# ZhengkunTian/OpenTransformer

Measured on AMD Instinct MI355X. Metric: utterances/sec (80-d fbank, ~1000 frames) train fwd+bwd, higher is better.
Workload: dtype fp16; 1 GPU; AISHELL-1 transformer_baseline.yaml (+input_size 80), 12 enc / 6 dec layers, B=32/GPU x 1000 frames x 80-d fbank, 15 decoder rows, V=4234, residual_dropout 0.1; step = fwd + bwd + grad all-reduce + clip/Adam/Noam; global_batch=32, frames=1000, parallelism=dp1, hipgraph=True

## Files before the change

### include/otrans_hip.h

```cpp
#ifndef OTRANS_HIP_H
#define OTRANS_HIP_H
#include <stddef.h>
#include <stdint.h>
#ifdef __cplusplus
extern "C" {
#endif

#define OTR_F32 0
#define OTR_BF16 1
#define OTR_F16 2
#define OTR_ACT_NONE 0
#define OTR_ACT_RELU 1

#define OTR_ABI_VERSION 606
int32_t otr_version(void);
int32_t otr_half_type(void);
int32_t otr_debug_set(int32_t key, int32_t value);
int32_t otr_set_fault_counter(void* device_word);
int32_t otr_debug_trread(const void* image, const int32_t* addr, void* out, void* stream);
int32_t otr_debug_trace(void* buf);
const char* otr_last_error_string(void);

typedef struct {
  int32_t M, N, K;
// ... 34 lines not shown
int32_t otr_proj_ln_fwd(const float* x, const void* c16, int64_t ldc, const void* w_pack, const float* bias, const float* gamma,
                        const float* beta, const uint64_t* seed, float* y, void* y16, float* z, float* mean, float* rstd,
                        int64_t M, int32_t d_model, float eps, float p_drop, uint64_t rng_offset, void* stream);
int64_t otr_ln_bwd_proj_partial_rows(int64_t M);
int32_t otr_rb_linear_ln_bwd(const void* g16, int64_t ldg, const void* wt_pack, const float* skip, int64_t lds, const float* z,
                             const float* mean, const float* rstd, const float* gamma, const uint64_t* seed, float p_drop,
                             uint64_t rng_offset, float* dx, void* da16, float* partial, int64_t M, int32_t N, int32_t K,
                             void* stream);
int32_t otr_touch(const void* p, int64_t bytes, void* stream);
int32_t otr_zero_tick(float* buf, int64_t n, int64_t* counter, int64_t inc, void* stream);
int32_t otr_touch_hint(const void* p0, int64_t bytes0, const void* p1, int64_t bytes1);
int32_t otr_rb_linear_ln_bwd_pf(const void* g16, int64_t ldg, const void* wt_pack, const float* skip, int64_t lds, const float* z,
                                const float* mean, const float* rstd, const float* gamma, const uint64_t* seed, float p_drop,
                                uint64_t rng_offset, float* dx, void* da16, float* partial, int64_t M, int32_t N, int32_t K,
                                const void* prefetch, int64_t prefetch_bytes, void* stream);
int32_t otr_ln_bwd_proj(const float* dy, const float* z, const float* mean, const float* rstd, const float* gamma,
                        const uint64_t* seed, const void* wt_pack, float* dx, void* da16, void* dc16, int64_t ldc,
                        float* partial, int64_t M, int32_t d_model, float p_drop, uint64_t rng_offset, void* stream);

int64_t otr_ffn_split_scratch_bytes(int64_t M);
int64_t otr_ffn_split_sync_ints(int64_t M);
int64_t otr_ffn_split_hsave_bytes(int64_t M, int32_t F);
int64_t otr_ffn_split_padded_rows(int64_t M);
int32_t otr_ffn_ln_fwd_split(const float* x, const void* x16, const void* w1_pack, const float* b1, const void* w2_pack,
                             const float* b2, const float* gamma, const float* beta, const uint64_t* seed, float p_drop,
                             uint64_t rng_offset, float eps, float* y, void* y16, float* z, float* mean, float* rstd,
                             void* hsave, void* usave, void* scratch, int64_t scratch_bytes, int32_t* sync, int64_t sync_ints,
                             int64_t M, int32_t F, int32_t d_model, void* stream);
int32_t otr_ffn_bwd_split(const void* dy16, const void* hsave, const void* w2t_pack, const void* w1t_pack, void* dh,
                          const float* skip, float* dx, void* scratch, int64_t scratch_bytes, int32_t* sync, int64_t sync_ints,
                          int64_t M, int32_t F, int32_t d_model, void* stream);
int32_t otr_ffn_fwd_split_slab(const void* x16, const void* w1_pack, const float* b1, const void* w2_pack, void* hsave, void* usave,
                               void* slabs, int64_t M, int32_t F, int32_t d_model, void* stream);
int32_t otr_ffn_bwd_split_slab(const void* dy16, const void* hsave, const void* w2t_pack, const void* w1t_pack, void* dh, void* slabs,
                               int64_t M, int32_t F, int32_t d_model, void* stream);
int32_t otr_ln_bwd_proj_slabs(const float* dskip, const void* slabs, int32_t nslab, const float* z, const float* mean, const float* rstd,
                              const float* gamma, const uint64_t* seed, const void* wt_pack, float* dx, void* da16, void* dc16, int64_t ldc,
                              float* partial, int64_t M, int32_t d_model, float p_drop, uint64_t rng_offset, void* stream);
typedef struct {
  const void* dy;
  const void* x;
  float* dw;
  int32_t M, N, K;
  int64_t ldy, ldx, ldw;
  int32_t dy_dtype, x_dtype;
  float* dbias;
  int32_t overwrite;
} otr_wgrad_item_t;
int32_t otr_wgrad256_takes(const otr_wgrad_item_t* item, int32_t compute);
int32_t otr_debug_ffn_split_map(int64_t M, int32_t map, int32_t* out, int32_t cap);
int32_t otr_debug_attention_grid(int32_t nx, int32_t H, int32_t B, int32_t* out, int32_t cap);
int32_t otr_debug_wgrad256_plan(const otr_wgrad_item_t* items, int32_t n, int32_t grid_cap, int32_t* out);
int32_t otr_debug_wgrad256_errors(const void* workspace);
int32_t otr_linear_wgrad_grouped(const otr_wgrad_item_t* items, int32_t n, int32_t compute, void* workspace,
                                 int64_t workspace_bytes, void* stream);
typedef struct {
  const void* a;
  float* out;
  int64_t M, N, lda;
  int32_t dtype;
} otr_colsum_item_t;
int32_t otr_colsum_grouped(const otr_colsum_item_t* items, int32_t n, void* stream);

typedef struct {
  int32_t B, H, Tq, Tk, dk;
  int32_t dtype;
  int64_t q_bs, q_ts, k_bs, k_ts, v_bs, v_ts, o_bs, o_ts;
  int32_t causal;
  float scale;
} otr_attn_desc_t;
int32_t otr_attention_fwd(const otr_attn_desc_t* d, const void* q, const void* k, const void* v,
                          const uint8_t* key_mask, void* o, float* lse, void* stream);
int32_t otr_attention_bwd(const otr_attn_desc_t* d, const void* q, const void* k, const void* v,
                          const uint8_t* key_mask, const void* o, const void* do_, const float* lse,
                          float* delta, void* dq, void* dk, void* dv, void* stream);

int32_t otr_attention_bias_fwd(const otr_attn_desc_t* d, const void* q, const void* k, const void* v,
                               const uint8_t* key_mask, const float* bias, int64_t bias_bs, int64_t bias_hs,
                               int64_t bias_rs, int32_t rel_shift, void* o, float* lse, void* stream);
int32_t otr_attention_bias_bwd(const otr_attn_desc_t* d, const void* q, const void* k, const void* v,
                               const uint8_t* key_mask, const float* bias, void* dbias, int32_t dbias_dtype, int64_t bias_bs,
                               int64_t bias_hs, int64_t bias_rs, int32_t rel_shift, const void* o, const void* do_,
                               const float* lse, float* delta, void* dq, void* dk, void* dv, void* stream);

typedef struct {
  int64_t M;
  int32_t d;
  int32_t a_dtype;
  float eps, p_drop;
  uint64_t rng_offset;
  float a_scale;
  const uint8_t* a_row_mask;
  int32_t dy_dtype;
} otr_ln_desc_t;
int32_t otr_add_layernorm_fwd(const otr_ln_desc_t* d, const float* x, const void* a, const float* gamma,
                              const float* beta, const uint64_t* seed, float* y, void* y_bf16, float* z, float* mean,
                              float* rstd, void* stream);
int32_t otr_add_layernorm_bwd(const otr_ln_desc_t* d, const float* dy, const float* z, const float* mean,
                              const float* rstd, const float* gamma, const uint64_t* seed, float* dx, void* da,
                              float* dgamma, float* dbeta, float* da_colsum, float* partial, void* stream);
int64_t otr_add_layernorm_bwd_partial_rows(int64_t M);
int32_t otr_add_layernorm_bwd_skip(const otr_ln_desc_t* d, const float* dy, const float* z, const float* mean,
                                   const float* rstd, const float* gamma, const uint64_t* seed, const float* skip, float* dx,
                                   void* da, float* dgamma, float* dbeta, float* da_colsum, float* partial, void* stream);

int32_t otr_add_layernorm2_fwd(const otr_ln_desc_t* d, const float* x, const void* a, const float* gamma, const float* beta,
// ... 297 lines not shown
```

### opentransformer_amd/_lib.py

```python
import ctypes as C
import os

_HERE = os.path.dirname(os.path.abspath(__file__))
_LIB_DIR = os.environ.get('OTR_LIB_DIR') or os.path.join(_HERE, 'lib')
LIB_PATHS = {'bf16': os.path.join(_LIB_DIR, 'libotrans_hip.so'), 'fp16': os.path.join(_LIB_DIR, 'libotrans_hip_f16.so')}
LIB_PATH = LIB_PATHS['bf16']

OTR_F32, OTR_BF16, OTR_F16 = 0, 1, 2
OTR_ABI_VERSION = 606
OTR_OPT_STATE_FLOATS = 528
ACT_NONE, ACT_RELU = 0, 1


class LinearDesc(C.Structure):
    _fields_ = [('M', C.c_int32), ('N', C.c_int32), ('K', C.c_int32),
                ('x_dtype', C.c_int32), ('w_dtype', C.c_int32), ('y_dtype', C.c_int32), ('compute', C.c_int32),
                ('ldx', C.c_int64), ('ldw', C.c_int64), ('ldy', C.c_int64),
                ('act', C.c_int32), ('accumulate', C.c_int32)]


class WgradItem(C.Structure):
    _fields_ = [('dy', C.c_void_p), ('x', C.c_void_p), ('dw', C.c_void_p), ('M', C.c_int32), ('N', C.c_int32),
                ('K', C.c_int32), ('ldy', C.c_int64), ('ldx', C.c_int64), ('ldw', C.c_int64),
                ('dy_dtype', C.c_int32), ('x_dtype', C.c_int32), ('dbias', C.c_void_p), ('overwrite', C.c_int32)]
# ... 53 lines not shown
_I32, _I64, _F32 = C.c_int32, C.c_int64, C.c_float

SIGNATURES = {
    'otr_version': [],
    'otr_half_type': [],
    'otr_debug_set': [_I32, _I32],
    'otr_set_fault_counter': [_P],
    'otr_last_error_string': [],
    'otr_linear_fwd': [C.POINTER(LinearDesc), _P, _P, _P, _P, _P, _I64, _P],
    'otr_linear_fwd_batched': [C.POINTER(LinearDesc), _P, _P, _P, _I32, _I64, _I64, _I64, _P],
    'otr_linear_dgrad': [C.POINTER(LinearDesc), _P, _P, _P, _P, _I64, _P],
    'otr_linear_wgrad': [C.POINTER(LinearDesc), _P, _P, _P, _P, _I64, _P],
    'otr_ffn_glu_fwd': [_P, _I64, _P, _I64, _P, _P, _P, _I32, _I32, _I32, _P],
    'otr_ffn_glu_bwd': [_P, _I32, _I64, _P, _I64, _P, _I32, _P, _P, _I32, _P, _I32, _I32, _I32, _P],
    'otr_pack_frags': [_P, _P, _P, _I32, _I64, _P],
    'otr_ffn_ln_fwd': [_P, _P, _P, _P, _P, _P, _P, _P, _P, _F32, C.c_uint64, _F32, _P, _P, _P, _P, _P, _I64, _I32, _I32, _P],
    'otr_ffn_bwd': [_P, _P, _P, _P, _P, _P, _P, _P, _P, _P, _P, _I64, _I32, _I32, _P],
    'otr_ffn_split_scratch_bytes': [_I64],
    'otr_ffn_split_sync_ints': [_I64],
    'otr_ffn_split_hsave_bytes': [_I64, _I32],
    'otr_ffn_split_padded_rows': [_I64],
    'otr_ffn_ln_fwd_split': [_P, _P, _P, _P, _P, _P, _P, _P, _P, _F32, C.c_uint64, _F32, _P, _P, _P, _P, _P, _P, _P, _P, _I64, _P, _I64, _I64, _I32, _I32, _P],
    'otr_ffn_bwd_split': [_P, _P, _P, _P, _P, _P, _P, _P, _I64, _P, _I64, _I64, _I32, _I32, _P],
    'otr_linear_wgrad_grouped': [_P, _I32, _I32, _P, _I64, _P],
    'otr_colsum_grouped': [_P, _I32, _P],
    'otr_colsum': [_P, _I32, _I64, _I64, _I64, _P, _I32, _P],
    'otr_attention_fwd': [C.POINTER(AttnDesc), _P, _P, _P, _P, _P, _P, _P],
    'otr_attention_bwd': [C.POINTER(AttnDesc), _P, _P, _P, _P, _P, _P, _P, _P, _P, _P, _P, _P],
    'otr_attention_bias_fwd': [C.POINTER(AttnDesc), _P, _P, _P, _P, _P, _I64, _I64, _I64, _I32, _P, _P, _P],
    'otr_attention_bias_bwd': [C.POINTER(AttnDesc), _P, _P, _P, _P, _P, _P, _I32, _I64, _I64, _I64, _I32, _P, _P, _P, _P, _P, _P, _P, _P],
    'otr_add_layernorm_fwd': [C.POINTER(LnDesc), _P, _P, _P, _P, _P, _P, _P, _P, _P, _P, _P],
    'otr_add_layernorm_bwd': [C.POINTER(LnDesc), _P, _P, _P, _P, _P, _P, _P, _P, _P, _P, _P, _P, _P],
    'otr_add_layernorm_bwd_skip': [C.POINTER(LnDesc), _P, _P, _P, _P, _P, _P, _P, _P, _P, _P, _P, _P, _P, _P],
    'otr_add_layernorm2_fwd': [C.POINTER(LnDesc)] + [_P] * 15,
    'otr_add_layernorm2_bwd': [C.POINTER(LnDesc)] + [_P] * 15,
    'otr_add_layernorm3_fwd': [C.POINTER(LnDesc)] + [_P] * 20,
    'otr_add_layernorm3_bwd': [C.POINTER(LnDesc), _P, _P, _I32] + [_P] * 18,
    'otr_add_layernorm_bwd_partial_rows': [_I64],
    'otr_rb_linear': [_P, _I64, _P, _P, _P, _I64, _P, _I32, _I64, _I64, _I32, _I32, _P],
    'otr_proj_ln_fwd': [_P, _P, _I64, _P, _P, _P, _P, _P, _P, _P, _P, _P, _P, _I64, _I32, _F32, _F32, C.c_uint64, _P],
    'otr_ln_bwd_proj_partial_rows': [_I64],
    'otr_rb_linear_ln_bwd': [_P, _I64, _P, _P, _I64, _P, _P, _P, _P, _P, _F32, C.c_uint64, _P, _P, _P, _I64, _I32, _I32, _P],
    'otr_touch': [_P, _I64, _P],
    'otr_zero_tick': [_P, _I64, _P, _I64, _P],
    'otr_touch_hint': [_P, _I64, _P, _I64],
    'otr_rb_linear_ln_bwd_pf': [_P, _I64, _P, _P, _I64, _P, _P, _P, _P, _P, _F32, C.c_uint64, _P, _P, _P, _I64, _I32, _I32, _P, _I64, _P],
    'otr_ln_bwd_proj': [_P, _P, _P, _P, _P, _P, _P, _P, _P, _P, _I64, _P, _I64, _I32, _F32, C.c_uint64, _P],
    'otr_debug_trace': [_P],
    'otr_wgrad256_takes': [C.POINTER(WgradItem), _I32],
    'otr_debug_ffn_split_map': [_I64, _I32, _P, _I32],
    'otr_debug_attention_grid': [_I32, _I32, _I32, _P, _I32],
    'otr_debug_wgrad256_plan': [C.POINTER(WgradItem), _I32, _I32, _P],
    'otr_debug_wgrad256_errors': [_P],
    'otr_debug_trread': [_P, _P, _P, _P],
    'otr_spec_mask': [_P, _P, _I32, _I32, _I32, _I32, _P],
    'otr_transpose_batched': [_P, _P, _P, _I32, _I64, _I32, _P],
    'otr_glu_fwd': [_P, _P, _I32, _I64, _I64, _P, _P],
    'otr_glu_bwd': [_P, _P, _P, _P, _I32, _I64, _I64, _P, _I32, _P],
    'otr_posenc_fwd': [_P, _P, _P, _I64, _I32, _I32, _F32, _P],
    'otr_posenc_mask_fwd': [_P, _P, _P, _I64, _I32, _I32, _F32, _P, _I64, _I64, _P, _P],
    'otr_embed_posenc_fwd': [_P, _P, _P, _P, _I64, _I32, _I32, _I32, _F32, _P],
    'otr_embed_posenc_fwd_ld': [_P, _I64, _P, _P, _P, _I64, _I32, _I32, _I32, _F32, _P],
    'otr_embed_bwd_ld': [_P, _I64, _I32, _P, _P, _I32, _P, _I64, _I32, _I32, _F32, _P],
    'otr_embed_bwd': [_P, _P, _P, _I64, _I32, _I32, _F32, _P],
    'otr_scale': [_P, _P, _I64, _P, _F32, _P],
    'otr_scale_cast': [_P, _P, _I64, _F32, _P],
    'otr_cast_f32_to_bf16': [_P, _P, _I64, _P],
    'otr_conv1_fwd': [C.POINTER(ConvDesc), _P, _P, _P, _P, _P],
    'otr_conv1_wgrad': [C.POINTER(ConvDesc), _P, _P, _P, _P, _P, _P],
    'otr_conv1_wgrad_partial_rows': [],
    'otr_conv2_fwd': [C.POINTER(ConvDesc), _P, _P, _P, _P, _P],
    'otr_conv12_fwd': [C.POINTER(ConvDesc), _P, _P, _P, _P, _P, _P, _P, _P],
    'otr_conv2_dgrad_cols': [C.POINTER(ConvDesc), _P, _P, _P, _P],
    'otr_conv2_col2im': [C.POINTER(ConvDesc), _P, _P, _P, _P],
    'otr_conv2_dgrad': [C.POINTER(ConvDesc), _P, _P, _P, _P, _P],
    'otr_conv2_wide_scratch_bytes': [],
    'otr_conv2_dgrad_wide': [C.POINTER(ConvDesc), _P, _P, _P, _P, _P, _I64, _P],
    'otr_debug_conv2_dgrad_plan': [C.POINTER(ConvDesc), _P],
    'otr_conv2_wgrad': [C.POINTER(ConvDesc), _P, _P, _P, _P, _I64, _P],
    'otr_relu_bwd': [_P, _P, _P, _I32, _I64, _P],
    'otr_relu_bwd_colsum_partial_rows': [_I64, _I32, _I32],
    'otr_relu_bwd_colsum': [_P, _P, _P, _P, _I32, _I64, _I32, _P],
    'otr_act_fwd': [_P, _P, _I32, _I64, _I32, _P],
    'otr_act_bwd': [_P, _P, _P, _I32, _I64, _I32, _P],
    'otr_label_smoothing_loss': [_P, _P, _I64, _I32, _F32, _I32, _P, _P, _P, _P],
    'otr_label_smoothing_loss_ld': [_P, _I64, _P, _I64, _I32, _F32, _I32, _P, _P, _I64, _P, _P],
    'otr_label_smoothing_loss_fused': [_P, _I64, _P, _I64, _I32, _I64, _I32, _F32, _I32, _P, _P, _P, _I32, _I64, _P, _P, _P],
    'otr_log_softmax': [_P, _P, _I64, _I32, _P],
    'otr_ctc_loss': [_P, _P, _I64, _P, _P, _I32, _I32, _I32, _I32, _I32, _P, _P, _P, _P, _P],
    'otr_ffn_fwd_split_slab': [_P, _P, _P, _P, _P, _P, _P, _I64, _I32, _I32, _P],
    'otr_ffn_bwd_split_slab': [_P, _P, _P, _P, _P, _P, _I64, _I32, _I32, _P],
    'otr_ln_bwd_proj_slabs': [_P, _P, _I32, _P, _P, _P, _P, _P, _P, _P, _P, _P, _I64, _P, _I64, _I32, _F32, C.c_uint64, _P],
    'otr_rb_linear_ln': [C.POINTER(DecLn), _P, _P, _P, _I32, _I64, _I64, _I32, _I32, _P],
    'otr_dec_self_fwd': [C.POINTER(DecLn), _I32, _I32, _P, _P, _P, _P, _P, _P, _P, _P],
    'otr_dec_self_step': [C.POINTER(DecLn), _I64, _P, _P, _P, _P, _P, _P, _P, _I32, _P, _P],
    'otr_dec_cross_fwd': [C.POINTER(DecLn), _I32, _I32, _P, _P, _P, _P, _I64, _I64, _I32, _I32, _P, _I32, _P, _P, _P, _P, _P],
    'otr_dec_cross_fwd_shared': [C.POINTER(DecLn), _I32, _I32, _P, _P, _P, _P, _I64, _I64, _I32, _I32, _P, _I32, _I32, _P, _P, _P, _P, _P],
    'otr_dec_ffn_hsave_bytes': [_I64, _I32],
    'otr_dec_ffn_fwd': [C.POINTER(DecLn), _I64, _P, _P, _P, _I32, _I32, _P, _P, _P],
    'otr_dec_ln': [C.POINTER(DecLn), _I64, _P],
    'otr_dec_self_step_pair': [C.POINTER(DecSelfStep), C.POINTER(DecSelfStep), _P],
    'otr_dec_ffn_fwd_pair': [C.POINTER(DecFfnFwd), C.POINTER(DecFfnFwd), _P],
    'otr_dec_ln_pair': [C.POINTER(DecLn), _I64, C.POINTER(DecLn), _I64, _P],
    'otr_dec_ffn_bwd': [C.POINTER(DecLnB), _I64, _P, _P, _P, _I32, _I32, _P, _P, _P, _P, _P],
    'otr_dec_cross_bwd': [C.POINTER(DecLnB), _I32, _I32, _P, _P, _P, _P, _P, _P, _P, _I64, _I64, _I32, _I32, _P, _I32, _P, _P, _P],
    'otr_dec_self_bwd': [C.POINTER(DecLnB), _I32, _I32, _P, _P, _P, _P, _P, _P, _P, _P],
# ... 11 lines not shown
    'otr_ctc_topk': [_P, _I64, _P, _I32, _I32, _I32, _I32, _P, _P, _P],
    'otr_ctc_beam_search': [_P, _P, _P, _I32, _I32, _I32, _I32, _I32, _I32, _P, _I64, _P, _P, _P, _P],
    'otr_ngram_lookup': [_P, _I64, _I32, _I32, _I32, _P, _P, _P, _I64, _F32, _P, _P],
    'otr_ctc_beam_search_lm': [_P, _P, _P, _I32, _I32, _I32, _I32, _I32, _I32, _P, _I64, _P, _P, _P, _P, _I64, _I32, _I32, _F32, _F32,
                               _F32, _P, _P],
    'otr_ctc_align_workspace_bytes': [_I32, _I32, _I32],
    'otr_ctc_align': [_P, _I64, _P, _I64, _P, _P, _I32, _I32, _I32, _I32, _I32, _P, _I64, _P, _P, _P, _P, _P],
    'otr_edit_distance': [_P, _I64, _P, _P, _I64, _I64, _P, _I32, _I32, _I32, _I32, _I32, _P, _P, _P, _P],
    'otr_joint_prebeam': [_P, _I64, _P, _I64, _F32, _F32, _I64, _I32, _I32, _P, _P, _P],
    'otr_ctc_prefix_score': [_P, _I64, _P, _I32, _I32, _I32, _I32, _I32, _I64, _I32, _I32, _P, _P, _P, _P, _I64, _I32, _P, _P, _P, _P, _P,
                             _F32, _P, _P, _P, _I32, _P, _P, _P, _P],
    'otr_beam_prune_joint': [_P, _P, _P, _P, _P, _I64, _I32, _I32, _I32, _I32, _P, _P, _P, _P, _P, _P, _P],
    'otr_beam_prune_cached_joint': [_P, _P, _P, _P, _P, _I64, _I32, _I32, _I32, _P, _P, _P, _P, _I32, _P, _P, _P, _P, _P, _P, _P],
    'otr_rescore_pack': [_P, _P, _P, _I64, _I32, _I32, _I32, _I32, _I32, _P, _P, _P, _P],
    'otr_rescore_score': [_P, _I64, _P, _I64, _P, _I64, _P, _I64, _I32, _I32, _P, _P, _P],
    'otr_rescore_select': [_P, _P, _P, _P, _P, _P, _I32, _I32, _I32, _I32, _F32, _F32, _F32, _F32, _P, _P, _P, _P, _P, _P],
    'otr_rescore_select_add': [_P, _P, _P, _P, _P, _P, _P, _I32, _I32, _I32, _I32, _F32, _F32, _F32, _F32, _P, _P, _P, _P, _P, _P],
    'otr_ngram_score_cands': [_P, _I64, _I32, _I32, _I32, _P, _I64, _I32, _P, _P, _P, _P, _I64, _I32, _F32, _F32, _F32, _I32, _P, _P, _I32,
                              _P, _P, _P],
    'otr_ngram_score_seqs': [_P, _I64, _I32, _I32, _I32, _P, _P, _I64, _I32, _F32, _F32, _F32, _I32, _P, _P, _P],
    'otr_decode_embed': [_P, _I64, _P, _P, _P, _P, _I64, _I32, _I32, _F32, _P],
    'otr_decode_lookup': [_P, _I64, _P, _P, _P, _P, _I64, _I32, _I32, _P],
    'otr_lstm_cell': [_P, _P, _P, _P, _P, _P, _P, _I64, _I32, _P],
    'otr_lstm_step_supported': [_I64, _I32],
    'otr_lstm_pack_whh': [_P, _P, _P, _I32, _I32, _P],
    'otr_lstm_fwd_step': [_P, _P, _P, _P, _P, _P, _P, _P, _P, _I32, _I64, _I32, _P],
    'otr_lstm_bwd_step': [_P, _P, _P, _P, _P, _P, _P, _P, _P, _I32, _I64, _I32, _P],
    'otr_lstm_cell_fwd': [_P, _P, _P, _P, _P, _P, _P, _P, _I64, _I32, _P],
    'otr_lstm_cell_bwd': [_P, _P, _P, _P, _P, _P, _P, _P, _I32, _I64, _I32, _P],
    'otr_decode_self_attention': [_P, _P, _P, _P, _P, _P, _I32, _I64, _I32, _I32, _I32, _F32, _P],
    'otr_residual_add_fwd': [_P, _P, _I32, _P, _I64, _F32, _F32, _P, C.c_uint64, _P],
    'otr_residual_add_bwd': [_P, _P, _I32, _I64, _F32, _F32, _P, C.c_uint64, _P],
    'otr_dropout': [_P, _P, _I32, _I64, _F32, _P, C.c_uint64, _P],
    'otr_head_bias_add': [_P, _I64, _P, _P, _P, _I32, _I64, _I32, _P],
    'otr_add2_strided': [_P, _I64, _P, _I64, _P, _I64, _I32, _I64, _I32, _P],
    'otr_add2_colsum_partial_rows': [_I64],
    'otr_add2_strided_colsum': [_P, _I64, _P, _I64, _P, _I64, _I32, _I64, _I32, _P, _P],
    'otr_regroup_add': [_P, _P, _I64, _I32, _I32, _I32, _P],
    'otr_row_mask': [_P, _P, _P, _I64, _I32, _P],
    'otr_row_mask_cast': [_P, _I32, _P, _P, _I32, _I64, _I32, _P],
    'otr_dwconv_fwd': [_P, _I32, _P, _P, _P, _P, _I32, _I32, _I32, _I32, _I32, _P],
    'otr_dwconv_bwd': [_P, _P, _I32, _P, _P, _P, _P, _I32, _I32, _I32, _I32, _I32, _P],
    'otr_dwconv_bwd_part': [_P, _P, _I32, _P, _P, _P, _I32, _I32, _I32, _I32, _I32, _P],
    'otr_dwconv_bwd_partial_rows': [_I64],
    'otr_bn_swish_fwd': [_P, _P, _P, _P, _P, _P, _P, _P, _I32, _I64, _I32, _F32, _F32, _I32, _P],
    'otr_bn_swish_fwd_part': [_P, _P, _I32, _P, _P, _P, _P, _P, _P, _I32, _I64, _I32, _F32, _F32, _P],
    'otr_dwconv_fwd_part': [_P, _I32, _P, _P, _P, _P, _I32, _I32, _I32, _I32, _I32, _P],
    'otr_dwconv_fwd_partial_rows': [_I64],
    'otr_bn_swish_bwd_partial_rows': [_I64],
    'otr_bn_swish_bwd': [_P, _P, _I32, _P, _P, _P, _P, _P, _P, _P, _P, _I64, _I32, _I32, _P],
    'otr_bn_swish_bwd_sums': [_P, _P, _I32, _P, _P, _P, _P, _P, _P, _P, _I64, _I32, _P],
    'otr_conformer_conv_bwd_mid': [_P] * 13 + [_I32] * 7 + [_P],
}
_RESTYPE = {'otr_last_error_string': C.c_char_p, 'otr_dec_ffn_hsave_bytes': C.c_int64, 'otr_ffn_split_scratch_bytes': C.c_int64, 'otr_ffn_split_sync_ints': C.c_int64, 'otr_ffn_split_hsave_bytes': C.c_int64,
            'otr_ffn_split_padded_rows': C.c_int64, 'otr_add_layernorm_bwd_partial_rows': C.c_int64,
            'otr_ln_bwd_proj_partial_rows': C.c_int64, 'otr_dwconv_bwd_partial_rows': C.c_int64, 'otr_dwconv_fwd_partial_rows': C.c_int64,
            'otr_conv2_wide_scratch_bytes': C.c_int64, 'otr_add2_colsum_partial_rows': C.c_int64,
            'otr_ctc_beam_workspace_bytes': C.c_int64, 'otr_ctc_align_workspace_bytes': C.c_int64}

_libs = {}
_kind = 'bf16'


class OtransHipError(RuntimeError):
    pass


def select(kind):
    global _kind
    assert kind in LIB_PATHS
    _kind = kind


def load(kind=None):
    kind = kind or _kind
    lib = _libs.get(kind)
    if lib is not None:
        return lib
    path = LIB_PATHS[kind]
    if not os.path.exists(path):
        raise OtransHipError(
            '%s not found. Build it with `python -c "import __graft_entry__ as g; g.build()"` '
            '(or `make -C opentransformer_amd/csrc`). There is no CPU/PyTorch fallback.' % path)
    lib = C.CDLL(path)
    lib.otr_version.restype = C.c_int32
    if lib.otr_version() != OTR_ABI_VERSION:
        raise OtransHipError('%s answers ABI version %d, this binding was written against %d (include/otrans_hip.h): rebuild it with '
                             '`make -C opentransformer_amd/csrc`' % (path, lib.otr_version(), OTR_ABI_VERSION))
    for name, argtypes in SIGNATURES.items():
        fn = getattr(lib, name)
        fn.argtypes = argtypes
        fn.restype = _RESTYPE.get(name, C.c_int32)
    assert lib.otr_half_type() == (OTR_F16 if kind == 'fp16' else OTR_BF16), 'library / 16-bit type mismatch'
    for kv in filter(None, os.environ.get('OTR_DEBUG_SET', '').split(',')):
        k, v = kv.split('=')
        if lib.otr_debug_set(int(k), int(v)) != 0:
            raise OtransHipError('OTR_DEBUG_SET: bad entry %r' % kv)
    _libs[kind] = lib
    return lib


def check(ret, what):
    if ret != 0:
        msg = load().otr_last_error_string()
        raise OtransHipError('%s failed (%d): %s' % (what, ret, msg.decode() if msg else '?'))
```

### opentransformer_amd/csrc/api.hip

```cpp
#include <stdarg.h>
#include <stdio.h>
#include <stdlib.h>

#include <algorithm>
#include <vector>

#include "gemm_kernel.h"
#include "wgrad256.h"

static thread_local char g_err[512] = "";

void otr_set_error(const char* fmt, ...) {
  va_list ap;
  va_start(ap, fmt);
  vsnprintf(g_err, sizeof(g_err), fmt, ap);
  va_end(ap);
}

int32_t otr_check_launch(const char* what) {
  hipError_t e = hipGetLastError();
  if (e != hipSuccess) {
    otr_set_error("%s: launch failed: %s", what, hipGetErrorString(e));
    return (int32_t)e;
  }
  return 0;
}

static __global__ void zero_f32_kernel(float* p, int64_t n) {
  for (int64_t i = (int64_t)blockIdx.x * blockDim.x + threadIdx.x; i < n; i += (int64_t)gridDim.x * blockDim.x) p[i] = 0.f;
}
void otr_zero_f32(float* p, int64_t n, hipStream_t s) {
  if (n <= 0) return;
  unsigned g = (unsigned)((n + 255) / 256 > 1024 ? 1024 : (n + 255) / 256);
  hipLaunchKernelGGL(zero_f32_kernel, dim3(g), dim3(256), 0, s, p, n);
}

int g_otr_force_tile = 0;
int g_otr_force_ksplit = 0;
int g_otr_conv2_wgrad256 = 1;
int g_otr_attn_enc96 = 1;
int g_otr_wgrad256 = -1;
int g_otr_wgrad256_grid = 0;
int g_otr_conv2_fwd_direct = 1;
int g_otr_attn_enc = 1;
int g_otr_attn_xmap = 1;
int g_otr_attn_bwd_split = 0;
int g_otr_beam_reg = 1;
int g_otr_decode_attn64 = 1;
int g_otr_dec_group = 0;
int g_otr_ffn_map = 1;
int g_otr_ffn_coh_only = 0;
int g_otr_spin_limit = 1 << 22;
int32_t* g_otr_fault = nullptr;
unsigned long long* g_otr_trace = nullptr;
extern "C" int32_t otr_debug_trace(void* buf) { g_otr_trace = (unsigned long long*)buf; return 0; }
extern "C" int32_t otr_debug_set(int32_t key, int32_t value) {
  if (key == 0) g_otr_force_tile = value;
  else if (key == 1) g_otr_force_ksplit = value;
  else if (key == 6) g_otr_wgrad256 = value;
  else if (key == 7) g_otr_wgrad256_grid = value;
  else if (key == 11) g_otr_spin_limit = value > 0 ? value : 1 << 22;
  else if (key == 12) g_otr_ffn_coh_only = value;
  else if (key == 13) g_otr_attn_bwd_split = value;
  else if (key == 15) g_otr_ffn_map = value;
  else if (key == 16) g_otr_attn_xmap = value;
  else if (key == 21) g_otr_attn_enc = value;
  else if (key == 22) g_otr_conv2_fwd_direct = value;
  else if (key == 23) g_otr_dec_group = value;
  else if (key == 24) g_otr_decode_attn64 = value;
  else if (key == 25) g_otr_beam_reg = value;
  else if (key == 29) g_otr_conv2_wgrad256 = value;
  else if (key == 30) g_otr_conv2_dgrad_wide = value;
// ... 149 lines not shown
  a.act = OTR_ACT_GLU_BWD; a.accumulate = 0; a.aux_flag = h_has_sigmoid ? 1 : 0;
  a.a_vec = 1; a.b_vec = 1;
  a.allow_split = 0; a.ws = nullptr; a.ws_bytes = 0; a.trace = g_otr_trace;
  a.aux_in = h; a.aux_out = dh; a.aux_part = dbias_partial;
  const int keep = g_otr_force_tile;
  g_otr_force_tile = big ? 128 : 64;
  const int32_t e = run_gemm(a, OTR_H16, OTR_H16, OTR_H16, OTR_H16, MODE_KC, MODE_KC, stream);
  g_otr_force_tile = keep;
  if (e) return e;
  *partial_rows = rows;
  return 0;
}

static bool wgrad256_ok(const otr_wgrad_item_t& it, int compute) {
  return compute == OTR_H16 && it.dy && it.x && it.dw && it.dy_dtype == OTR_H16 && it.x_dtype == OTR_H16 && it.M >= 256 && it.N >= 128 &&
         it.K >= 96 && it.N % 8 == 0 && it.K % 8 == 0 && it.ldy >= it.N && it.ldx >= it.K && it.ldw >= it.K && it.ldy % 8 == 0 &&
         it.ldx % 8 == 0 && it.ldw % 4 == 0 && (uintptr_t)it.dy % 16 == 0 && (uintptr_t)it.x % 16 == 0 && (uintptr_t)it.dw % 16 == 0 &&
         it.ldy < (1ll << 24) && it.ldx < (1ll << 24) && (int64_t)(it.N + 256) * it.ldw * 4 < (1ll << 31) &&
         (!it.dbias || (uintptr_t)it.dbias % 4 == 0);
}
static void wgrad256_env() {
  if (g_otr_wgrad256 < 0) {
    const char* e = getenv("OTR_WGRAD256");
    g_otr_wgrad256 = (e && e[0] == '0') ? 0 : 1;
  }
}
extern "C" int32_t otr_wgrad256_takes(const otr_wgrad_item_t* item, int32_t compute) {
  wgrad256_env();
  return (item && g_otr_wgrad256 && wgrad256_ok(*item, compute)) ? 1 : 0;
}

extern "C" int32_t otr_linear_wgrad_grouped(const otr_wgrad_item_t* items, int32_t n, int32_t compute, void* workspace,
                                            int64_t workspace_bytes, void* stream) {
  OTR_REQUIRE(n >= 0 && (items || n == 0), "linear_wgrad_grouped: null items");
  OTR_REQUIRE(compute == OTR_H16 || compute == OTR_F32, "linear_wgrad_grouped: bad compute type");
  const int pm = compute == OTR_H16 ? 4 : 2;
  wgrad256_env();
  hipStream_t s = (hipStream_t)stream;
  std::vector<char> taken((size_t)n, 0);
  if (g_otr_wgrad256 && compute == OTR_H16) {
    std::vector<W256Item> big;
    std::vector<int> idx;
    for (int i = 0; i < n; ++i) {
      const otr_wgrad_item_t& it = items[i];
      if (!(it.dy && it.x && it.dw)) continue;
      const bool ok = wgrad256_ok(it, compute);
      if (ok) idx.push_back(i);
    }
    auto narrow = [&](int a) { return items[a].K < 128 ? 1 : 0; };
    std::stable_sort(idx.begin(), idx.end(), [&](int a, int b) {
      if (items[a].M != items[b].M) return items[a].M > items[b].M;
      return narrow(a) < narrow(b);
    });
    size_t c0 = 0;
    while (c0 < idx.size()) {
      size_t c1 = c0;
      while (c1 < idx.size() && c1 - c0 < (size_t)W256_MAX_PROBS && items[idx[c1]].M == items[idx[c0]].M && narrow(idx[c1]) == narrow(idx[c0])) ++c1;
      big.clear();
      for (size_t c = c0; c < c1; ++c) {
        const otr_wgrad_item_t& it = items[idx[c]];
        big.push_back(W256Item{it.dy, it.x, it.dw, it.dbias, it.M, it.N, it.K, it.ldy, it.ldx, it.ldw, it.overwrite != 0});
      }
      if (!workspace || wgrad256_workspace_bytes(big.data(), (int)big.size()) > workspace_bytes) break;
      if (int32_t e = wgrad256_launch(big.data(), (int)big.size(), workspace, workspace_bytes, g_otr_wgrad256_grid, s)) return e;
      for (size_t c = c0; c < c1; ++c) taken[(size_t)idx[c]] = 1;
      c0 = c1;
    }
  }
  std::vector<int> order[16];
  for (int i = 0; i < n; ++i) {
    if (taken[(size_t)i]) continue;
    const otr_wgrad_item_t& it = items[i];
    OTR_REQUIRE(!it.dbias, "linear_wgrad_grouped: item %d carries a bias gradient but does not run on the 256-wide kernel "
                "(check otr_wgrad256_takes first)", i);
    OTR_REQUIRE(it.dy && it.x && it.dw, "linear_wgrad_grouped: item %d has a null pointer", i);
    OTR_REQUIRE(it.M >= 0 && it.N > 0 && it.K > 0 && it.ldy >= it.N && it.ldx >= it.K && it.ldw >= it.K,
                "linear_wgrad_grouped: item %d has a bad shape", i);
    OTR_REQUIRE(dtype_ok(it.dy_dtype) && dtype_ok(it.x_dtype), "linear_wgrad_grouped: item %d has a bad dtype", i);
    if (it.M == 0) continue;
    const bool fast = mc_vec(it.dy, it.ldy, it.dy_dtype, compute) && mc_vec(it.x, it.ldx, it.x_dtype, compute) &&
                      it.N % pm == 0 && it.K % pm == 0 && it.M % (compute == OTR_H16 ? 8 : 4) == 0 &&
                      (uintptr_t)it.dw % 16 == 0 && it.ldw % 4 == 0 &&
                      it.ldy < (1ll << 31) && it.ldx < (1ll << 31) && it.ldw < (1ll << 31);
    if (!fast) {
      otr_linear_desc_t d{};
      d.M = it.M; d.N = it.N; d.K = it.K;
      d.x_dtype = it.x_dtype; d.w_dtype = OTR_F32; d.y_dtype = it.dy_dtype; d.compute = compute;
      d.ldx = it.ldx; d.ldw = it.ldw; d.ldy = it.ldy; d.act = OTR_ACT_NONE; d.accumulate = 1;
      if (int32_t e = otr_linear_wgrad(&d, it.dy, it.x, it.dw, workspace, workspace_bytes, stream)) return e;
      continue;
    }
    const int big = (it.N >= 128 && it.K >= 96) ? 1 : 0;
    order[(big << 2) | ((it.dy_dtype != OTR_F32) << 1) | (it.x_dtype != OTR_F32)].push_back(i);
  }
  for (int key = 4; key < 8; ++key) {
    int64_t t128 = 0;
    for (int i : order[key]) t128 += (int64_t)((items[i].N + 127) / 128) * ((items[i].K + 127) / 128);
    if (!order[key].empty() && t128 < 128) {
      order[key & 3].insert(order[key & 3].end(), order[key].begin(), order[key].end());
      order[key].clear();
    }
  }
  for (int key = 0; key < 8; ++key) {
    std::vector<int>& v = order[key];
    if (v.empty()) continue;
    std::stable_sort(v.begin(), v.end(), [&](int a, int b) { return items[a].M > items[b].M; });
    std::vector<GroupDesc> d(v.size());
    for (size_t c = 0; c < v.size(); ++c) {
      const otr_wgrad_item_t& it = items[v[c]];
      d[c].A = it.dy; d[c].B = it.x; d[c].C = it.dw;
      d[c].M = it.N; d[c].N = it.K; d[c].K = it.M;
      d[c].lda = (int)it.ldy; d[c].ldb = (int)it.ldx; d[c].ldc = (int)it.ldw;
      d[c].a_vec = 1; d[c].b_vec = 1;
    }
    const int ad = ((key >> 1) & 1) ? OTR_H16 : OTR_F32, bd = (key & 1) ? OTR_H16 : OTR_F32, big = key >> 2;
    OTR_REQUIRE(workspace && workspace_bytes >= 4096, "linear_wgrad_grouped: needs a workspace (descriptor table)");
    int32_t e = compute == OTR_H16 ? gemm_grouped_wgrad_bf16(d.data(), (int)d.size(), ad, bd, big, workspace, workspace_bytes, s)
                                    : gemm_grouped_wgrad_f32(d.data(), (int)d.size(), ad, bd, big, workspace, workspace_bytes, s);
    if (e) return e;
// ... 90 lines not shown
```

### opentransformer_amd/csrc/common.h

```cpp
#pragma once
#include <hip/hip_runtime.h>
#include <stdint.h>

#include "../../include/otrans_hip.h"

#ifdef OTR_HALF_FP16
typedef _Float16 otr_hreal;
#define OTR_H16 OTR_F16
#else
typedef __bf16 otr_hreal;
#define OTR_H16 OTR_BF16
#endif
typedef __attribute__((ext_vector_type(8))) otr_hreal bf16x8;
typedef __attribute__((ext_vector_type(2))) otr_hreal bf16x2;
typedef __attribute__((ext_vector_type(4))) float f32x4;
typedef __attribute__((ext_vector_type(2))) float f32x2;
typedef uint16_t bf16_t;

void otr_set_error(const char* fmt, ...);
int32_t otr_check_launch(const char* what);
void otr_zero_f32(float* p, int64_t n, hipStream_t s);
#define OTR_REQUIRE(cond, ...)          \
  do {                                  \
    if (!(cond)) {                      \
      otr_set_error(__VA_ARGS__);       \
      return -1;                        \
    }                                   \
  } while (0)

extern int g_otr_force_tile;
extern int g_otr_force_ksplit;
extern int g_otr_conv2_wgrad256;
extern int g_otr_attn_enc96;
extern int g_otr_wgrad256;
extern int g_otr_wgrad256_grid;
extern int g_otr_conv2_dgrad_wide;
extern int g_otr_conv2_wide;
extern int g_otr_conv2_fwd_direct;
extern int g_otr_attn_enc;
extern int g_otr_attn_xmap;
extern int g_otr_attn_bwd_split;
extern int g_otr_beam_reg;
extern int g_otr_decode_attn64;
extern int g_otr_dec_group;
extern int g_otr_ffn_map;
extern int g_otr_ffn_coh_only;
extern int g_otr_spin_limit;
extern int32_t* g_otr_fault;
extern unsigned long long* g_otr_trace;

typedef uint32_t otr_u32x4 __attribute__((ext_vector_type(4)));
typedef uint32_t otr_u32x2 __attribute__((ext_vector_type(2)));
#define OTR_GLOBAL __attribute__((address_space(1)))
__device__ __forceinline__ uint4 ld_global_b128(const void* p) {
  otr_u32x4 v = *(const OTR_GLOBAL otr_u32x4*)(p);
  return make_uint4(v.x, v.y, v.z, v.w);
}
__device__ __forceinline__ uint2 ld_global_b64(const void* p) {
  otr_u32x2 v = *(const OTR_GLOBAL otr_u32x2*)(p);
  return make_uint2(v.x, v.y);
}
__device__ __forceinline__ void st_global_b128(void* p, uint4 v) {
  otr_u32x4 t = {v.x, v.y, v.z, v.w};
  *(OTR_GLOBAL otr_u32x4*)(p) = t;
}

__device__ __forceinline__ void st_global_b128_nt(void* p, uint4 v) {
  otr_u32x4 t = {v.x, v.y, v.z, v.w};
#if defined(OTR_ST_WT) && OTR_ST_WT
  asm volatile("global_store_dwordx4 %0, %1, off sc0 sc1 nt\n\ts_nop 1" ::"v"(p), "v"(t) : "memory");
#else
  __builtin_nontemporal_store(t, (OTR_GLOBAL otr_u32x4*)(p));
#endif
}

#ifdef OTR_HALF_FP16
__device__ __forceinline__ float bf2f(bf16_t v) { return (float)__builtin_bit_cast(_Float16, v); }
__device__ __forceinline__ float h2f_lo(uint32_t w) { return bf2f((bf16_t)(w & 0xffffu)); }
__device__ __forceinline__ float h2f_hi(uint32_t w) { return bf2f((bf16_t)(w >> 16)); }
#else
__device__ __forceinline__ float bf2f(bf16_t v) { return __uint_as_float(((uint32_t)v) << 16); }
__device__ __forceinline__ float h2f_lo(uint32_t w) { return __uint_as_float(w << 16); }
__device__ __forceinline__ float h2f_hi(uint32_t w) { return __uint_as_float(w & 0xffff0000u); }
#endif
__device__ __forceinline__ bf16_t f2bf(float f) {
  otr_hreal h = (otr_hreal)f;
  return __builtin_bit_cast(bf16_t, h);
}
__device__ __forceinline__ uint32_t pack2bf(float lo, float hi) {
  f32x2 v = {lo, hi};
  bf16x2 h = __builtin_convertvector(v, bf16x2);
  return __builtin_bit_cast(uint32_t, h);
}

__device__ __forceinline__ float h2f(bf16_t v) { return bf2f(v); }
__device__ __forceinline__ bf16_t f2h(float f) { return f2bf(f); }
__device__ __forceinline__ uint32_t pack2h(float lo, float hi) { return pack2bf(lo, hi); }

typedef __attribute__((ext_vector_type(16))) float f32x16;
__device__ __forceinline__ void mma32(f32x16& acc, const uint4& a, const uint4& b) {
#ifdef OTR_HALF_FP16
  acc = __builtin_amdgcn_mfma_f32_32x32x16_f16(__builtin_bit_cast(bf16x8, a), __builtin_bit_cast(bf16x8, b), acc, 0, 0, 0);
#else
// ... 197 lines not shown
```

### opentransformer_amd/csrc/declayer.hip

```cpp
#include "tile32.h"
#include "ln_pro.h"

namespace {

constexpr int DL_H = 4, DL_DK = 64;
constexpr int DL_YS = DL_D * 2 + 16;
constexpr int DL_HS = DL_DK * 2 + 16;
constexpr int DL_VT = DL_RB * 2 + 8;
constexpr int DL_RS = DL_D + 4;

template <int TPW, int NK, int PD> struct DlStream {
  static constexpr int STEPS = TPW * NK;
  static_assert(STEPS % PD == 0 && PD <= STEPS, "ring slots are compile-time constants");
  const uint4* P;
  int nks, tstep;
  uint4 ring[PD];
  __device__ __forceinline__ const uint4* fptr(int s) const { return P + (int64_t)((s % TPW) * tstep * nks + (s / TPW)) * 64; }
  __device__ __forceinline__ void fill(const uint4* pack, int nks_total, int t0, int tstep_, int ks0, int lane) {
    nks = nks_total; tstep = tstep_;
    P = pack + ((int64_t)t0 * nks_total + ks0) * 64 + lane;
#pragma unroll
    for (int s = 0; s < PD; ++s) ring[s] = ld_global_b128(fptr(s));
    __builtin_amdgcn_sched_barrier(0);
  }
// ... 723 lines not shown
  const uint64_t seed = drop ? *q.seed : 0;
  const uint32_t thr = drop ? (uint32_t)fminf(q.p_drop * 4294967296.f, 4294967295.f) : 0;
  const float inv_keep = drop ? 1.f / (1.f - q.p_drop) : 1.f;
  float4 bb = make_float4(0.f, 0.f, 0.f, 0.f);
  if (q.bias) bb = *reinterpret_cast<const float4*>(q.bias + col);
  const float4 gm = *reinterpret_cast<const float4*>(q.gamma + col);
  const float4 bt = *reinterpret_cast<const float4*>(q.beta + col);
  const float g4[4] = {gm.x, gm.y, gm.z, gm.w}, b4[4] = {bt.x, bt.y, bt.z, bt.w};
#pragma unroll
  for (int i = 0; i < 2; ++i) {
    const int r = wid * 2 + i;
    if (r >= nrows) break;
    const int64_t row = row0 + r;
    const float4 xr = *reinterpret_cast<const float4*>(q.xres + row * DL_D + col);
    float a[4] = {bb.x, bb.y, bb.z, bb.w};
    for (int s0 = 0; s0 < q.nslab; s0 += 4) {
      uint2 t[4];
#pragma unroll
      for (int s = 0; s < 4; ++s)
        t[s] = *reinterpret_cast<const uint2*>(reinterpret_cast<const uint16_t*>(q.slabs) + ((int64_t)min(s0 + s, q.nslab - 1) * q.R + row) * DL_D + col);
#pragma unroll
      for (int s = 0; s < 4; ++s) {
        const float live = s0 + s < q.nslab ? 1.f : 0.f;
        a[0] += live * h2f_lo(t[s].x); a[1] += live * h2f_hi(t[s].x); a[2] += live * h2f_lo(t[s].y); a[3] += live * h2f_hi(t[s].y);
      }
    }
    const float xv[4] = {xr.x, xr.y, xr.z, xr.w};
    float v[4], sm = 0.f;
#pragma unroll
    for (int e = 0; e < 4; ++e) {
      float sc = 1.f;
      if (drop) sc = otr_rand32(seed, q.rng_offset + (uint64_t)(row * DL_D + col + e)) >= thr ? inv_keep : 0.f;
      v[e] = xv[e] + a[e] * sc;
      sm += v[e];
    }
    sm = wave_sum(sm) * (1.f / DL_D);
    float qq = 0.f;
#pragma unroll
    for (int e = 0; e < 4; ++e) { const float d = v[e] - sm; qq += d * d; }
    qq = wave_sum(qq);
    const float rstd = rsqrtf(qq * (1.f / DL_D) + q.eps);
    float o[4];
#pragma unroll
    for (int e = 0; e < 4; ++e) o[e] = (v[e] - sm) * rstd * g4[e] + b4[e];
    if (q.z) *reinterpret_cast<float4*>(q.z + row * DL_D + col) = make_float4(v[0], v[1], v[2], v[3]);
    if (q.y) *reinterpret_cast<float4*>(q.y + row * DL_D + col) = make_float4(o[0], o[1], o[2], o[3]);
    if (q.y16) *reinterpret_cast<uint2*>(q.y16 + row * DL_D + col) = make_uint2(pack2h(o[0], o[1]), pack2h(o[2], o[3]));
    if (lane == 0) {
      if (q.mean) q.mean[row] = sm;
      if (q.rstd) q.rstd[row] = rstd;
    }
  }
}
__global__ __launch_bounds__(256) void dec_ln_kernel(DlLnArgs p) { dec_ln_body(p, (int)blockIdx.x); }
struct DlLnPair { DlLnArgs a, b; int n0; };
__global__ __launch_bounds__(256) void dec_ln_pair_kernel(DlLnPair pp) {
  if ((int)blockIdx.x < pp.n0) dec_ln_body(pp.a, (int)blockIdx.x);
  else dec_ln_body(pp.b, (int)blockIdx.x - pp.n0);
}

struct DlLnB {
  const float* dskip;
  const void* slabs;
  int nslab;
  const float* z; const float* mean; const float* rstd; const float* gamma; const uint64_t* seed;
  float p_drop;
  uint64_t rng_offset;
  float* dz;
  uint16_t* da16;
  float* partial;
  int64_t R;
};

template <int NW, int NS> struct DlProB {
  static constexpr int RPW = DL_RB / NW, NP = RPW / 2, D = DL_D;
  int64_t rows[NP];
  float4 z0[NP], z1[NP], k0[NP], k1[NP];
  float mean[NP], rstd[NP];
  otr_u32x4 t[NS][NP];
  float4 gm0, gm1;
  uint64_t seed;
  __device__ __forceinline__ void issue(const DlLnB& p, int64_t row0, int nrows, int tid) {
    const int lane = tid & 63, wid = tid >> 6, hw = lane >> 5, col = (lane & 31) * 8;
    gm0 = *reinterpret_cast<const float4*>(p.gamma + col); gm1 = *reinterpret_cast<const float4*>(p.gamma + col + 4);
    seed = p.p_drop > 0.f ? *p.seed : 0;
#pragma unroll
    for (int k = 0; k < NP; ++k) {
      rows[k] = row0 + min(wid * RPW + 2 * k + hw, nrows - 1);
      z0[k] = *reinterpret_cast<const float4*>(p.z + rows[k] * D + col);
      z1[k] = *reinterpret_cast<const float4*>(p.z + rows[k] * D + col + 4);
      mean[k] = p.mean[rows[k]]; rstd[k] = p.rstd[rows[k]];
      k0[k] = k1[k] = make_float4(0.f, 0.f, 0.f, 0.f);
      if (p.dskip) { k0[k] = *reinterpret_cast<const float4*>(p.dskip + rows[k] * D + col); k1[k] = *reinterpret_cast<const float4*>(p.dskip + rows[k] * D + col + 4); }
    }
#pragma unroll
    for (int s = 0; s < NS; ++s)
      if (s < p.nslab) {
#pragma unroll
        for (int k = 0; k < NP; ++k) {
          const uint4 q = ld_global_b128(reinterpret_cast<const uint16_t*>(p.slabs) + ((int64_t)s * p.R + rows[k]) * D + col);
          t[s][k] = otr_u32x4{q.x, q.y, q.z, q.w};
        }
      }
  }
  __device__ __forceinline__ void finish(const DlLnB& p, int nrows, int block, bool write, unsigned char* img, float* stage, int tid) {
    const int lane = tid & 63, wid = tid >> 6, hw = lane >> 5, col = (lane & 31) * 8;
    const bool drop = p.p_drop > 0.f;
// ... 762 lines not shown
    return e;
  hipLaunchKernelGGL(dec_cross_fwd_kernel<false>, dim3(dl_grid(DL_H, (B + a.g.G - 1) / a.g.G)), dim3(512), 0, (hipStream_t)stream, a);
  return otr_check_launch("dec_cross_fwd");
}

extern "C" int32_t otr_dec_cross_fwd_shared(const otr_dec_ln_t* ln, int32_t B, int32_t L, const void* wq_pack, const float* bq, const void* wo_pack,
                                            const void* kv, int64_t kv_bs, int64_t kv_ts, int32_t koff, int32_t voff, const uint8_t* key_mask,
                                            int32_t Tk, int32_t share, void* q16, void* ctx16, float* lse, void* slabs, void* stream) {
  DlCrossArgs a{};
  OTR_REQUIRE(share >= 1 && B > 0 && B % share == 0, "dec_cross_fwd_shared: %d sequences are not a multiple of share=%d", B, share);
  if (int32_t e = dl_fill_cross("dec_cross_fwd_shared", a, ln, B, L, wq_pack, bq, wo_pack, kv, kv_bs, kv_ts, koff, voff, key_mask, Tk, q16, ctx16,
                                lse, slabs))
    return e;
  a.share = share;
  hipLaunchKernelGGL(dec_cross_fwd_kernel<true>, dim3(dl_grid(DL_H, (B + a.g.G - 1) / a.g.G)), dim3(512), 0, (hipStream_t)stream, a);
  return otr_check_launch("dec_cross_fwd_shared");
}

extern "C" int64_t otr_dec_ffn_hsave_bytes(int64_t R, int32_t F) { return R > 0 && F > 0 ? ((R + DL_RB - 1) / DL_RB) * (int64_t)(F / 32) * 4096 : 0; }

static int32_t dl_fill_ffn_fwd(DlFfnArgs& a, const otr_dec_ln_t* ln, int64_t R, const void* w1_pack, const float* b1, const void* w2_pack, int32_t F,
                               int32_t S, void* slabs, void* hsave) {
  OTR_REQUIRE(R > 0 && R < (1ll << 31), "dec_ffn_fwd: bad row count");
  if (int32_t e = dl_check_ln("dec_ffn_fwd", ln, R, a.ln)) return e;
  OTR_REQUIRE(w1_pack && b1 && w2_pack && slabs, "dec_ffn_fwd: null pointer");
  OTR_REQUIRE(F > 0 && S > 0 && F % (128 * S) == 0, "dec_ffn_fwd: d_ff = %d does not split into %d slices of whole 128-unit wave rounds", F, S);
  OTR_REQUIRE(((uintptr_t)w1_pack | (uintptr_t)b1 | (uintptr_t)w2_pack | (uintptr_t)slabs | (uintptr_t)hsave) % 16 == 0, "dec_ffn_fwd: buffers must be 16-byte aligned");
  a.p1 = (const uint4*)w1_pack; a.b1 = b1; a.p2 = (const uint4*)w2_pack; a.slabs = (uint16_t*)slabs; a.hsave = (uint4*)hsave; a.F = F; a.S = S; a.trace = g_otr_trace;
  return 0;
}
extern "C" int32_t otr_dec_ffn_fwd(const otr_dec_ln_t* ln, int64_t R, const void* w1_pack, const float* b1, const void* w2_pack, int32_t F,
                                   int32_t S, void* slabs, void* hsave, void* stream) {
  DlFfnArgs a{};
  if (int32_t e = dl_fill_ffn_fwd(a, ln, R, w1_pack, b1, w2_pack, F, S, slabs, hsave)) return e;
  hipLaunchKernelGGL(dec_ffn_fwd_kernel, dim3(dl_grid(S, (int)((R + DL_RB - 1) / DL_RB))), dim3(256), 0, (hipStream_t)stream, a);
  return otr_check_launch("dec_ffn_fwd");
}
extern "C" int32_t otr_dec_ffn_fwd_pair(const otr_dec_ffn_fwd_t* x, const otr_dec_ffn_fwd_t* y, void* stream) {
  OTR_REQUIRE(x && y, "dec_ffn_fwd_pair: null descriptor");
  DlFfnPair pp{};
  if (int32_t e = dl_fill_ffn_fwd(pp.a, &x->ln, x->R, x->w1_pack, x->b1, x->w2_pack, x->F, x->S, x->slabs, x->hsave)) return e;
  if (int32_t e = dl_fill_ffn_fwd(pp.b, &y->ln, y->R, y->w1_pack, y->b1, y->w2_pack, y->F, y->S, y->slabs, y->hsave)) return e;
  pp.n0 = (int)dl_grid(x->S, (int)((x->R + DL_RB - 1) / DL_RB));
  const unsigned n1 = dl_grid(y->S, (int)((y->R + DL_RB - 1) / DL_RB));
  hipLaunchKernelGGL(dec_ffn_fwd_pair_kernel, dim3((unsigned)pp.n0 + n1), dim3(256), 0, (hipStream_t)stream, pp);
  return otr_check_launch("dec_ffn_fwd_pair");
}

extern "C" int32_t otr_dec_ln(const otr_dec_ln_t* ln, int64_t R, void* stream) {
  DlLnArgs a{};
  OTR_REQUIRE(R > 0 && R < (1ll << 31), "dec_ln: bad row count");
  if (int32_t e = dl_check_ln("dec_ln", ln, R, a.ln)) return e;
  OTR_REQUIRE(ln->nslab > 0, "dec_ln: nothing to normalise");
  hipLaunchKernelGGL(dec_ln_kernel, dim3((unsigned)((R + 7) / 8)), dim3(256), 0, (hipStream_t)stream, a);
  return otr_check_launch("dec_ln");
}

extern "C" int32_t otr_dec_ln_pair(const otr_dec_ln_t* lx, int64_t Rx, const otr_dec_ln_t* ly, int64_t Ry, void* stream) {
  DlLnPair pp{};
  OTR_REQUIRE(Rx > 0 && Rx < (1ll << 31) && Ry > 0 && Ry < (1ll << 31), "dec_ln_pair: bad row count");
  if (int32_t e = dl_check_ln("dec_ln_pair", lx, Rx, pp.a.ln)) return e;
  if (int32_t e = dl_check_ln("dec_ln_pair", ly, Ry, pp.b.ln)) return e;
  OTR_REQUIRE(lx->nslab > 0 && ly->nslab > 0, "dec_ln_pair: nothing to normalise");
  pp.n0 = (int)((Rx + 7) / 8);
  hipLaunchKernelGGL(dec_ln_pair_kernel, dim3((unsigned)(pp.n0 + (int)((Ry + 7) / 8))), dim3(256), 0, (hipStream_t)stream, pp);
  return otr_check_launch("dec_ln_pair");
}

extern "C" int32_t otr_dec_ffn_bwd(const otr_dec_lnb_t* ln, int64_t R, const void* hsave, const void* w2t_pack, const void* w1t_pack,
                                   int32_t F, int32_t S, void* dh, void* u, float* db1_part, void* slabs, void* stream) {
  DlFfnBwdArgs a{};
  OTR_REQUIRE(R > 0 && R < (1ll << 31), "dec_ffn_bwd: bad row count");
  if (int32_t e = dl_check_lnb("dec_ffn_bwd", ln, R, a.ln)) return e;
  OTR_REQUIRE(hsave && w2t_pack && w1t_pack && dh && u && db1_part && slabs, "dec_ffn_bwd: null pointer");
  OTR_REQUIRE(F > 0 && S > 0 && F % (128 * S) == 0, "dec_ffn_bwd: d_ff = %d does not split into %d slices of whole 128-unit wave rounds", F, S);
  OTR_REQUIRE(((uintptr_t)hsave | (uintptr_t)w2t_pack | (uintptr_t)w1t_pack | (uintptr_t)dh | (uintptr_t)u |
               (uintptr_t)db1_part | (uintptr_t)slabs) % 16 == 0, "dec_ffn_bwd: buffers must be 16-byte aligned");
  a.hsave = (const uint4*)hsave; a.p3 = (const uint4*)w2t_pack; a.p4 = (const uint4*)w1t_pack;
  a.dh = (uint16_t*)dh; a.u = (uint16_t*)u; a.bpart = db1_part; a.slabs = (uint16_t*)slabs; a.F = F; a.S = S; a.trace = g_otr_trace;
  hipLaunchKernelGGL(dec_ffn_bwd_kernel, dim3(dl_grid(S, (int)((R + DL_RB - 1) / DL_RB))), dim3(256), 0, (hipStream_t)stream, a);
  return otr_check_launch("dec_ffn_bwd");
}

extern "C" int32_t otr_dec_cross_bwd(const otr_dec_lnb_t* ln, int32_t B, int32_t L, const void* wo_dgrad_pack, const void* wq_dgrad_pack,
                                     const void* q16, const void* ctx16, const float* lse, const void* kv, void* dkv, int64_t kv_bs,
                                     int64_t kv_ts, int32_t koff, int32_t voff, const uint8_t* key_mask, int32_t Tk, void* dq16, void* slabs,
                                     void* stream) {
  DlCrossBwdArgs a{};
  if (int32_t e = dl_check_geom("dec_cross_bwd", B, L, a.g)) return e;
  if (int32_t e = dl_check_lnb("dec_cross_bwd", ln, (int64_t)B * L, a.ln)) return e;
  OTR_REQUIRE(wo_dgrad_pack && wq_dgrad_pack && q16 && ctx16 && lse && kv && dkv && dq16 && slabs, "dec_cross_bwd: null pointer");
  OTR_REQUIRE(Tk > 0 && kv_ts % 8 == 0 && kv_bs % 8 == 0 && koff % 8 == 0 && voff % 8 == 0, "dec_cross_bwd: key / value rows must be 16-byte aligned");
  OTR_REQUIRE(((uintptr_t)wo_dgrad_pack | (uintptr_t)wq_dgrad_pack | (uintptr_t)q16 | (uintptr_t)ctx16 | (uintptr_t)kv | (uintptr_t)dkv |
               (uintptr_t)dq16 | (uintptr_t)slabs) % 16 == 0, "dec_cross_bwd: buffers must be 16-byte aligned");
  a.wo_t = (const uint4*)wo_dgrad_pack; a.wq_t = (const uint4*)wq_dgrad_pack; a.q16 = (const uint16_t*)q16; a.ctx16 = (const uint16_t*)ctx16;
  a.lse = lse; a.kv = (const uint16_t*)kv; a.dkv = (uint16_t*)dkv; a.kv_bs = kv_bs; a.kv_ts = kv_ts; a.koff = koff; a.voff = voff;
  a.kmask = key_mask; a.Tk = Tk; a.dq16 = (uint16_t*)dq16; a.slabs = (uint16_t*)slabs; a.scale = 0.125f; a.trace = g_otr_trace;
  hipLaunchKernelGGL(dec_cross_bwd_kernel, dim3(dl_grid(DL_H, (B + a.g.G - 1) / a.g.G)), dim3(512), 0, (hipStream_t)stream, a);
  return otr_check_launch("dec_cross_bwd");
}

extern "C" int32_t otr_dec_self_bwd(const otr_dec_lnb_t* ln, int32_t B, int32_t L, const void* wo_dgrad_pack, const void* wqkv_dgrad_pack,
                                    const void* qkv16, const void* ctx16, const float* lse, void* dqkv16, void* slabs, void* stream) {
  DlSelfBwdArgs a{};
  if (int32_t e = dl_check_geom("dec_self_bwd", B, L, a.g)) return e;
  if (int32_t e = dl_check_lnb("dec_self_bwd", ln, (int64_t)B * L, a.ln)) return e;
  OTR_REQUIRE(wo_dgrad_pack && wqkv_dgrad_pack && qkv16 && ctx16 && lse && dqkv16 && slabs, "dec_self_bwd: null pointer");
// ... 17 lines not shown
```

### opentransformer_amd/csrc/elementwise.hip

```cpp
#include "common.h"

static inline unsigned grid_for(int64_t work_items, int block = 256, int64_t cap = 2048 * 4) {
  int64_t g = (work_items + block - 1) / block;
  if (g < 1) g = 1;
  if (g > cap) g = cap;
  return (unsigned)g;
}

__device__ __forceinline__ float sigmoidf_(float x) { return 1.f / (1.f + __expf(-x)); }

template <class T> __global__ void glu_fwd_kernel(const T* h, T* u, int64_t M, int64_t F, const uint8_t* row_mask) {
  constexpr int V = 16 / sizeof(T);
  const int64_t per_row = F / V, total = M * per_row;
  for (int64_t i = (int64_t)blockIdx.x * blockDim.x + threadIdx.x; i < total; i += (int64_t)gridDim.x * blockDim.x) {
    int64_t row = i / per_row, c = (i - row * per_row) * V;
    float a[V], g[V], o[V];
    load_row<T, V>(h + row * 2 * F + c, V, true, a);
    load_row<T, V>(h + row * 2 * F + F + c, V, true, g);
    const bool live = !row_mask || row_mask[row];
#pragma unroll
    for (int e = 0; e < V; ++e) o[e] = live ? a[e] * sigmoidf_(g[e]) : 0.f;
    if constexpr (sizeof(T) == 4) *reinterpret_cast<float4*>(u + row * F + c) = make_float4(o[0], o[1], o[2], o[3]);
    else *reinterpret_cast<uint4*>(u + row * F + c) = MMA<bf16_t>::pack(o);
  }
// ... 454 lines not shown
    const int c = c0 + ty + 8 * i, f = f0 + tx;
    if (f < F && c < C) d[(int64_t)c * F + f] += tile[tx][ty + 8 * i];
  }
}
extern "C" int32_t otr_regroup_add(float* dst, float* src, int64_t rows, int32_t C, int32_t F, int32_t clear_src, void* stream) {
  OTR_REQUIRE(dst && src, "regroup_add: null pointer");
  OTR_REQUIRE(rows >= 0 && rows < 65536 && C > 0 && F > 0, "regroup_add: bad shape");
  if (rows == 0) return 0;
  hipLaunchKernelGGL(regroup_add_kernel, dim3((unsigned)((C + 31) / 32), (unsigned)((F + 31) / 32), (unsigned)rows), dim3(256), 0, (hipStream_t)stream,
                     dst, src, C, F, clear_src);
  return otr_check_launch("regroup_add");
}

constexpr int CS_RPB = 128;
template <class T> __global__ void colsum_kernel(const T* a, int64_t M, int64_t N, int64_t lda, float* out) {
  __shared__ float red[4][64][4];
  const int tx = threadIdx.x, ty = threadIdx.y;
  const int64_t c = ((int64_t)blockIdx.x * 64 + tx) * 4;
  float s[4] = {0.f, 0.f, 0.f, 0.f};
  if (c < N) {
    const int64_t r0 = (int64_t)blockIdx.y * CS_RPB, r1 = min(M, r0 + CS_RPB);
    const bool full = c + 4 <= N && (lda % 4 == 0);
    for (int64_t r = r0 + ty; r < r1; r += 4) {
      float v[4];
      load_row<T, 4>(a + r * lda + c, (int)min((int64_t)4, N - c), full, v);
#pragma unroll
      for (int e = 0; e < 4; ++e) s[e] += v[e];
    }
  }
#pragma unroll
  for (int e = 0; e < 4; ++e) red[ty][tx][e] = s[e];
  __syncthreads();
  if (ty == 0 && c < N) {
#pragma unroll
    for (int e = 0; e < 4; ++e)
      if (c + e < N) atomicAdd(out + c + e, red[0][tx][e] + red[1][tx][e] + red[2][tx][e] + red[3][tx][e]);
  }
}
extern "C" int32_t otr_colsum(const void* a, int32_t dtype, int64_t M, int64_t N, int64_t lda, float* out,
                              int32_t accumulate, void* stream) {
  OTR_REQUIRE(a && out, "colsum: null pointer");
  OTR_REQUIRE(dtype == OTR_F32 || dtype == OTR_H16, "colsum: bad dtype");
  OTR_REQUIRE(N > 0 && M >= 0 && lda >= N, "colsum: bad shape");
  OTR_REQUIRE((uintptr_t)a % 16 == 0, "colsum: input must be 16-byte aligned");
  hipStream_t s = (hipStream_t)stream;
  if (!accumulate) otr_zero_f32(out, N, s);
  if (M == 0) return 0;
  dim3 grid((unsigned)((N + 255) / 256), (unsigned)((M + CS_RPB - 1) / CS_RPB)), block(64, 4);
  if (dtype == OTR_F32) hipLaunchKernelGGL(colsum_kernel<float>, grid, block, 0, s, (const float*)a, M, N, lda, out);
  else hipLaunchKernelGGL(colsum_kernel<bf16_t>, grid, block, 0, s, (const bf16_t*)a, M, N, lda, out);
  return otr_check_launch("colsum");
}

constexpr int CSG_MAX = 64;
struct ColsumGroup {
  int n;
  int first[CSG_MAX + 1];
  const void* a[CSG_MAX];
  float* out[CSG_MAX];
  int M[CSG_MAX], N[CSG_MAX], lda[CSG_MAX], rblocks[CSG_MAX];
  int tpr[CSG_MAX];
  int rpb[CSG_MAX];
};
template <class T> __global__ void colsum_grouped_kernel(ColsumGroup g) {
  constexpr int EPT = 4, UN = 8;
  __shared__ float red[256][EPT];
  const int b = (int)blockIdx.x;
  int i = 0;
  for (int j = 1; j < g.n; ++j) i = (g.first[j] <= b) ? j : i;
  const T* a = reinterpret_cast<const T*>(g.a[i]);
  float* out = g.out[i];
  const int64_t M = g.M[i], N = g.N[i], lda = g.lda[i];
  const int tpr = g.tpr[i], nrl = 256 / tpr;
  const int rpb = g.rpb[i];
  const int lb = b - g.first[i], by = lb % g.rblocks[i], bx = lb / g.rblocks[i];
  const int t = (int)(threadIdx.y * 64 + threadIdx.x);
  const int tx = t % tpr, ty = t / tpr;
  const int64_t c = ((int64_t)bx * tpr + tx) * EPT;
  float s[EPT];
#pragma unroll
  for (int e = 0; e < EPT; ++e) s[e] = 0.f;
  if (c < N && ty < nrl) {
    const int64_t r0 = (int64_t)by * rpb, r1 = min(M, r0 + rpb);
    const bool full = c + EPT <= N && (lda % EPT == 0);
    int64_t r = r0 + ty;
    if (full) {
      for (; r < r1; r += (int64_t)UN * nrl) {
        float v[UN][EPT];
#pragma unroll
        for (int u = 0; u < UN; ++u) load_row<T, EPT>(a + min(r + (int64_t)nrl * u, M - 1) * lda + c, EPT, true, v[u]);
#pragma unroll
        for (int u = 0; u < UN; ++u) {
          const float w = (r + (int64_t)nrl * u < r1) ? 1.f : 0.f;
#pragma unroll
          for (int e = 0; e < EPT; ++e) s[e] += w * v[u][e];
        }
      }
    } else {
      for (; r < r1; r += nrl) {
        float v[EPT];
        load_row<T, EPT>(a + r * lda + c, (int)min((int64_t)EPT, N - c), false, v);
#pragma unroll
        for (int e = 0; e < EPT; ++e) s[e] += v[e];
      }
    }
  }
#pragma unroll
  for (int e = 0; e < EPT; ++e) red[t][e] = s[e];
  __syncthreads();
  if (ty == 0 && c < N) {
#pragma unroll
    for (int e = 0; e < EPT; ++e) {
      float v = 0.f;
      for (int q = 0; q < nrl; ++q) v += red[q * tpr + tx][e];
      if (c + e < N) atomicAdd(out + c + e, v);
    }
  }
}
extern "C" int32_t otr_colsum_grouped(const otr_colsum_item_t* items, int32_t n, void* stream) {
  OTR_REQUIRE(n >= 0 && (items || n == 0), "colsum_grouped: null items");
  hipStream_t s = (hipStream_t)stream;
  for (int pass = 0; pass < 2; ++pass) {
    const int dt = pass == 0 ? OTR_F32 : OTR_H16;
    ColsumGroup g{};
    int blocks = 0;
    auto flush = [&]() -> int32_t {
      if (g.n == 0) return 0;
      g.first[g.n] = blocks;
      if (dt == OTR_F32) hipLaunchKernelGGL(colsum_grouped_kernel<float>, dim3((unsigned)blocks), dim3(64, 4), 0, s, g);
      else hipLaunchKernelGGL(colsum_grouped_kernel<bf16_t>, dim3((unsigned)blocks), dim3(64, 4), 0, s, g);
      g.n = 0;
      blocks = 0;
      return otr_check_launch("colsum_grouped");
    };
    for (int i = 0; i < n; ++i) {
      const otr_colsum_item_t& it = items[i];
      OTR_REQUIRE(it.a && it.out, "colsum_grouped: item %d has a null pointer", i);
      OTR_REQUIRE(it.dtype == OTR_F32 || it.dtype == OTR_H16, "colsum_grouped: item %d has a bad dtype", i);
      OTR_REQUIRE(it.N > 0 && it.M >= 0 && it.lda >= it.N && it.lda < (1ll << 31) && it.M < (1ll << 31),
                  "colsum_grouped: item %d has a bad shape", i);
      OTR_REQUIRE((uintptr_t)it.a % 16 == 0, "colsum_grouped: item %d input must be 16-byte aligned", i);
      if (it.dtype != dt || it.M == 0) continue;
      int tpr = 64;
      while (tpr > 8 && (int64_t)(tpr / 2) * 4 >= it.N) tpr /= 2;
      const int nrl = 256 / tpr, pass_rows = nrl * 8 > 128 ? nrl * 8 : 128;
      int rpb = pass_rows;
      if ((it.M + rpb - 1) / rpb > 192) rpb = (int)(((it.M + 191) / 192 + pass_rows - 1) / pass_rows) * pass_rows;
      const int cpb = tpr * 4;
      const int rb = (int)((it.M + rpb - 1) / rpb), cb = (int)((it.N + cpb - 1) / cpb);
      const int k = g.n++;
      g.first[k] = blocks;
      g.a[k] = it.a; g.out[k] = it.out; g.M[k] = (int)it.M; g.N[k] = (int)it.N; g.lda[k] = (int)it.lda; g.rblocks[k] = rb; g.tpr[k] = tpr; g.rpb[k] = rpb;
      blocks += rb * cb;
      if (g.n == CSG_MAX)
        if (int32_t e = flush()) return e;
    }
    if (int32_t e = flush()) return e;
  }
  return 0;
}

template <class T>
__global__ __launch_bounds__(256) void transpose_batched_kernel(const T* __restrict__ src, T* __restrict__ dst,
                                                               const int64_t* __restrict__ table, int n_mats) {
  __shared__ T tile[64][65];
  const int64_t b = blockIdx.x;
  int lo = 0, hi = n_mats - 1;
  while (lo < hi) {
    int mid = (lo + hi + 1) >> 1;
    if (table[mid * 4 + 3] <= b) lo = mid; else hi = mid - 1;
  }
  const int64_t off = table[lo * 4], rows = table[lo * 4 + 1], cols = table[lo * 4 + 2];
  const int64_t t = b - table[lo * 4 + 3];
  const int64_t tc = (cols + 63) >> 6;
  const int64_t r0 = (t / tc) << 6, c0 = (t % tc) << 6;
  const T* s = src + off;
  T* d = dst + off;
  if constexpr (sizeof(T) == 2) {
    const bool fast = r0 + 64 <= rows && c0 + 64 <= cols && cols % 8 == 0 && rows % 8 == 0 && off % 8 == 0;
    if (fast) {
      const int tid = threadIdx.x;
#pragma unroll
      for (int u = 0; u < 2; ++u) {
        const int id = tid + 256 * u, r = id >> 3, ch = id & 7;
        const uint4 v = *reinterpret_cast<const uint4*>(s + (r0 + r) * cols + c0 + ch * 8);
        const uint32_t w[4] = {v.x, v.y, v.z, v.w};
#pragma unroll
        for (int e = 0; e < 8; ++e) tile[r][ch * 8 + e] = (T)((w[e >> 1] >> ((e & 1) * 16)) & 0xffffu);
      }
      __syncthreads();
#pragma unroll
      for (int u = 0; u < 2; ++u) {
        const int id = tid + 256 * u, c = id >> 3, ch = id & 7;
        uint32_t w[4];
#pragma unroll
        for (int e = 0; e < 4; ++e) w[e] = (uint32_t)tile[ch * 8 + 2 * e][c] | ((uint32_t)tile[ch * 8 + 2 * e + 1][c] << 16);
        *reinterpret_cast<uint4*>(d + (c0 + c) * rows + r0 + ch * 8) = make_uint4(w[0], w[1], w[2], w[3]);
      }
      return;
    }
  }
  const int tx = threadIdx.x & 63, ty = threadIdx.x >> 6;
  for (int r = ty; r < 64; r += 4)
    if (r0 + r < rows && c0 + tx < cols) tile[r][tx] = s[(r0 + r) * cols + c0 + tx];
  __syncthreads();
  for (int c = ty; c < 64; c += 4)
    if (c0 + c < cols && r0 + tx < rows) d[(c0 + c) * rows + r0 + tx] = tile[tx][c];
}

extern "C" int32_t otr_transpose_batched(const void* src, void* dst, const int64_t* table, int32_t n_mats,
                                         int64_t total_tiles, int32_t elem_bytes, void* stream) {
  OTR_REQUIRE(src && dst && table, "transpose_batched: null pointer");
// ... 36 lines not shown
```

### opentransformer_amd/csrc/norm.hip

```cpp
#include "common.h"

struct LnArgs {
  const float* x; const void* a; const float* gamma; const float* beta; const uint64_t* seed;
  float* y; float* z; float* mean; float* rstd; bf16_t* y_lp;
  const float* dy; float* dx; void* da; float* dgamma; float* dbeta; const float* zin; float* da_colsum; float* partial;
  int64_t M; int d;
  float eps, p_drop;
  uint64_t rng_offset;
  const float* skip;
  float a_scale;
  const float* gamma2; const float* beta2; float* mean2; float* rstd2;
  const float* gamma3; const float* beta3; float* mean3; float* rstd3; float* y3; bf16_t* y3_lp; const void* dy3; int dy3_h16;
  int dy_h16;
  const uint8_t* amask;
};

constexpr int LN_MAXV = 4;

template <class AT> __device__ __forceinline__ void ld4(const AT* p, float* o) {
  if constexpr (sizeof(AT) == 4) {
    float4 v = *reinterpret_cast<const float4*>(p);
    o[0] = v.x; o[1] = v.y; o[2] = v.z; o[3] = v.w;
  } else {
    uint2 v = *reinterpret_cast<const uint2*>(p);
    o[0] = h2f_lo(v.x); o[1] = h2f_hi(v.x);
    o[2] = h2f_lo(v.y); o[3] = h2f_hi(v.y);
  }
}
template <class AT> __device__ __forceinline__ void st4(AT* p, const float* o) {
  if constexpr (sizeof(AT) == 4) *reinterpret_cast<float4*>(p) = make_float4(o[0], o[1], o[2], o[3]);
  else *reinterpret_cast<uint2*>(p) = make_uint2(pack2bf(o[0], o[1]), pack2bf(o[2], o[3]));
}

__device__ __forceinline__ float drop_scale(uint64_t seed, uint64_t idx, uint32_t thr, float inv_keep) {
  return otr_rand32(seed, idx) >= thr ? inv_keep : 0.f;
}

template <class AT, bool HAS_A, bool LN2 = false> __global__ __launch_bounds__(256) void add_ln_fwd_kernel(LnArgs p) {
  const int lane = threadIdx.x & 63, wid = threadIdx.x >> 6;
  const int64_t row = (int64_t)blockIdx.x * 4 + wid;
  if (row >= p.M) return;
  const int d = p.d;
  const bool drop = HAS_A && p.p_drop > 0.f;
  const uint64_t seed = drop ? *p.seed : 0;
  const uint32_t thr = drop ? (uint32_t)fminf(p.p_drop * 4294967296.f, 4294967295.f) : 0;
  const float inv_keep = (drop ? 1.f / (1.f - p.p_drop) : 1.f) * p.a_scale;
  float v[LN_MAXV][4];
  float s = 0.f;
  const float am = (HAS_A && p.amask) ? (p.amask[row] ? 1.f : 0.f) : 1.f;
#pragma unroll
  for (int i = 0; i < LN_MAXV; ++i) {
    int col = (i * 64 + lane) * 4;
    if (col < d) {
      ld4<float>(p.x + row * d + col, v[i]);
      if constexpr (HAS_A) {
        float a[4];
        ld4<AT>(reinterpret_cast<const AT*>(p.a) + row * d + col, a);
#pragma unroll
        for (int e = 0; e < 4; ++e) {
          float sc = drop ? drop_scale(seed, p.rng_offset + (uint64_t)(row * d + col + e), thr, inv_keep) : inv_keep;
          v[i][e] += a[e] * sc * am;
        }
      }
      if (p.z) st4<float>(p.z + row * d + col, v[i]);
      s += v[i][0] + v[i][1] + v[i][2] + v[i][3];
    }
  }
// ... 49 lines not shown
    }
    if (lane == 0) { p.mean[row] = mean; p.rstd[row] = rstd; p.mean2[row] = mean2; p.rstd2[row] = rstd2; }
    if (p.gamma3) {
      float s3 = 0.f;
#pragma unroll
      for (int i = 0; i < LN_MAXV; ++i)
        if ((i * 64 + lane) * 4 < d) s3 += v[i][0] + v[i][1] + v[i][2] + v[i][3];
      const float mean3 = wave_sum(s3) / d;
      float q3 = 0.f;
#pragma unroll
      for (int i = 0; i < LN_MAXV; ++i)
        if ((i * 64 + lane) * 4 < d) {
#pragma unroll
          for (int e = 0; e < 4; ++e) { float t = v[i][e] - mean3; q3 += t * t; }
        }
      const float rstd3 = rsqrtf(wave_sum(q3) / d + p.eps);
#pragma unroll
      for (int i = 0; i < LN_MAXV; ++i) {
        int col = (i * 64 + lane) * 4;
        if (col < d) {
          float g[4], bta[4], o[4];
          ld4<float>(p.gamma3 + col, g);
          ld4<float>(p.beta3 + col, bta);
#pragma unroll
          for (int e = 0; e < 4; ++e) o[e] = (v[i][e] - mean3) * rstd3 * g[e] + bta[e];
          if (p.y3) st4<float>(p.y3 + row * d + col, o);
          if (p.y3_lp) st4<bf16_t>(p.y3_lp + row * d + col, o);
        }
      }
      if (lane == 0) { p.mean3[row] = mean3; p.rstd3[row] = rstd3; }
    }
    return;
  }
#pragma unroll
  for (int i = 0; i < LN_MAXV; ++i) {
    int col = (i * 64 + lane) * 4;
    if (col < d) {
      float g[4], bta[4], o[4];
      ld4<float>(p.gamma + col, g);
      ld4<float>(p.beta + col, bta);
#pragma unroll
      for (int e = 0; e < 4; ++e) o[e] = (v[i][e] - mean) * rstd * g[e] + bta[e];
      if (p.y) st4<float>(p.y + row * d + col, o);
      if (p.y_lp) st4<bf16_t>(p.y_lp + row * d + col, o);
    }
  }
  if (lane == 0) { p.mean[row] = mean; p.rstd[row] = rstd; }
}

constexpr int LN_BWD_ROWS = 4;

template <class AT, bool HAS_A, int NV, bool LN2 = false> __global__ __launch_bounds__(512) void add_ln_bwd_kernel(LnArgs p) {
  constexpr int ROWS = 1, NWV = 8, NTH = 64 * NWV;
  __shared__ float red[2][NWV][NV * 256];
  const int lane = threadIdx.x & 63, wid = threadIdx.x >> 6;
  const int d = p.d;
  const bool drop = HAS_A && p.p_drop > 0.f;
  const uint64_t seed = drop ? *p.seed : 0;
  const uint32_t thr = drop ? (uint32_t)fminf(p.p_drop * 4294967296.f, 4294967295.f) : 0;
  const float inv_keep = (drop ? 1.f / (1.f - p.p_drop) : 1.f) * p.a_scale;
  const bool want_ab = HAS_A && p.da_colsum != nullptr;
  float gam[NV][4], dg[NV][4], db[NV][4], dab[NV][4];
  int colv[NV];
  float cmask[NV];
#pragma unroll
  for (int i = 0; i < NV; ++i) {
    const int col = (i * 64 + lane) * 4;
    cmask[i] = col < d ? 1.f : 0.f;
    colv[i] = min(col, d - 4);
#pragma unroll
    for (int e = 0; e < 4; ++e) { dg[i][e] = 0.f; db[i][e] = 0.f; dab[i][e] = 0.f; }
    ld4<float>(p.gamma + colv[i], gam[i]);
  }
  float gam2[NV][4], bet1[NV][4], dg2[NV][4], db2[NV][4];
  float gam3[NV][4], bet2[NV][4], dg3[NV][4], db3[NV][4];
  const bool three = LN2 && p.dy3 != nullptr;
  if constexpr (LN2) {
#pragma unroll
    for (int i = 0; i < NV; ++i) {
      ld4<float>(p.gamma2 + colv[i], gam2[i]);
      ld4<float>(p.beta + colv[i], bet1[i]);
#pragma unroll
      for (int e = 0; e < 4; ++e) { dg2[i][e] = 0.f; db2[i][e] = 0.f; dg3[i][e] = 0.f; db3[i][e] = 0.f; gam3[i][e] = 0.f; bet2[i][e] = 0.f; }
      if (three) { ld4<float>(p.gamma3 + colv[i], gam3[i]); ld4<float>(p.beta2 + colv[i], bet2[i]); }
    }
  }
  const int64_t row0 = ((int64_t)blockIdx.x * NWV + wid) * ROWS;
  float dyv[ROWS][NV][4], zh[ROWS][NV][4], mean[ROWS], rstd[ROWS];
  float mean2[ROWS], rstd2[ROWS], mean3[ROWS], rstd3[ROWS];
  float dy3v[LN2 ? ROWS : 1][NV][4];
#pragma unroll
  for (int rr = 0; rr < ROWS; ++rr) {
    const int64_t row = min(row0 + rr, p.M - 1);
    mean[rr] = p.mean[row];
    rstd[rr] = p.rstd[row];
    if constexpr (LN2) {
      mean2[rr] = p.mean2[row]; rstd2[rr] = p.rstd2[row];
      mean3[rr] = three ? p.mean3[row] : 0.f; rstd3[rr] = three ? p.rstd3[row] : 0.f;
    }
#pragma unroll
    for (int i = 0; i < NV; ++i) {
      if (p.dy_h16) ld4<bf16_t>(reinterpret_cast<const bf16_t*>(p.dy) + row * d + colv[i], dyv[rr][i]);
      else ld4<float>(p.dy + row * d + colv[i], dyv[rr][i]);
      ld4<float>(p.zin + row * d + colv[i], zh[rr][i]);
      if constexpr (LN2) {
        if (three) {
// ... 175 lines not shown
    }
  }
}

static int32_t ln_check(const otr_ln_desc_t* d) {
  OTR_REQUIRE(d != nullptr, "layernorm: null descriptor");
  OTR_REQUIRE(d->M >= 0 && d->d > 0 && d->d % 4 == 0 && d->d <= LN_MAXV * 256,
              "layernorm: d=%d must be a multiple of 4 and <= %d", d->d, LN_MAXV * 256);
  OTR_REQUIRE(d->p_drop >= 0.f && d->p_drop < 1.f, "layernorm: p_drop=%f out of [0,1)", (double)d->p_drop);
  OTR_REQUIRE(d->a_dtype == OTR_F32 || d->a_dtype == OTR_H16, "layernorm: bad a_dtype");
  return 0;
}

extern "C" int32_t otr_add_layernorm_fwd(const otr_ln_desc_t* d, const float* x, const void* a, const float* gamma,
                                         const float* beta, const uint64_t* seed, float* y, void* y_bf16, float* z,
                                         float* mean, float* rstd, void* stream) {
  if (int32_t e = ln_check(d)) return e;
  OTR_REQUIRE(x && gamma && beta && (y || y_bf16) && mean && rstd, "add_layernorm_fwd: null pointer");
  OTR_REQUIRE(d->p_drop == 0.f || (a && seed), "add_layernorm_fwd: dropout needs a and seed");
  if (d->M == 0) return 0;
  LnArgs p{};
  p.x = x; p.a = a; p.gamma = gamma; p.beta = beta; p.seed = seed; p.y = y; p.z = z; p.mean = mean; p.rstd = rstd; p.y_lp = (bf16_t*)y_bf16;
  p.M = d->M; p.d = d->d; p.eps = d->eps; p.p_drop = d->p_drop; p.rng_offset = d->rng_offset;
  p.a_scale = d->a_scale == 0.f ? 1.f : d->a_scale; p.amask = d->a_row_mask;
  dim3 grid((unsigned)((d->M + 3) / 4));
  hipStream_t s = (hipStream_t)stream;
  if (!a) hipLaunchKernelGGL((add_ln_fwd_kernel<float, false>), grid, dim3(256), 0, s, p);
  else if (d->a_dtype == OTR_F32) hipLaunchKernelGGL((add_ln_fwd_kernel<float, true>), grid, dim3(256), 0, s, p);
  else hipLaunchKernelGGL((add_ln_fwd_kernel<bf16_t, true>), grid, dim3(256), 0, s, p);
  return otr_check_launch("add_layernorm_fwd");
}

extern "C" int32_t otr_add_layernorm_bwd(const otr_ln_desc_t* d, const float* dy, const float* z, const float* mean,
                                         const float* rstd, const float* gamma, const uint64_t* seed, float* dx,
                                         void* da, float* dgamma, float* dbeta, float* da_colsum, float* partial,
                                         void* stream) {
  return otr_add_layernorm_bwd_skip(d, dy, z, mean, rstd, gamma, seed, nullptr, dx, da, dgamma, dbeta, da_colsum, partial, stream);
}
extern "C" int32_t otr_add_layernorm_bwd_skip(const otr_ln_desc_t* d, const float* dy, const float* z, const float* mean,
                                              const float* rstd, const float* gamma, const uint64_t* seed, const float* skip,
                                              float* dx, void* da, float* dgamma, float* dbeta, float* da_colsum, float* partial,
                                              void* stream) {
  if (int32_t e = ln_check(d)) return e;
  OTR_REQUIRE(dy && z && mean && rstd && gamma && dx && (partial || (dgamma && dbeta)), "add_layernorm_bwd: null pointer");
  OTR_REQUIRE(d->p_drop == 0.f || seed, "add_layernorm_bwd: dropout needs seed");
  if (d->M == 0) return 0;
  LnArgs p{};
  p.dy = dy; p.zin = z; p.mean = const_cast<float*>(mean); p.rstd = const_cast<float*>(rstd); p.gamma = gamma;
  OTR_REQUIRE(d->dy_dtype == OTR_F32 || d->dy_dtype == OTR_H16, "add_layernorm_bwd: bad dy_dtype %d", d->dy_dtype);
  p.dy_h16 = d->dy_dtype == OTR_H16;
  p.seed = seed; p.skip = skip; p.dx = dx; p.da = da; p.dgamma = dgamma; p.dbeta = dbeta; p.da_colsum = da ? da_colsum : nullptr; p.partial = partial;
  p.M = d->M; p.d = d->d; p.eps = d->eps; p.p_drop = d->p_drop; p.rng_offset = d->rng_offset;
  p.a_scale = d->a_scale == 0.f ? 1.f : d->a_scale; p.amask = d->a_row_mask;
  dim3 grid((unsigned)((d->M + 2 * LN_BWD_ROWS - 1) / (2 * LN_BWD_ROWS)));
  hipStream_t s = (hipStream_t)stream;
#define LN_BWD_LAUNCH(NV)                                                                                   \
  {                                                                                                         \
    if (!da) hipLaunchKernelGGL((add_ln_bwd_kernel<float, false, NV>), grid, dim3(512), 0, s, p);           \
    else if (d->a_dtype == OTR_F32) hipLaunchKernelGGL((add_ln_bwd_kernel<float, true, NV>), grid, dim3(512), 0, s, p); \
    else hipLaunchKernelGGL((add_ln_bwd_kernel<bf16_t, true, NV>), grid, dim3(512), 0, s, p);               \
  }
  const int nv = (d->d + 255) / 256;
  if (nv == 1) LN_BWD_LAUNCH(1) else if (nv == 2) LN_BWD_LAUNCH(2) else if (nv == 3) LN_BWD_LAUNCH(3) else LN_BWD_LAUNCH(4)
#undef LN_BWD_LAUNCH
  return otr_check_launch("add_layernorm_bwd");
}

extern "C" int32_t otr_add_layernorm2_fwd(const otr_ln_desc_t* d, const float* x, const void* a, const float* gamma, const float* beta,
                                          const float* gamma2, const float* beta2, const uint64_t* seed, float* y2, void* y2_bf16,
                                          float* z, float* mean, float* rstd, float* mean2, float* rstd2, void* stream) {
  if (int32_t e = ln_check(d)) return e;
  OTR_REQUIRE(x && gamma && beta && gamma2 && beta2 && y2 && mean && rstd && mean2 && rstd2, "add_layernorm2_fwd: null pointer");
  OTR_REQUIRE(d->p_drop == 0.f || (a && seed), "add_layernorm2_fwd: dropout needs a and seed");
  if (d->M == 0) return 0;
  LnArgs p{};
  p.x = x; p.a = a; p.gamma = gamma; p.beta = beta; p.gamma2 = gamma2; p.beta2 = beta2; p.seed = seed; p.y = y2; p.z = z;
  p.mean = mean; p.rstd = rstd; p.mean2 = mean2; p.rstd2 = rstd2; p.y_lp = (bf16_t*)y2_bf16;
  p.M = d->M; p.d = d->d; p.eps = d->eps; p.p_drop = d->p_drop; p.rng_offset = d->rng_offset;
  p.a_scale = d->a_scale == 0.f ? 1.f : d->a_scale; p.amask = d->a_row_mask;
  dim3 grid((unsigned)((d->M + 3) / 4));
  hipStream_t s = (hipStream_t)stream;
  if (!a) hipLaunchKernelGGL((add_ln_fwd_kernel<float, false, true>), grid, dim3(256), 0, s, p);
  else if (d->a_dtype == OTR_F32) hipLaunchKernelGGL((add_ln_fwd_kernel<float, true, true>), grid, dim3(256), 0, s, p);
  else hipLaunchKernelGGL((add_ln_fwd_kernel<bf16_t, true, true>), grid, dim3(256), 0, s, p);
  return otr_check_launch("add_layernorm2_fwd");
}

extern "C" int32_t otr_add_layernorm2_bwd(const otr_ln_desc_t* d, const float* dy2, const float* z, const float* mean, const float* rstd,
                                          const float* gamma, const float* beta, const float* mean2, const float* rstd2,
                                          const float* gamma2, const uint64_t* seed, const float* skip, float* dx, void* da,
                                          float* partial, void* stream) {
  if (int32_t e = ln_check(d)) return e;
  OTR_REQUIRE(dy2 && z && mean && rstd && gamma && beta && mean2 && rstd2 && gamma2 && dx && partial, "add_layernorm2_bwd: null pointer");
  OTR_REQUIRE(d->p_drop == 0.f || seed, "add_layernorm2_bwd: dropout needs seed");
  if (d->M == 0) return 0;
  LnArgs p{};
  p.dy = dy2; p.zin = z; p.mean = const_cast<float*>(mean); p.rstd = const_cast<float*>(rstd); p.gamma = gamma; p.beta = beta;
  p.mean2 = const_cast<float*>(mean2); p.rstd2 = const_cast<float*>(rstd2); p.gamma2 = gamma2;
  p.seed = seed; p.skip = skip; p.dx = dx; p.da = da; p.partial = partial;
  p.M = d->M; p.d = d->d; p.eps = d->eps; p.p_drop = d->p_drop; p.rng_offset = d->rng_offset;
  p.a_scale = d->a_scale == 0.f ? 1.f : d->a_scale; p.amask = d->a_row_mask;
  dim3 grid((unsigned)((d->M + 2 * LN_BWD_ROWS - 1) / (2 * LN_BWD_ROWS)));
  hipStream_t s = (hipStream_t)stream;
#define LN2_BWD_LAUNCH(NV)                                                                                        \
  {                                                                                                               \
    if (!da) hipLaunchKernelGGL((add_ln_bwd_kernel<float, false, NV, true>), grid, dim3(512), 0, s, p);           \
    else if (d->a_dtype == OTR_F32) hipLaunchKernelGGL((add_ln_bwd_kernel<float, true, NV, true>), grid, dim3(512), 0, s, p); \
// ... 64 lines not shown
```

### opentransformer_amd/csrc/optim.hip

```cpp
#include "common.h"

struct OptState {
  float step;
  float lr;
  float bc1, bc2;
  float sqnorm;
  float skipped;
  float loss_scale;
  float good_steps;
  float unscale;
  float growth_interval;
  float faults;
  float reserved[5];
  float norm_part[512];
};
constexpr int OPT_NORM_WG = 512;

__global__ void sqnorm_kernel(const float* g, int64_t n, OptState* st) {
  __shared__ float sh[4];
  float s = 0.f;
  const int64_t n4 = n / 4;
  const float4* g4 = reinterpret_cast<const float4*>(g);
  const int64_t stride = (int64_t)gridDim.x * blockDim.x;
  int64_t i = (int64_t)blockIdx.x * blockDim.x + threadIdx.x;
  for (; i + 3 * stride < n4; i += 4 * stride) {
    float4 v0 = g4[i], v1 = g4[i + stride], v2 = g4[i + 2 * stride], v3 = g4[i + 3 * stride];
    s += v0.x * v0.x + v0.y * v0.y + v0.z * v0.z + v0.w * v0.w;
    s += v1.x * v1.x + v1.y * v1.y + v1.z * v1.z + v1.w * v1.w;
    s += v2.x * v2.x + v2.y * v2.y + v2.z * v2.z + v2.w * v2.w;
    s += v3.x * v3.x + v3.y * v3.y + v3.z * v3.z + v3.w * v3.w;
  }
  for (; i < n4; i += stride) {
    float4 v = g4[i];
    s += v.x * v.x + v.y * v.y + v.z * v.z + v.w * v.w;
  }
  if (blockIdx.x == 0 && threadIdx.x < (n & 3)) { float v = g[n4 * 4 + threadIdx.x]; s += v * v; }
  s = wave_sum(s);
  if ((threadIdx.x & 63) == 0) sh[threadIdx.x >> 6] = s;
  __syncthreads();
  if (threadIdx.x == 0) st->norm_part[blockIdx.x] = sh[0] + sh[1] + sh[2] + sh[3];
}

__global__ void opt_tick_kernel(OptState* st, float base_lr, float model_size, float warmup, float factor,
                                float step_offset, float beta1, float beta2, float grad_scale, int32_t* fault, int nparts) {
  float part = 0.f;
  for (int i = threadIdx.x; i < nparts; i += 64) part += st->norm_part[i];
  part = wave_sum(part);
  if (threadIdx.x != 0) return;
  st->sqnorm = part;
  const float ls = st->loss_scale > 0.f ? st->loss_scale : 1.f;
  const float us = grad_scale / ls;
  st->unscale = us;
  if (fault) {
    const int32_t nf = __hip_atomic_exchange(fault, 0, __ATOMIC_RELAXED, __HIP_MEMORY_SCOPE_AGENT);
    if (nf != 0) {
      st->faults += (float)nf;
      st->skipped += 1.f;
      st->unscale = __builtin_nanf("");
      return;
    }
  }
  float norm = sqrtf(st->sqnorm) * us;
  if (!isfinite(norm)) {
    st->skipped += 1.f;
    if (st->loss_scale > 0.f) { st->loss_scale = fmaxf(ls * 0.5f, 1.f); st->good_steps = 0.f; }
    return;
  }
  if (st->loss_scale > 0.f) {
    st->good_steps += 1.f;
    if (st->growth_interval > 0.f && st->good_steps >= st->growth_interval) {
      st->loss_scale = fminf(ls * 2.f, 65536.f);
      st->good_steps = 0.f;
    }
  }
  float t = st->step + 1.f;
  st->step = t;
  st->bc1 = 1.f - powf(beta1, t);
  st->bc2 = 1.f - powf(beta2, t);
  if (warmup > 0.f) {
    float s = t + step_offset;
    st->lr = factor * rsqrtf(model_size) * fminf(rsqrtf(s), s * powf(warmup, -1.5f));
  } else {
    st->lr = base_lr;
  }
}

__device__ __forceinline__ float otr_gauss(uint64_t seed, uint64_t idx) {
  const float u1 = ((float)otr_rand32_sm64(seed, 2 * idx) + 1.f) * (1.f / 4294967296.f);
  const float u2 = (float)otr_rand32_sm64(seed, 2 * idx + 1) * (1.f / 4294967296.f);
  return sqrtf(-2.f * __logf(u1)) * __cosf(6.2831853f * u2);
}

__device__ __forceinline__ void adam_one(float& pi, float gi, float& mi, float& vi, int64_t i, float coef, float wd, float beta1, float beta2,
                                         float step_size, float rbc2, float eps, float noise_std, uint64_t nseed) {
  const bool pad = gi == 0.f && pi == 0.f;
  gi *= coef;
  if (noise_std > 0.f && !pad) gi += noise_std * otr_gauss(nseed, (uint64_t)i);
  gi += wd * pi;
  mi = beta1 * mi + (1.f - beta1) * gi;
  vi = beta2 * vi + (1.f - beta2) * gi * gi;
  pi = pi - step_size * mi / (sqrtf(vi) * rbc2 + eps);
}
__global__ __launch_bounds__(256) void adam_kernel(float* p, const float* g, float* m, float* v, int64_t n, const OptState* st, bf16_t* p_lp,
                                                   float beta1, float beta2, float eps, float wd, float clip, float noise_std) {
  const float us = st->unscale;
  const float norm = sqrtf(st->sqnorm) * us;
  if (!isfinite(norm)) return;
  const float coef = us * (clip > 0.f ? fminf(1.f, clip / (norm + 1e-6f)) : 1.f);
  const float lr = st->lr, bc1 = st->bc1, rbc2 = rsqrtf(st->bc2);
  const float step_size = lr / bc1;
  const uint64_t nseed = 0x6E015Eull + (uint64_t)st->step * 0x9E3779B97F4A7C15ull;
  typedef float f4 __attribute__((ext_vector_type(4)));
  const int64_t n4 = n >> 2;
  for (int64_t i = (int64_t)blockIdx.x * blockDim.x + threadIdx.x; i < n4; i += (int64_t)gridDim.x * blockDim.x) {
    f4 pv = __builtin_nontemporal_load(reinterpret_cast<const f4*>(p) + i);
    const f4 gv = *(reinterpret_cast<const f4*>(g) + i);
    f4 mv = __builtin_nontemporal_load(reinterpret_cast<const f4*>(m) + i);
    f4 vv = __builtin_nontemporal_load(reinterpret_cast<const f4*>(v) + i);
#pragma unroll
    for (int e = 0; e < 4; ++e) {
      float pi = pv[e], mi = mv[e], vi = vv[e];
      adam_one(pi, gv[e], mi, vi, 4 * i + e, coef, wd, beta1, beta2, step_size, rbc2, eps, noise_std, nseed);
      pv[e] = pi; mv[e] = mi; vv[e] = vi;
    }
    __builtin_nontemporal_store(mv, reinterpret_cast<f4*>(m) + i);
    __builtin_nontemporal_store(vv, reinterpret_cast<f4*>(v) + i);
    __builtin_nontemporal_store(pv, reinterpret_cast<f4*>(p) + i);
    if (p_lp) *reinterpret_cast<uint2*>(p_lp + 4 * i) = make_uint2((uint32_t)f2bf(pv[0]) | ((uint32_t)f2bf(pv[1]) << 16), (uint32_t)f2bf(pv[2]) | ((uint32_t)f2bf(pv[3]) << 16));
  }
  if (blockIdx.x == 0 && threadIdx.x < (n & 3)) {
    const int64_t i = 4 * n4 + threadIdx.x;
    float pi = p[i], mi = m[i], vi = v[i];
    adam_one(pi, g[i], mi, vi, i, coef, wd, beta1, beta2, step_size, rbc2, eps, noise_std, nseed);
    p[i] = pi; m[i] = mi; v[i] = vi;
    if (p_lp) p_lp[i] = f2bf(pi);
  }
}

extern "C" int32_t otr_optimizer_step(float* param, const float* grad, float* exp_avg, float* exp_avg_sq, int64_t n,
                                      float* state, int32_t state_floats, void* param_bf16, float base_lr, float beta1, float beta2, float eps,
                                      float weight_decay, float grad_scale, float clip_norm, float noam_model_size,
                                      float noam_warmup, float noam_factor, float noam_step_offset, float grad_noise_std,
                                      void* stream) {
  OTR_REQUIRE(param && grad && exp_avg && exp_avg_sq && state, "optimizer_step: null pointer");
  OTR_REQUIRE(n > 0, "optimizer_step: empty parameter buffer");
  OTR_REQUIRE(grad_noise_std >= 0.f, "optimizer_step: grad_noise_std must be >= 0");
  OTR_REQUIRE((uintptr_t)grad % 16 == 0, "optimizer_step: grad buffer must be 16-byte aligned");
  OTR_REQUIRE(state_floats >= OTR_OPT_STATE_FLOATS, "optimizer_step: the state block must hold OTR_OPT_STATE_FLOATS floats "
              "(the gradient-norm partial sums live behind the 16 state slots)");
  OTR_REQUIRE(((uintptr_t)param | (uintptr_t)exp_avg | (uintptr_t)exp_avg_sq) % 16 == 0 && (!param_bf16 || (uintptr_t)param_bf16 % 8 == 0),
              "optimizer_step: parameter / moment buffers must be 16-byte aligned (the 16-bit shadow 8-byte)");
  hipStream_t s = (hipStream_t)stream;
  OptState* st = reinterpret_cast<OptState*>(state);
  unsigned grid = (unsigned)((n / 4 + 255) / 256 > OPT_NORM_WG ? OPT_NORM_WG : (n / 4 + 255) / 256);
  if (grid < 1) grid = 1;
  hipLaunchKernelGGL(sqnorm_kernel, dim3(grid), dim3(256), 0, s, grad, n, st);
  hipLaunchKernelGGL(opt_tick_kernel, dim3(1), dim3(64), 0, s, st, base_lr, noam_model_size, noam_warmup, noam_factor,
                     noam_step_offset, beta1, beta2, grad_scale, g_otr_fault, (int)grid);
  unsigned g2 = (unsigned)((n / 4 + 255) / 256 > 4096 ? 4096 : (n / 4 + 255) / 256);
  if (g2 < 1) g2 = 1;
  hipLaunchKernelGGL(adam_kernel, dim3(g2), dim3(256), 0, s, param, grad, exp_avg, exp_avg_sq, n, st, (bf16_t*)param_bf16, beta1, beta2, eps,
                     weight_decay, clip_norm, grad_noise_std);
  return otr_check_launch("optimizer_step");
}
```

### opentransformer_amd/csrc/rowblock.hip

```cpp
#include "tile32.h"
#include "ln_pro.h"

namespace {

constexpr int RB = 32;
constexpr int RB_PD = 16;

template <int K, int NTHR = 256> __device__ __forceinline__ void rb_stage_rows(uint4* dst, const uint16_t* src, int64_t ld, int row0, int M, int tid) {
  constexpr int CPR = K / 8, PER = RB * CPR / NTHR;
  uint4 v[PER];
#pragma unroll
  for (int j = 0; j < PER; ++j) {
    const int i = tid + j * NTHR, r = i / CPR, ch = i % CPR;
    v[j] = ld_global_b128(src + (int64_t)min(row0 + r, M - 1) * ld + ch * 8);
  }
#pragma unroll
  for (int j = 0; j < PER; ++j) {
    const int i = tid + j * NTHR, r = i / CPR, ch = i % CPR;
    dst[r * CPR + (ch ^ (r & 15))] = v[j];
  }
}

template <int K, int TPW> struct RbStream {
  static constexpr int NKS = K / 16, STEPS = NKS * TPW;
  static_assert(STEPS % RB_PD == 0, "ring slots are compile-time constants");
  const uint4* P;
  int rot;
  uint4 ring[RB_PD];
  __device__ __forceinline__ int ks_of(int s) const {
    const int k = s / TPW + rot;
    return k >= NKS ? k - NKS : k;
  }
  __device__ __forceinline__ const uint4* fptr(int s) const { return P + (int64_t)((s % TPW) * NKS + ks_of(s)) * 64; }
  __device__ __forceinline__ void fill(const uint4* pw, int t0, int lane) {
    rot = (int)((blockIdx.x >> 3) % (unsigned)NKS);
    P = pw + (int64_t)t0 * NKS * 64 + lane;
#pragma unroll
    for (int s = 0; s < RB_PD; ++s) ring[s] = ld_global_b128(fptr(s));
    __builtin_amdgcn_sched_barrier(0);
  }
  __device__ __forceinline__ void run(f32x16 (&acc)[TPW], const uint4* xs, int lane) {
    const int m = lane & 31, hi = lane >> 5;
    uint4 xb;
#pragma clang loop unroll(full)
    for (int s = 0; s < STEPS; ++s) {
      if (s % TPW == 0) xb = frag_xor<K>(xs, m, hi, ks_of(s));
      const uint4 w = ring[s % RB_PD];
      mma32(acc[s % TPW], w, xb);
      if (s + RB_PD < STEPS) ring[s % RB_PD] = ld_global_b128(fptr(s + RB_PD));
      __builtin_amdgcn_sched_barrier(0);
    }
  }
};

struct RbTouch { const unsigned char* p[2]; int64_t lines[2]; };
constexpr int RB_TOUCH_PER = 10;
__device__ __forceinline__ void rb_touch_issue(const RbTouch& t, uint32_t (&sink)[RB_TOUCH_PER], int tid, int nthr) {
  if (!t.p[0]) return;
  const int64_t total = t.lines[0] + t.lines[1];
  const int64_t per = min((total + gridDim.x - 1) / gridDim.x, (int64_t)RB_TOUCH_PER * nthr), l0 = (int64_t)blockIdx.x * per;
#pragma unroll
  for (int k = 0; k < RB_TOUCH_PER; ++k) {
    const int64_t l = l0 + tid + (int64_t)k * nthr;
    if (l < l0 + per && l < total) {
      const unsigned char* a = l < t.lines[0] ? t.p[0] + l * 64 : t.p[1] + (l - t.lines[0]) * 64;
      asm volatile("global_load_dword %0, %1, off" : "+v"(sink[k]) : "v"(a) : "memory");
    }
  }
}
__device__ __forceinline__ void rb_touch_wait(uint32_t (&sink)[RB_TOUCH_PER]) {
  asm volatile("s_waitcnt vmcnt(0)" : "+v"(sink[0]), "+v"(sink[1]), "+v"(sink[2]), "+v"(sink[3]), "+v"(sink[4]), "+v"(sink[5]), "+v"(sink[6]), "+v"(sink[7]),
               "+v"(sink[8]), "+v"(sink[9])::"memory");
}

struct RbLinArgs {
  const uint16_t* x16;
  const uint4* pw;
  const float* bias;
  const float* skip;
  void* out;
  int64_t ldx, lds, ldo;
  int M, N, out_h16;
};

template <int K, int TPW, int NSPLIT = 1>
__global__ __launch_bounds__(256, NSPLIT) void rb_linear_kernel(RbLinArgs p) {
  constexpr int N = 128 * TPW, RS = N + 4;
  const int cbase = (int)blockIdx.y * N;
  __shared__ __attribute__((aligned(16))) unsigned char smem[RB * K * 2 + RB * RS * 4];
  uint4* xs = reinterpret_cast<uint4*>(smem);
  float* red = reinterpret_cast<float*>(smem + RB * K * 2);
  const int tid = threadIdx.x, lane = tid & 63;
  const int wid = __builtin_amdgcn_readfirstlane(tid >> 6);
  const int row0 = blockIdx.x * RB;
  RbStream<K, TPW> ws;
  ws.fill(p.pw, (int)blockIdx.y * 4 * TPW + wid * TPW, lane);
  rb_stage_rows<K>(xs, p.x16, p.ldx, row0, p.M, tid);
  __syncthreads();
  f32x16 acc[TPW];
#pragma unroll
  for (int i = 0; i < TPW; ++i)
#pragma unroll
    for (int r = 0; r < 16; ++r) acc[i][r] = 0.f;
  ws.run(acc, xs, lane);
#pragma unroll
  for (int i = 0; i < TPW; ++i) put_tile<RS>(red, acc[i], (wid * TPW + i) * 32, lane);
  __syncthreads();
#pragma unroll
// ... 438 lines not shown

}

extern "C" int32_t otr_rb_linear(const void* x16, int64_t ldx, const void* w_pack, const float* bias, const float* skip, int64_t lds,
                                 void* out, int32_t out_dtype, int64_t ldo, int64_t M, int32_t N, int32_t K, void* stream) {
  OTR_REQUIRE(x16 && w_pack && out, "rb_linear: null pointer");
  OTR_REQUIRE(M >= 0 && M < (1ll << 31), "rb_linear: bad M");
  OTR_REQUIRE((K == 256 && (N == 256 || N == 768)) || (K == 768 && N == 256), "rb_linear: built for (N, K) in {(256,256), (768,256), (256,768)}, got (%d, %d)", N, K);
  OTR_REQUIRE(out_dtype == OTR_F32 || out_dtype == OTR_H16, "rb_linear: bad out dtype");
  OTR_REQUIRE(ldx >= K && ldx % 8 == 0 && (uintptr_t)x16 % 16 == 0, "rb_linear: x rows must be 16-byte aligned");
  OTR_REQUIRE(ldo >= N && ldo % 4 == 0 && (uintptr_t)out % 16 == 0 && (uintptr_t)w_pack % 16 == 0, "rb_linear: out / pack alignment");
  OTR_REQUIRE(!skip || (lds >= N && lds % 4 == 0 && (uintptr_t)skip % 16 == 0), "rb_linear: skip alignment");
  OTR_REQUIRE(!bias || (uintptr_t)bias % 16 == 0, "rb_linear: bias alignment");
  if (M == 0) return 0;
  RbLinArgs p{};
  p.x16 = reinterpret_cast<const uint16_t*>(x16); p.pw = reinterpret_cast<const uint4*>(w_pack); p.bias = bias; p.skip = skip; p.out = out;
  p.ldx = ldx; p.lds = lds; p.ldo = ldo; p.M = (int)M; p.N = N; p.out_h16 = out_dtype == OTR_H16;
  const dim3 grid((unsigned)((M + RB - 1) / RB));
  hipStream_t s = (hipStream_t)stream;
  if (K == 256 && N == 256) hipLaunchKernelGGL((rb_linear_kernel<256, 2>), grid, dim3(256), 0, s, p);
  else if (K == 256) hipLaunchKernelGGL((rb_linear_kernel<256, 3, 2>), dim3(grid.x, 2), dim3(256), 0, s, p);
  else hipLaunchKernelGGL((rb_linear_kernel<768, 2>), grid, dim3(256), 0, s, p);
  return otr_check_launch("rb_linear");
}

extern "C" int32_t otr_rb_linear_ln(const otr_dec_ln_t* ln, const void* w_pack, const float* bias, void* out, int32_t out_dtype, int64_t ldo,
                                    int64_t M, int32_t N, int32_t K, void* stream) {
  OTR_REQUIRE(ln && w_pack && out, "rb_linear_ln: null pointer");
  OTR_REQUIRE(M > 0 && M < (1ll << 31) && N == 768 && K == 256, "rb_linear_ln: built for the q|k|v projection (N, K) = (768, 256), got (%d, %d)", N, K);
  OTR_REQUIRE(ln->nslab > 0 && ln->nslab <= 4 && ln->xres && ln->slabs && ln->gamma && ln->beta, "rb_linear_ln: bad LayerNorm descriptor");
  OTR_REQUIRE(ln->p_drop >= 0.f && ln->p_drop < 1.f && (ln->p_drop == 0.f || ln->seed), "rb_linear_ln: bad dropout arguments");
  OTR_REQUIRE(out_dtype == OTR_F32 || out_dtype == OTR_H16, "rb_linear_ln: bad out dtype");
  OTR_REQUIRE(ldo >= N && ldo % 4 == 0 && ((uintptr_t)out | (uintptr_t)w_pack | (uintptr_t)bias | (uintptr_t)ln->xres | (uintptr_t)ln->slabs |
                                           (uintptr_t)ln->bias | (uintptr_t)ln->gamma | (uintptr_t)ln->beta | (uintptr_t)ln->y | (uintptr_t)ln->y16 |
                                           (uintptr_t)ln->z) % 16 == 0, "rb_linear_ln: alignment");
  RbLinLnArgs p{};
  p.ln.xres = ln->xres; p.ln.x16 = nullptr; p.ln.slabs = ln->slabs; p.ln.nslab = ln->nslab; p.ln.bias = ln->bias; p.ln.gamma = ln->gamma;
  p.ln.beta = ln->beta; p.ln.seed = ln->seed; p.ln.p_drop = ln->p_drop; p.ln.eps = ln->eps; p.ln.rng_offset = ln->rng_offset;
  p.ln.y = ln->y; p.ln.y16 = (uint16_t*)ln->y16; p.ln.z = ln->z; p.ln.mean = ln->mean; p.ln.rstd = ln->rstd; p.ln.R = M;
  p.pw = reinterpret_cast<const uint4*>(w_pack); p.bias = bias; p.out = out; p.ldo = ldo; p.M = (int)M; p.out_h16 = out_dtype == OTR_H16;
  hipLaunchKernelGGL((rb_linear_ln_kernel<3, 1, 8>), dim3((unsigned)((M + RB - 1) / RB), 1), dim3(512), 0, (hipStream_t)stream, p);
  return otr_check_launch("rb_linear_ln");
}

static thread_local RbTouch g_touch_hint{};
extern "C" int32_t otr_touch_hint(const void* p0, int64_t bytes0, const void* p1, int64_t bytes1) {
  OTR_REQUIRE(bytes0 >= 0 && bytes1 >= 0 && (p0 || bytes0 == 0) && (p1 || bytes1 == 0), "touch_hint: bad range");
  g_touch_hint = RbTouch{};
  int n = 0;
  if (bytes0 >= 64) { g_touch_hint.p[n] = reinterpret_cast<const unsigned char*>(p0); g_touch_hint.lines[n] = bytes0 / 64; ++n; }
  if (bytes1 >= 64) { g_touch_hint.p[n] = reinterpret_cast<const unsigned char*>(p1); g_touch_hint.lines[n] = bytes1 / 64; ++n; }
  return 0;
}
static RbTouch take_touch_hint() { RbTouch t = g_touch_hint; g_touch_hint = RbTouch{}; return t; }

extern "C" int32_t otr_proj_ln_fwd(const float* x, const void* c16, int64_t ldc, const void* w_pack, const float* bias, const float* gamma,
                                   const float* beta, const uint64_t* seed, float* y, void* y16, float* z, float* mean, float* rstd,
                                   int64_t M, int32_t d_model, float eps, float p_drop, uint64_t rng_offset, void* stream) {
  OTR_REQUIRE(x && c16 && w_pack && gamma && beta && y && mean && rstd, "proj_ln_fwd: null pointer");
  OTR_REQUIRE(d_model == 256, "proj_ln_fwd: built for d_model = 256 (got %d)", d_model);
  OTR_REQUIRE(M >= 0 && M < (1ll << 31) && ldc >= 256 && ldc % 8 == 0 && (uintptr_t)c16 % 16 == 0, "proj_ln_fwd: bad shape / alignment");
  OTR_REQUIRE(p_drop >= 0.f && p_drop < 1.f && (p_drop == 0.f || seed), "proj_ln_fwd: bad dropout");
  if (M == 0) return 0;
  ProjLnArgs p{};
  p.x = x; p.c16 = reinterpret_cast<const uint16_t*>(c16); p.pw = reinterpret_cast<const uint4*>(w_pack); p.bias = bias; p.gamma = gamma;
  p.beta = beta; p.seed = seed; p.y = y; p.y16 = reinterpret_cast<uint16_t*>(y16); p.z = z; p.mean = mean; p.rstd = rstd;
  p.ldc = ldc; p.M = (int)M; p.eps = eps; p.p_drop = p_drop; p.rng_offset = rng_offset;
  p.touch = take_touch_hint();
  hipLaunchKernelGGL(proj_ln_fwd_kernel<8>, dim3((unsigned)((M + RB - 1) / RB)), dim3(512), 0, (hipStream_t)stream, p);
  return otr_check_launch("proj_ln_fwd");
}

extern "C" int64_t otr_ln_bwd_proj_partial_rows(int64_t M) { return (M + RB - 1) / RB; }


extern "C" int32_t otr_ln_bwd_proj(const float* dy, const float* z, const float* mean, const float* rstd, const float* gamma,
                                   const uint64_t* seed, const void* wt_pack, float* dx, void* da16, void* dc16, int64_t ldc,
                                   float* partial, int64_t M, int32_t d_model, float p_drop, uint64_t rng_offset, void* stream) {
  OTR_REQUIRE(dy && z && mean && rstd && gamma && wt_pack && dc16, "ln_bwd_proj: null pointer");
  OTR_REQUIRE(d_model == 256, "ln_bwd_proj: built for d_model = 256 (got %d)", d_model);
  OTR_REQUIRE(M >= 0 && M < (1ll << 31) && ldc >= 256 && ldc % 4 == 0 && (uintptr_t)dc16 % 8 == 0, "ln_bwd_proj: bad shape / alignment");
  OTR_REQUIRE(p_drop >= 0.f && p_drop < 1.f && (p_drop == 0.f || seed), "ln_bwd_proj: bad dropout");
  if (M == 0) return 0;
  LnBwdProjArgs p{};
  p.dy = dy; p.z = z; p.mean = mean; p.rstd = rstd; p.gamma = gamma; p.seed = seed; p.pwt = reinterpret_cast<const uint4*>(wt_pack);
  p.dx = dx; p.da16 = reinterpret_cast<uint16_t*>(da16); p.dc16 = reinterpret_cast<uint16_t*>(dc16); p.partial = partial;
  p.ldc = ldc; p.M = (int)M; p.p_drop = p_drop; p.rng_offset = rng_offset;
  p.touch = take_touch_hint();
  hipLaunchKernelGGL(ln_bwd_proj_kernel<8>, dim3((unsigned)((M + RB - 1) / RB)), dim3(512), 0, (hipStream_t)stream, p);
  return otr_check_launch("ln_bwd_proj");
}

extern "C" int32_t otr_ln_bwd_proj_slabs(const float* dskip, const void* slabs, int32_t nslab, const float* z, const float* mean, const float* rstd,
                                         const float* gamma, const uint64_t* seed, const void* wt_pack, float* dx, void* da16, void* dc16,
                                         int64_t ldc, float* partial, int64_t M, int32_t d_model, float p_drop, uint64_t rng_offset,
                                         void* stream) {
  OTR_REQUIRE(dskip && slabs && z && mean && rstd && gamma && wt_pack && dc16, "ln_bwd_proj_slabs: null pointer");
  OTR_REQUIRE(nslab > 0 && nslab <= 4 && (uintptr_t)slabs % 8 == 0, "ln_bwd_proj_slabs: 1 .. 4 slabs");
  OTR_REQUIRE(d_model == 256, "ln_bwd_proj_slabs: built for d_model = 256 (got %d)", d_model);
  OTR_REQUIRE(M >= 0 && M < (1ll << 31) && ldc >= 256 && ldc % 4 == 0 && (uintptr_t)dc16 % 8 == 0, "ln_bwd_proj_slabs: bad shape / alignment");
  OTR_REQUIRE(p_drop >= 0.f && p_drop < 1.f && (p_drop == 0.f || seed), "ln_bwd_proj_slabs: bad dropout");
  if (M == 0) return 0;
  LnBwdProjArgs p{};
  p.slabs = reinterpret_cast<const uint16_t*>(slabs); p.nslab = nslab;
  p.dy = dskip; p.z = z; p.mean = mean; p.rstd = rstd; p.gamma = gamma; p.seed = seed; p.pwt = reinterpret_cast<const uint4*>(wt_pack);
  p.dx = dx; p.da16 = reinterpret_cast<uint16_t*>(da16); p.dc16 = reinterpret_cast<uint16_t*>(dc16); p.partial = partial;
  p.ldc = ldc; p.M = (int)M; p.p_drop = p_drop; p.rng_offset = rng_offset;
  p.touch = take_touch_hint();
  hipLaunchKernelGGL(ln_bwd_proj_kernel<8>, dim3((unsigned)((M + RB - 1) / RB)), dim3(512), 0, (hipStream_t)stream, p);
  return otr_check_launch("ln_bwd_proj_slabs");
}

extern "C" int32_t otr_rb_linear_ln_bwd_pf(const void* g16, int64_t ldg, const void* wt_pack, const float* skip, int64_t lds, const float* z,
                                           const float* mean, const float* rstd, const float* gamma, const uint64_t* seed, float p_drop,
                                           uint64_t rng_offset, float* dx, void* da16, float* partial, int64_t M, int32_t N, int32_t K,
                                           const void* prefetch, int64_t prefetch_bytes, void* stream);
extern "C" int32_t otr_rb_linear_ln_bwd(const void* g16, int64_t ldg, const void* wt_pack, const float* skip, int64_t lds, const float* z,
                                        const float* mean, const float* rstd, const float* gamma, const uint64_t* seed, float p_drop,
                                        uint64_t rng_offset, float* dx, void* da16, float* partial, int64_t M, int32_t N, int32_t K,
                                        void* stream) {
  return otr_rb_linear_ln_bwd_pf(g16, ldg, wt_pack, skip, lds, z, mean, rstd, gamma, seed, p_drop, rng_offset, dx, da16, partial, M, N, K, nullptr,
                                 0, stream);
}

extern "C" int32_t otr_rb_linear_ln_bwd_pf(const void* g16, int64_t ldg, const void* wt_pack, const float* skip, int64_t lds, const float* z,
                                           const float* mean, const float* rstd, const float* gamma, const uint64_t* seed, float p_drop,
                                           uint64_t rng_offset, float* dx, void* da16, float* partial, int64_t M, int32_t N, int32_t K,
                                           const void* prefetch, int64_t prefetch_bytes, void* stream) {
  OTR_REQUIRE(prefetch_bytes >= 0 && (prefetch || prefetch_bytes == 0), "rb_linear_ln_bwd: bad prefetch range");
  OTR_REQUIRE(g16 && wt_pack && z && mean && rstd && gamma && dx && da16 && partial, "rb_linear_ln_bwd: null pointer");
  OTR_REQUIRE(N == 256 && (K == 256 || K == 768), "rb_linear_ln_bwd: built for N = 256, K in {256, 768} (got %d, %d)", N, K);
  OTR_REQUIRE(M >= 0 && M < (1ll << 31) && ldg >= K && ldg % 8 == 0 && (uintptr_t)g16 % 16 == 0 && (uintptr_t)wt_pack % 16 == 0,
              "rb_linear_ln_bwd: bad shape / alignment");
  OTR_REQUIRE(!skip || (lds >= N && lds % 4 == 0 && (uintptr_t)skip % 16 == 0), "rb_linear_ln_bwd: skip alignment");
  OTR_REQUIRE(p_drop >= 0.f && p_drop < 1.f && (p_drop == 0.f || seed), "rb_linear_ln_bwd: bad dropout");
  if (M == 0) return 0;
  RbLinLnBwdArgs p{};
  p.g16 = reinterpret_cast<const uint16_t*>(g16); p.pw = reinterpret_cast<const uint4*>(wt_pack); p.skip = skip; p.z = z; p.mean = mean;
  p.rstd = rstd; p.gamma = gamma; p.seed = seed; p.dx = dx; p.da16 = reinterpret_cast<uint16_t*>(da16); p.partial = partial;
  p.ldg = ldg; p.lds = lds; p.M = (int)M; p.p_drop = p_drop; p.rng_offset = rng_offset;
  if (prefetch_bytes >= 64) { p.touch.p[0] = reinterpret_cast<const unsigned char*>(prefetch); p.touch.lines[0] = prefetch_bytes / 64; }
  {
    const RbTouch h = take_touch_hint();
    if (h.p[0]) {
      const int k = p.touch.p[0] ? 1 : 0;
      p.touch.p[k] = h.p[0]; p.touch.lines[k] = h.lines[0];
    }
  }
  const dim3 grid((unsigned)((M + RB - 1) / RB));
  hipStream_t s = (hipStream_t)stream;
  if (K == 768) hipLaunchKernelGGL((rb_linear_ln_bwd_kernel<768, 8>), grid, dim3(512), 0, s, p);
  else hipLaunchKernelGGL((rb_linear_ln_bwd_kernel<256, 8>), grid, dim3(512), 0, s, p);
  return otr_check_launch("rb_linear_ln_bwd");
}
```

### opentransformer_amd/csrc/wgrad256.h

```cpp
#pragma once
#include <hip/hip_runtime.h>
#include <stdint.h>

#include "common.h"

constexpr int W256_MAX_PROBS = 56;

struct W256Item {
  const void* dy;
  const void* x;
  float* dw;
  float* dbias;
  int M, N, K;
  int64_t ldy, ldx, ldw;
  int overwrite;
};

struct W256Prob {
  const uint16_t* dy;
  const uint16_t* x;
  float* dw;
  float* dbias;
  int start;
  int M, N, K, ldy, ldx, ldw;
  int flag0;
};

struct W256Args {
  W256Prob p[W256_MAX_PROBS];
  int total, chunk;
  int mode, nfull, rem_tiles, parts;
  int nprob, spin_limit;
  int cT1, cF1, cT2, cF2, cC1;
  FastDiv cdivF2, cdivT2;
  float* split_ws;
  int* flags;
  const void* zeros;
  int* fault;
};

int32_t wgrad256_launch(const W256Item* items, int n, void* workspace, int64_t workspace_bytes, int grid_cap, hipStream_t s);
int64_t wgrad256_workspace_bytes(const W256Item* items, int n);
int32_t wgrad256_conv_launch(const void* g2, const void* act1, float* dw2r, int B, int T1, int F1, int T2, int F2, int C1, int C2,
                             void* workspace, int64_t workspace_bytes, hipStream_t s);
```

### opentransformer_amd/csrc/wgrad256.hip

```cpp
#include "common.h"
#include "wgrad256.h"

#include <algorithm>

namespace {

typedef short v4s __attribute__((ext_vector_type(4)));
typedef __attribute__((address_space(3))) v4s lds_v4s;

constexpr int SLAB_ROWS = 16;
constexpr int SLAB_BYTES = 16384;
constexpr int RING = 8, AHEAD = 6;
constexpr int LDS_BYTES = RING * SLAB_BYTES;

__device__ __forceinline__ uint2 tr_read(uint32_t lds_addr) {
  v4s r = __builtin_amdgcn_ds_read_tr16_b64_v4i16((lds_v4s*)(uintptr_t)lds_addr);
  return __builtin_bit_cast(uint2, r);
}

struct Frags {
  uint4 a[4], b[2];
};

__device__ __forceinline__ void read_frags_lo(Frags& f, uint32_t slab_addr, uint32_t a_off, uint32_t b_off) {
// ... 358 lines not shown
}

static inline int w256_tiles(const W256Item& it) { return ((it.N + 255) / 256) * ((it.K + 255) / 256); }

static int32_t wgrad256_plan(const W256Item* it, int n, int grid_cap, W256Args& g, int& grid, int& flags) {
  if (n > W256_MAX_PROBS) {
    otr_set_error("wgrad256: %d problems exceed the table of %d", n, W256_MAX_PROBS);
    return -1;
  }
  int64_t total = 0;
  flags = 0;
  bool same_rows = true;
  for (int i = 0; i < n; ++i) {
    W256Prob& p = g.p[i];
    p.dy = reinterpret_cast<const uint16_t*>(it[i].dy); p.x = reinterpret_cast<const uint16_t*>(it[i].x); p.dw = it[i].dw;
    p.dbias = it[i].dbias;
    p.M = it[i].M; p.N = it[i].N; p.K = it[i].K; p.ldy = (int)it[i].ldy; p.ldx = (int)it[i].ldx; p.ldw = (int)it[i].ldw;
    p.start = (int)total;
    p.flag0 = flags | (it[i].overwrite ? (1 << 30) : 0);
    const int tiles = w256_tiles(it[i]), slabs = (it[i].M + SLAB_ROWS - 1) / SLAB_ROWS;
    same_rows = same_rows && it[i].M == it[0].M;
    total += (int64_t)tiles * slabs;
    flags += tiles;
  }
  if (total >= (1ll << 30)) {
    otr_set_error("wgrad256: %lld slabs do not fit the 32-bit work index", (long long)total);
    return -1;
  }
  int cap = grid_cap > 0 ? grid_cap : (grid_cap < 0 ? -grid_cap : 248);
  g.nprob = n; g.total = (int)total; g.spin_limit = g_otr_spin_limit; g.fault = g_otr_fault;
  if (same_rows && grid_cap >= 0 && flags >= 8) {
    const int R = (it[0].M + SLAB_ROWS - 1) / SLAB_ROWS, T = flags;
    double best = 1e30;
    int bestG = 8;
    for (int G = cap / 8 * 8; G >= 8 && G >= cap / 2; G -= 8) {
      const int nfull = T / G, rem = T - nfull * G, parts = rem ? std::min(G / rem, 8) : 1;
      const double cost = nfull + (rem ? 1.0 / parts + 0.02 : 0.0);
      if (cost < best - 1e-9) { best = cost; bestG = G; }
    }
    grid = bestG;
    g.mode = 1; g.chunk = R;
    g.nfull = T / grid; g.rem_tiles = T - g.nfull * grid; g.parts = g.rem_tiles ? std::min(grid / g.rem_tiles, 8) : 1;
    if (g.parts > R) g.parts = R;
  } else {
    while (cap > 1 && total / cap < 64) cap /= 2;
    const int64_t chunk = (total + cap - 1) / cap;
    grid = (int)((total + chunk - 1) / chunk);
    if (grid >= 8) grid = (grid + 7) / 8 * 8;
    g.mode = 0; g.chunk = (int)chunk;
  }
  return 0;
}

int32_t wgrad256_launch(const W256Item* it, int n, void* workspace, int64_t workspace_bytes, int grid_cap, hipStream_t s) {
  if (n <= 0) return 0;
  W256Args g{};
  int grid = 0, flags = 0;
  if (int32_t e = wgrad256_plan(it, n, grid_cap, g, grid, flags)) return e;
  const int64_t need = 64 + (int64_t)flags * 4;
  if (!workspace || workspace_bytes < need) {
    otr_set_error("wgrad256: workspace of %lld bytes, need %lld", (long long)workspace_bytes, (long long)need);
    return -1;
  }
  g.zeros = workspace;
  g.flags = reinterpret_cast<int*>(reinterpret_cast<unsigned char*>(workspace) + 64);
  hipLaunchKernelGGL(wgrad256_init_kernel, dim3(1), dim3(256), 0, s, g.flags, flags, reinterpret_cast<uint32_t*>(workspace));
  hipLaunchKernelGGL(wgrad256_kernel<>, dim3((unsigned)grid), dim3(512), 0, s, g);
  return otr_check_launch("wgrad256");
}

__global__ __launch_bounds__(256) void w256_reduce_kernel(const float* __restrict__ ws, int nslab, int64_t elems, float* __restrict__ dw) {
  const int64_t i = ((int64_t)blockIdx.x * 256 + threadIdx.x) * 4;
  if (i >= elems) return;
  float4 a = *reinterpret_cast<const float4*>(ws + i);
  for (int s = 1; s < nslab; ++s) {
    const float4 v = *reinterpret_cast<const float4*>(ws + (int64_t)s * elems + i);
    a.x += v.x; a.y += v.y; a.z += v.z; a.w += v.w;
  }
  *reinterpret_cast<float4*>(dw + i) = a;
}

int32_t wgrad256_conv_launch(const void* g2, const void* act1, float* dw2r, int B, int T1, int F1, int T2, int F2, int C1, int C2,
                             void* workspace, int64_t workspace_bytes, hipStream_t s) {
  const int64_t M = (int64_t)B * T2 * F2, K = 9ll * C1, elems = (int64_t)C2 * K;
  if (C1 % 256 != 0 || C2 % 8 != 0 || M < 16 * 2 * RING || M >= (1ll << 31) - 16) return 1;
  if (((uintptr_t)g2 | (uintptr_t)act1 | (uintptr_t)dw2r) % 16 != 0 || !workspace) return 1;
  const int tiles = ((C2 + 255) / 256) * (int)(K / 256);
  if (tiles > 256) return 1;
  const int64_t head = 256;
  int parts = 256 / tiles;
  const int64_t fit = (workspace_bytes - head) / (elems * 4);
  if (fit < parts) parts = (int)fit;
  const int R = (int)((M + SLAB_ROWS - 1) / SLAB_ROWS);
  if (parts > R / (2 * RING)) parts = R / (2 * RING);
  if (parts < 1) return 1;
  W256Args g{};
  W256Prob& p = g.p[0];
  p.dy = reinterpret_cast<const uint16_t*>(g2); p.x = reinterpret_cast<const uint16_t*>(act1); p.dw = dw2r; p.dbias = nullptr;
  p.M = (int)M; p.N = C2; p.K = (int)K; p.ldy = C2; p.ldx = C1; p.ldw = (int)K; p.start = 0; p.flag0 = 0;
  g.nprob = 1; g.total = tiles * R; g.chunk = R; g.mode = 2; g.nfull = 0; g.rem_tiles = tiles; g.parts = parts;
  g.spin_limit = g_otr_spin_limit; g.fault = g_otr_fault;
  g.cT1 = T1; g.cF1 = F1; g.cT2 = T2; g.cF2 = F2; g.cC1 = C1; g.cdivF2 = make_fastdiv((uint32_t)F2); g.cdivT2 = make_fastdiv((uint32_t)T2);
  g.zeros = workspace; g.flags = nullptr;
  g.split_ws = reinterpret_cast<float*>(reinterpret_cast<unsigned char*>(workspace) + head);
  hipLaunchKernelGGL(wgrad256_init_kernel, dim3(1), dim3(256), 0, s, nullptr, 0, reinterpret_cast<uint32_t*>(workspace));
  const int grid = (tiles * parts + 7) / 8 * 8;
  hipLaunchKernelGGL((wgrad256_kernel<true>), dim3((unsigned)grid), dim3(512), 0, s, g);
  if (int32_t e = otr_check_launch("wgrad256(conv)")) return e;
  hipLaunchKernelGGL(w256_reduce_kernel, dim3((unsigned)((elems / 4 + 255) / 256)), dim3(256), 0, s, g.split_ws, parts, elems, dw2r);
  return otr_check_launch("wgrad256(conv reduce)");
}

int64_t wgrad256_workspace_bytes(const W256Item* it, int n) {
  int64_t flags = 0;
  for (int i = 0; i < n; ++i) flags += w256_tiles(it[i]);
  return 64 + flags * 4;
}

extern "C" int32_t otr_debug_trread(const void* image, const int32_t* addr, void* out, void* stream) {
// ... 29 lines not shown
```

### opentransformer_amd/model.py

```python
import torch
import torch.nn as nn

from . import ops
from .nn import (BLK, EOS, ConformerEncoder, ConvFrontEnd, LabelSmoothingLoss, TransformerDecoder, TransformerEncoder,
                 _unsupported)

BuildFrontEnd = {'conv': ConvFrontEnd}
BuildEncoder = {'transformer': TransformerEncoder, 'conformer': ConformerEncoder}
BuildDecoder = {'transformer': TransformerDecoder}


class CTCAssistor(nn.Module):

    def __init__(self, hidden_size, vocab_size, blank=BLK, lookahead_steps=-1):
        super().__init__()
        self.lookahead_steps, self.apply_look_ahead, self.blank = lookahead_steps, lookahead_steps > 0, blank
        if self.apply_look_ahead:
            if lookahead_steps > 6 or hidden_size % 4:
                _unsupported('CTCAssistor lookahead_steps > 6 (the depthwise-conv kernels hold at most 7 taps)')
            self.lookahead_conv = nn.Conv1d(hidden_size, hidden_size, lookahead_steps + 1, padding=0, stride=1, bias=False,
                                            groups=hidden_size)
        self.output_layer = nn.Linear(hidden_size, vocab_size)

    def _look_ahead(self, memory):
        return ops.LookaheadConvFn.apply(memory, self.lookahead_conv.weight) if self.apply_look_ahead else memory

    def compute_logits(self, enc_states):
        return ops.linear(enc_states, self.output_layer.weight, self.output_layer.bias)

    def forward(self, memory, memory_length=None, targets=None, tgt_length=None, return_logits=False):
        logits = self.compute_logits(self._look_ahead(memory))
        if return_logits:
            return logits
        return self.compute_loss(logits, memory_length, targets, tgt_length)

    def compute_loss(self, logits, enc_length, targets, targets_length):
        return ops.CTCLossFn.apply(logits, targets, enc_length, targets_length, self.blank)

    def inference(self, memory, memory_mask):
        logits = self.compute_logits(self._look_ahead(memory))
        memory_length = torch.sum(memory_mask.squeeze(1) if memory_mask.dim() == 3 else memory_mask, dim=-1)
        return ops.log_softmax(logits), memory_length

    @torch.no_grad()
    def align(self, memory, memory_mask, labels, labels_length):
        log_probs, memory_length = self.inference(memory, memory_mask)
        return ops.ctc_forced_align(log_probs, memory_length, labels, labels_length, blank=self.blank)


class SpeechToText(nn.Module):

    def __init__(self, params):
        super().__init__()
        self.frontend = BuildFrontEnd[params['frontend_type']](**params['frontend'])
        self.encoder = BuildEncoder[params['encoder_type']](**params['encoder'])
        self.decoder = BuildDecoder[params['decoder_type']](**params['decoder'])
        self.crit = LabelSmoothingLoss(size=params['decoder']['vocab_size'], smoothing=params['smoothing'])
        self.ctc_weight = params['ctc_weight']
        if self.ctc_weight > 0.0:
            self.assistor = CTCAssistor(hidden_size=params['encoder_output_size'],
                                        vocab_size=params['decoder']['vocab_size'],
                                        lookahead_steps=params['lookahead_steps'] if 'lookahead_steps' in params else 0)

    def forward(self, inputs, targets):
        enc_inputs, enc_mask = inputs['inputs'], inputs['mask']
        truth, truth_length = targets['targets'], targets['targets_length']
        enc_inputs, enc_mask = self.frontend(enc_inputs, enc_mask)
        memory, memory_mask, _ = self.encoder(enc_inputs, enc_mask)
        memory = ops.early_mark(memory, self)
        if self.ctc_weight > 0 or not truth.is_cuda or truth.stride(-1) != 1:
            shifted = torch.stack((truth[:, :-1], truth[:, 1:]))
            dec_in, target_out = shifted[0], shifted[1]
        else:
            dec_in, target_out = truth[:, :-1], truth[:, 1:]
        logits, _ = self.decoder(dec_in, memory, memory_mask)
        if self.ctc_weight <= 0 and isinstance(self.crit, LabelSmoothingLoss):
            self.crit._otr_grad_scale = ops.loss_scale_of(self)
            try:
                return self.crit(logits, target_out), None
            finally:
                self.crit._otr_grad_scale = None
        loss = self.crit(logits, target_out)
        if self.ctc_weight > 0:
            loss_ctc = self.compute_ctc_loss(memory, memory_mask, target_out, truth_length)
            total = (1 - self.ctc_weight) * loss + self.ctc_weight * loss_ctc
            return ops.scale_loss_grad(total, self), {'CTCLoss': loss_ctc.detach()}
        return ops.scale_loss_grad(loss, self), None

    def compute_ctc_loss(self, memory, memory_mask, targets_out, targets_length):
        memory_length = torch.sum(memory_mask, dim=-1)
        return self.assistor(memory, memory_length, targets_out, targets_length)

    @torch.no_grad()
    def align(self, inputs, inputs_mask, labels, labels_length):
        if getattr(self, 'assistor', None) is None:
            raise ValueError('align needs the model\'s CTC head (model.assistor): build the model with ctc_weight > 0')
        n = labels_length.to(torch.int64)
        ext = torch.cat((labels.to(torch.int64), labels.new_zeros((labels.size(0), 1), dtype=torch.int64)), dim=1)
        ext.scatter_(1, n.clamp(0, labels.size(1)).unsqueeze(1), EOS)
        enc_inputs, enc_mask = self.frontend(inputs, inputs_mask)
        memory, memory_mask, _ = self.encoder(enc_inputs, enc_mask)
        frame_token, spans, label_logp, score = self.assistor.align(memory, memory_mask, ext, torch.where(n < 0, n, n + 1))
        keep = torch.arange(labels.size(1), device=labels.device).unsqueeze(0) < n.unsqueeze(1)
        spans = torch.where(keep.unsqueeze(-1), spans[:, :-1], torch.full_like(spans[:, :-1], -1))
        label_logp = torch.where(keep, label_logp[:, :-1], torch.zeros_like(label_logp[:, :-1]))
        return frame_token, spans, label_logp, score

    def save_checkpoint(self, params, name):
        checkpoint = {'params': params, 'frontend': self.frontend.state_dict(), 'encoder': self.encoder.state_dict(),
                      'decoder': self.decoder.state_dict()}
        if self.ctc_weight > 0.0:
            checkpoint['ctc'] = self.assistor.state_dict()
        torch.save(checkpoint, name)

    def load_model(self, chkpt):
        self.frontend.load_state_dict(chkpt['frontend'])
        self.encoder.load_state_dict(chkpt['encoder'])
        self.decoder.load_state_dict(chkpt['decoder'])
        if 'ctc' in chkpt and self.ctc_weight > 0.0:
            self.assistor.load_state_dict(chkpt['ctc'])

    def set_epoch(self, epoch):
        pass


class CTCModel(nn.Module):

    def __init__(self, params):
# ... 42 lines not shown
```

### opentransformer_amd/ops.py

```python
import contextlib
import ctypes as C
import gc
import math

import torch

from . import _lib as L

_state = {'compute': 'bf16', 'rng_offset': 0, 'seed': None}


@contextlib.contextmanager
def graph_capture(graph, **kw):
    gc.collect()
    was_enabled = gc.isenabled()
    gc.disable()
    _capture['serial'] += 1
    _capture['active'] = _capture['serial']
    try:
        with torch.cuda.graph(graph, **kw):
            yield graph
    finally:
        _capture['active'] = None
        if was_enabled:
# ... 306 lines not shown

    def __init__(self):
        self.armed = False
        self.buf = None


def new_link():
    return ResidualLink() if torch.is_grad_enabled() else None


class PreNormLink:
    __slots__ = ('armed', 'buf')

    def __init__(self):
        self.armed = False
        self.buf = None


def new_prenorm_link():
    return PreNormLink() if torch.is_grad_enabled() else None


class LnOutLink:
    __slots__ = ('armed', 'saved', 'params', 'result', 'prefetch')

    def __init__(self):
        self.armed, self.saved, self.params, self.result = False, None, None, None
        self.prefetch = None


_LNOUT = True


class LnInLink:
    __slots__ = ('armed', 'result', 'z')

    def __init__(self):
        self.armed, self.result, self.z = False, None, None


class PendingLn:
    __slots__ = ('kw', 'M', 'done')

    def __init__(self):
        self.kw, self.M, self.done = None, 0, True

    def desc(self):
        return _dec_ln(**self.kw)

    def finish(self):
        self.done, self.kw = True, None


def materialize(x):
    pend = getattr(x, '_otr_pending', None)
    if pend is not None and not pend.done:
        M = pend.M
        d = pend.desc()
        L.check(_timed('dec_ln', {'bytes': M * 256 * (4 + 8 + 4 + 2 + 4)}, lambda: L.load().otr_dec_ln(C.byref(d), M, _stream())), 'otr_dec_ln')
        pend.finish()
    return x


def _zero_placeholder(device, shape):
    z = _state.setdefault('zero_scalar', {}).get(device)
    if z is None:
        z = _state['zero_scalar'][device] = torch.zeros((), dtype=torch.float32, device=device)
    return z.expand(shape)


def _is_zero_placeholder(t):
    z = _state.get('zero_scalar', {}).get(t.device)
    return z is not None and t.data_ptr() == z.data_ptr() and all(st == 0 for st in t.stride())


def linear_fwd_raw(x2, w, b, out_dtype, act=L.ACT_NONE, out=None):
    M, K = x2.shape
    N = w.shape[0]
    y = out if out is not None else torch.empty((M, N), dtype=out_dtype, device=x2.device)
    d = _linear_desc(M, N, K, x2.dtype, w.dtype, y.dtype, x2.stride(0), w.stride(0), y.stride(0), act,
                     accumulate=int(out is not None))
    ws = _workspace(x2.device)
    L.check(_timed('linear_fwd %dx%dx%d' % (M, N, K), {'flops': 2.0 * M * N * K},
                   lambda: L.load().otr_linear_fwd(C.byref(d), _p(x2), _p(w), _p(b), _p(y), _p(ws), _WS_BYTES, _stream())),
            'otr_linear_fwd')
    return y


def linear_dgrad_raw(dy2, w, dx_dtype, out=None):
    M, N = dy2.shape
    K = w.shape[1]
    dx = out if out is not None else torch.empty((M, K), dtype=dx_dtype, device=dy2.device)
    d = _linear_desc(M, N, K, dx.dtype, w.dtype, dy2.dtype, dx.stride(0), w.stride(0), dy2.stride(0),
                     accumulate=int(out is not None))
    ws = _workspace(dy2.device)
    L.check(L.load().otr_linear_dgrad(C.byref(d), _p(dy2), _p(w), _p(dx), _p(ws), _WS_BYTES, _stream()), 'otr_linear_dgrad')
    return dx


_wq = {'on': False, 'w': [], 'b': [], 'post': [], 'armed': False, 'task': None}
_wq_excl = {'single_writer': set(), 'written': set(), 'cleared_in': {}}
_WG_OVERWRITE = True


def register_single_writer_grads(ptrs):
    _wq_excl['single_writer'].update(ptrs)


def unregister_single_writer_grads(ptrs):
    _wq_excl['single_writer'].difference_update(ptrs)
    _wq_excl['written'].difference_update(ptrs)
# ... 1344 lines not shown
                usave = torch.empty((lib.otr_ffn_split_padded_rows(M), F), dtype=x16.dtype, device=x.device)
            L.check(_timed('ffn_ln_fwd_split', {'flops': 6.0 * M * F * d,
                                                'bytes': M * d * (4 + 2 + 4 + 2 + 4) + 6 * F * d + (M * F * 6 if need_grad else 0)},
                           lambda: lib.otr_ffn_ln_fwd_split(_p(x2), _p(x16), _p(packs[0]), _p(b1), _p(packs[1]), _p(b2), _p(gamma),
                                                            _p(beta), _p(seed), p_drop, off, eps, _p(y), _p(y16), _p(z), _p(mean),
                                                            _p(rstd), _p(hsave), _p(usave), _p(scratch), nb, _p(sync), sync.numel(),
                                                            M, F, d, _stream())),
                    'otr_ffn_ln_fwd_split')
        else:
            L.check(_timed('ffn_ln_fwd', {'flops': 6.0 * M * F * d, 'bytes': M * d * (4 + 2 + 4 + 2 + 4) + 6 * F * d},
                           lambda: L.load().otr_ffn_ln_fwd(_p(x2), _p(x16), _p(packs[0]), _p(b1), _p(packs[1]), _p(b2), _p(gamma),
                                                           _p(beta), _p(seed), p_drop, off, eps, _p(y), _p(y16), _p(z), _p(mean),
                                                           _p(rstd), M, F, d, _stream())), 'otr_ffn_ln_fwd')
        ctx.save_for_backward(x16, z, mean, rstd, gamma, seed, b1, hsave, usave)
        ctx.packs = packs
        ctx.refs = (w1, b1, w2, b2, gamma, beta)
        ctx.cfg = (M, d, F, eps, p_drop, off, x.shape)
        ctx.olink = olink
        if olink is not None and need_grad:
            olink.saved, olink.params, olink.armed = (z, mean, rstd, gamma, seed, p_drop, off), (gamma, beta, b2), True
            if ctx.split and packs[3].data_ptr() == packs[2].data_ptr() + packs[2].numel() * packs[2].element_size():
                olink.prefetch = (packs[2], (packs[2].numel() + packs[3].numel()) * packs[2].element_size())
        y16 = y16.view(x.shape)
        ctx.mark_non_differentiable(y16)
        return y.view(x.shape), y16

    @staticmethod
    def backward(ctx, dy, _dy16=None):
        if dy is None:
            return (None,) * 13
        x16, z, mean, rstd, gamma, seed, b1, hsave, usave = ctx.saved_tensors
        M, d, F, eps, p_drop, off, xshape = ctx.cfg
        w1p, b1p, w2p, b2p, gp, bp = ctx.refs
        P1, _, P3, P4 = ctx.packs
        lib = L.load()
        gg, gb, gb2 = grad_target(gp), grad_target(bp), grad_target(b2p)
        stash = None
        if ctx.olink is not None:
            stash, ctx.olink.result = ctx.olink.result, None
        part, dgb = None, None
        if stash is not None and _is_zero_placeholder(dy):
            dx, da, part = stash
            stash = None
        else:
            dy2 = dy.reshape(-1, d).contiguous()
            dx = torch.empty_like(dy2)
            da = torch.empty((M, d), dtype=x16.dtype, device=dy.device)
            inplace = gg is not None and gb is not None and gb2 is not None
            desc = L.LnDesc(M, d, _code(da.dtype), eps, p_drop, off)
            if inplace and _wq['on'] and _in_backward():
                part = torch.empty((lib.otr_add_layernorm_bwd_partial_rows(M), 3 * d), dtype=torch.float32, device=dy.device)
            else:
                dgb = torch.zeros((3, d), dtype=torch.float32, device=dy.device)
            L.check(lib.otr_add_layernorm_bwd(C.byref(desc), _p(dy2), _p(z), _p(mean), _p(rstd), _p(gamma), _p(seed), _p(dx), _p(da),
                                              _p(dgb[0]) if dgb is not None else None, _p(dgb[1]) if dgb is not None else None,
                                              _p(dgb[2]) if dgb is not None else None, _p(part), _stream()), 'otr_add_layernorm_bwd')
            if stash is not None:
                dx.add_(stash[0])
                da = (da.float() + stash[1].float()).to(da.dtype)
                colsum_raw(stash[2][:, :d], out=gg)
                colsum_raw(stash[2][:, d:2 * d], out=gb)
                colsum_raw(stash[2][:, 2 * d:], out=gb2)
        ret_g = ret_b = ret_b2 = None
        if part is not None:
            colsum_raw(part[:, :d], out=gg)
            colsum_raw(part[:, d:2 * d], out=gb)
            colsum_raw(part[:, 2 * d:], out=gb2)
        else:
            if gg is not None:
                gg.add_(dgb[0])
            else:
                ret_g = dgb[0]
            if gb is not None:
                gb.add_(dgb[1])
            else:
                ret_b = dgb[1]
            if gb2 is not None:
                gb2.add_(dgb[2])
            else:
                ret_b2 = dgb[2]
        if ctx.split and hsave is not None:
            dh = torch.empty((usave.shape[0], 2 * F), dtype=x16.dtype, device=dy.device)[:M]
            if ctx.slab:
                bslabs = torch.empty((4, M, d), dtype=x16.dtype, device=dy.device)
                L.check(_timed('ffn_bwd_slab', {'flops': 6.0 * M * F * d, 'bytes': M * d * (2 + 8) + M * F * 8 + 6 * F * d},
                               lambda: lib.otr_ffn_bwd_split_slab(_p(da), _p(hsave), _p(P3), _p(P4), _p(dh), _p(bslabs), M, F, d,
                                                                  _stream())), 'otr_ffn_bwd_split_slab')
                il = ctx.ilink
                if il is not None and il.armed and il.result is None and _in_backward():
                    il.result = (dx, bslabs)
                    _park(il)
                    dx = _zero_placeholder(dy.device, xshape)
                else:
                    tot = torch.empty_like(dx)
                    L.check(lib.otr_dec_sum(_p(dx), _p(bslabs), 4, M, _p(tot), _stream()), 'otr_dec_sum')
                    dx = tot
            else:
                nb = lib.otr_ffn_split_scratch_bytes(M)
                scratch = torch.empty(nb // 4, dtype=torch.float32, device=dy.device)
                sync = _ffn_sync(dy.device)
                L.check(_timed('ffn_bwd_split', {'flops': 6.0 * M * F * d, 'bytes': M * d * (2 + 4 + 4) + M * F * 8 + 6 * F * d},
                               lambda: lib.otr_ffn_bwd_split(_p(da), _p(hsave), _p(P3), _p(P4), _p(dh), _p(dx), _p(dx), _p(scratch), nb,
                                                             _p(sync), sync.numel(), M, F, d, _stream())), 'otr_ffn_bwd_split')
            gw1, gb1, gw2 = grad_target(w1p), grad_target(b1p), grad_target(w2p)
            dw1 = linear_wgrad_raw(dh, x16, None, out=gw1)
            dw2 = linear_wgrad_raw(da, usave[:M], None, out=gw2)
# ... 47 lines not shown
        return u.view(*h.shape[:-1], F2 // 2)

    @staticmethod
    def backward(ctx, du):
        (h2,) = ctx.saved_tensors
        du2 = du.reshape(-1, du.shape[-1]).contiguous().to(h2.dtype)
        dh = torch.empty_like(h2)
        L.check(L.load().otr_glu_bwd(_p(h2), _p(du2), _p(dh), None, _code(h2.dtype), h2.shape[0], du2.shape[1], None, 0, _stream()),
                'otr_glu_bwd')
        return dh.view(ctx.hshape)


GLU_RPB = 32


_DEC_FUSED = True
_DEC_FFN_SLICES = 8
_EMBED_SINK = True
DEC_LAYER_PARAMS = 18


def dec_ffn_slices(F):
    for s in range(min(_DEC_FFN_SLICES, 64), 0, -1):
        if F % (128 * s) == 0:
            return s
    return 0


def _dec_ln(xres=None, x16=None, slabs=None, nslab=0, bias=None, gamma=None, beta=None, seed=None, p_drop=0.0, eps=1e-5, off=0,
            y=None, y16=None, z=None, mean=None, rstd=None):
    pv = lambda t: t.data_ptr() if t is not None else None
    return L.DecLn(pv(xres), pv(x16), pv(slabs), nslab, pv(bias), pv(gamma), pv(beta), pv(seed), p_drop, eps, off,
                   pv(y), pv(y16), pv(z), pv(mean), pv(rstd))


def _dec_lnb(dskip, slabs, nslab, saved, gamma, seed, p_drop, dz, da16, partial):
    z, mean, rstd, off = saved
    pv = lambda t: t.data_ptr() if t is not None else None
    return L.DecLnB(pv(dskip), pv(slabs), nslab, pv(z), pv(mean), pv(rstd), pv(gamma), pv(seed), p_drop, off, pv(dz), pv(da16), pv(partial))


def _grad_w(dy2, x2, w):
    gt = grad_target(w)
    r = linear_wgrad_raw(dy2, x2, None, out=gt)
    return None if gt is not None else r


def _grad_b(a2, b):
    gt = grad_target(b)
    r = colsum_raw(a2, out=gt)
    return None if gt is not None else r


class DecoderStackFn(torch.autograd.Function):

    @staticmethod
    def forward(ctx, x0, kv_all, kmask, n_layers, p_drop, eps, S, share, *params):
        _cuda(x0, kv_all)
        ctx.set_materialize_grads(False)
        lib = L.load()
        B, Lq, d = x0.shape
        R, H = B * Lq, 4
        T, W = kv_all.shape[1], kv_all.shape[2]
        dev, hdt = x0.device, half_dtype()
        assert share >= 1 and kv_all.shape[0] * share == B
        ctx.share = share
        assert d == 256 and kv_all.is_contiguous() and kv_all.dtype == hdt and W == n_layers * 512 and len(params) == DEC_LAYER_PARAMS * n_layers
        xres, x16 = x0.reshape(R, d).contiguous(), lp_of(x0).reshape(R, d).contiguous()
        seed = rng_seed_tensor(dev) if p_drop > 0 else None
        f32 = lambda *sh: torch.empty(sh, dtype=torch.float32, device=dev)
        h16 = lambda *sh: torch.empty(sh, dtype=hdt, device=dev)
        slA, slB, slC = h16(4, R, d), h16(4, R, d), h16(S, R, d)
        need = any(ctx.needs_input_grad)
        st = _stream()

        def ln_out(xres_, slabs, nslab, bias, gamma, beta):
            y, y16, z, mean, rstd = f32(R, d), h16(R, d), f32(R, d), f32(R), f32(R)
            off = _next_rng_offset(R * d) if p_drop > 0 else 0
            desc = _dec_ln(xres_, None, slabs, nslab, bias, gamma, beta, seed, p_drop, eps, off, y, y16, z, mean, rstd)
            return desc, y, y16, (z, mean, rstd, off)

        layers, packs_all = [], []
        y_in, y_in16, pending = xres, x16, None
        F = params[12].shape[0] // 2
        if need:
            rng = []
            for l in range(n_layers):
                pr = params[DEC_LAYER_PARAMS * l:DEC_LAYER_PARAMS * (l + 1)]
                for t in (*lin_packs(pr[0]), *lin_packs(pr[2]), *lin_packs(pr[6]), *lin_packs(pr[8]), *ffn_packs(pr[12], pr[14])):
                    rng.append((t.data_ptr(), t.numel() * t.element_size()))
            rng.sort()
            merged = [list(rng[0])]
            for a, n in rng[1:]:
                if a <= merged[-1][0] + merged[-1][1] + 4096:
                    merged[-1][1] = max(merged[-1][1], a + n - merged[-1][0])
                else:
                    merged.append([a, n])
            for a, n in merged:
                L.check(lib.otr_touch(C.c_void_p(a), n, st), 'otr_touch')
        for l in range(n_layers):
            (wqkv, bqkv, wo, bo, g1, be1, wq, bq, wo2, bo2, g2, be2, w1, b1, w2, b2, g3, be3) = params[DEC_LAYER_PARAMS * l:DEC_LAYER_PARAMS * (l + 1)]
            pk = (lin_packs(wqkv), lin_packs(wo), lin_packs(wq), lin_packs(wo2), ffn_packs(w1, w2))
            packs_all.append(pk)
            rec = {}
            if pending is None:
                lnA, y0, y016 = _dec_ln(None, x16, None, 0), xres, x16
            else:
                lnA, y0, y016, rec_prev = ln_out(y_in, *pending)
                layers[-1]['ln3'] = rec_prev
            qkv16, ctx1, lse1 = h16(R, 3 * d), h16(R, d), f32(B, H, Lq)
            fl_self = 2.0 * R * d * (3 * d + d) + 4.0 * R * Lq * d
            L.check(_timed('dec_self_fwd', {'flops': fl_self}, lambda lnA=lnA, pk=pk, bqkv=bqkv, qkv16=qkv16, ctx1=ctx1, lse1=lse1: lib.otr_dec_self_fwd(
                C.byref(lnA), B, Lq, _p(pk[0][0]), _p(bqkv), _p(pk[1][0]), _p(qkv16), _p(ctx1), _p(lse1), _p(slA), _stream())), 'otr_dec_self_fwd')
            lnB, y1, y116, rec['ln1'] = ln_out(y0, slA, 4, bo, g1, be1)
            q16, ctx2, lse2 = h16(R, d), h16(R, d), f32(B, H, Lq)
            fl_cross = 2.0 * R * d * (d + d) + 4.0 * R * T * d
            if share == 1:
                L.check(_timed('dec_cross_fwd', {'flops': fl_cross}, lambda lnB=lnB, pk=pk, bq=bq, q16=q16, ctx2=ctx2, lse2=lse2, l=l: lib.otr_dec_cross_fwd(
                    C.byref(lnB), B, Lq, _p(pk[2][0]), _p(bq), _p(pk[3][0]), _p(kv_all), T * W, W, l * 512, l * 512 + 256, _p(kmask), T, _p(q16), _p(ctx2),
                    _p(lse2), _p(slB), _stream())), 'otr_dec_cross_fwd')
            else:
                L.check(lib.otr_dec_cross_fwd_shared(C.byref(lnB), B, Lq, _p(pk[2][0]), _p(bq), _p(pk[3][0]), _p(kv_all), T * W, W, l * 512,
                                                     l * 512 + 256, _p(kmask), T, share, _p(q16), _p(ctx2), _p(lse2), _p(slB), _stream()),
                        'otr_dec_cross_fwd_shared')
            lnC, y2, y216, rec['ln2'] = ln_out(y1, slB, 4, bo2, g2, be2)
            hsave = torch.empty(lib.otr_dec_ffn_hsave_bytes(R, F) // 2, dtype=hdt, device=dev) if need else None
            L.check(_timed('dec_ffn_fwd', {'flops': 6.0 * R * F * d}, lambda lnC=lnC, pk=pk, b1=b1, hsave=hsave: lib.otr_dec_ffn_fwd(
                C.byref(lnC), R, _p(pk[4][0]), _p(b1), _p(pk[4][1]), F, S, _p(slC), _p(hsave), _stream())), 'otr_dec_ffn_fwd')
            rec.update(hsave=hsave, y016=y016, qkv16=qkv16, ctx1=ctx1, lse1=lse1, y116=y116, q16=q16, ctx2=ctx2, lse2=lse2, y216=y216)
            layers.append(rec)
            y_in, pending = y2, (slC, S, b2, g3, be3)
        lnF, y3, y316, rec_last = ln_out(y_in, *pending)
        layers[-1]['ln3'] = rec_last
        L.check(lib.otr_dec_ln(C.byref(lnF), R, st), 'otr_dec_ln')
        ctx.layers, ctx.packs, ctx.params = layers, packs_all, params
        ctx.cfg = (B, Lq, d, T, W, n_layers, p_drop, S, F, seed)
        ctx.kv, ctx.kmask = kv_all, kmask
        ctx.sink = getattr(x0, '_otr_embed_sink', None) if _EMBED_SINK else None
        y3, y316 = y3.view(B, Lq, d), y316.view(B, Lq, d)
        ctx.mark_non_differentiable(y316)
        return y3, y316

    @staticmethod
    def backward(ctx, dy, _dy16=None):
        n_in = 8
        assert ctx.share == 1, 'the shared-memory decoder stack is forward only'
        if dy is None:
            return (None,) * (n_in + len(ctx.params))
        lib = L.load()
        B, Lq, d, T, W, n_layers, p_drop, S, F, seed = ctx.cfg
        R, G = B * Lq, max(1, lib.otr_dec_group_size(B, Lq))
        ngrp, nblk = (B + G - 1) // G, (R + 31) // 32
# ... 30 lines not shown
            dz1, da1, part1, dqkv16, slAb = f32(R, d), h16(R, d), f32(ngrp, 3 * d), h16(R, 3 * d), h16(4, R, d)
            lnb = _dec_lnb(dz2, slBb, 4, rec['ln1'], g1, seed, p_drop, dz1, da1, part1)
            L.check(_timed('dec_self_bwd', {'flops': 2.0 * R * d * (3 * d + d) + 10.0 * R * Lq * d},
                           lambda lnb=lnb, pk=pk, rec=rec, dqkv16=dqkv16, slAb=slAb: lib.otr_dec_self_bwd(
                               C.byref(lnb), B, Lq, _p(pk[1][1]), _p(pk[0][1]), _p(rec['qkv16']), _p(rec['ctx1']), _p(rec['lse1']), _p(dqkv16),
                               _p(slAb), _stream())), 'otr_dec_self_bwd')
            grads[o + 4], grads[o + 5], grads[o + 3] = _grad_b(part1[:, :d], g1), _grad_b(part1[:, d:2 * d], be1), _grad_b(part1[:, 2 * d:], bo)
            grads[o + 2], grads[o + 0], grads[o + 1] = _grad_w(da1, rec['ctx1'], wo), _grad_w(dqkv16, rec['y016'], wqkv), _grad_b(dqkv16, bqkv)
            dskip, slabs, nslab = dz1, slAb, 4
        dx0 = None
        if ctx.needs_input_grad[0]:
            sink = ctx.sink
            if sink is not None and sink.buf is None and _in_backward() and slabs is not None:
                sink.buf = (dskip, slabs, nslab)
                _park(sink)
                dx0 = _zero_placeholder(dev, (B, Lq, d))
            else:
                dx0 = f32(R, d)
                L.check(lib.otr_dec_sum(_p(dskip), _p(slabs), nslab, R, _p(dx0), st), 'otr_dec_sum')
                dx0 = dx0.view(B, Lq, d)
        return (dx0, dkv if ctx.needs_input_grad[1] else None, None, None, None, None, None, None, *grads)


def decoder_stack_applies(x0, memory, blocks, normalize_before):
    if not _DEC_FUSED or not is_half() or not x0.is_cuda or normalize_before or lp_of(x0) is None or x0.dim() != 3:
        return 0
    B, Lq, d = x0.shape
    if d != 256 or Lq > 32 or Lq < 1 or len(blocks) < 1:
        return 0
    F = None
    for b in blocks:
        sa, ca, ff = b.slf_attn, b.src_attn, b.feed_forward
        if (b.concat_after or b.normalize_before or sa.nheads != 4 or ca.nheads != 4 or sa.share_qvk_proj or ca.share_vk_proj
                or ff.activation != 'glu' or (b.training and (sa.dropout_rate or ca.dropout_rate or ff.dropout))):
            return 0
        if ff.w_1.bias is None or ff.w_2.bias is None or tuple(ff.w_2.weight.shape) != (256, ff.w_1.weight.shape[0] // 2):
            return 0
        if F is None:
            F = ff.w_2.weight.shape[1]
        if ff.w_2.weight.shape[1] != F or tuple(ca.vk_proj.weight.shape) != (512, memory.shape[-1]):
            return 0
        for w in (sa.qvk_proj.weight, sa.output_proj.weight, ca.q_proj.weight, ca.output_proj.weight):
            if lin_packs(w) is None:
                return 0
        if ffn_packs(ff.w_1.weight, ff.w_2.weight) is None:
            return 0
    return dec_ffn_slices(F)


def decoder_stack(x0, kv_all, kmask_u8, blocks, S, share=1):
    p = blocks[0].residual_dropout if blocks[0].training else 0.0
    params = []
    for b in blocks:
        sa, ca, ff = b.slf_attn, b.src_attn, b.feed_forward
        params += [sa.qvk_proj.weight, sa.qvk_proj.bias, sa.output_proj.weight, sa.output_proj.bias, b.norm1.weight, b.norm1.bias,
                   ca.q_proj.weight, ca.q_proj.bias, ca.output_proj.weight, ca.output_proj.bias, b.norm2.weight, b.norm2.bias,
                   ff.w_1.weight, ff.w_1.bias, ff.w_2.weight, ff.w_2.bias, b.norm3.weight, b.norm3.bias]
    y, y16 = DecoderStackFn.apply(x0, kv_all, kmask_u8, len(blocks), float(p), float(blocks[0].norm1.eps), S, int(share), *params)
    return attach_lp(y, y16)


class _Grad16Link:
    buf = None
    armed = False


_G16 = True


class PosEncFn(torch.autograd.Function):

    @staticmethod
    def forward(ctx, x, mask=None):
        _cuda(x)
        ctx.set_materialize_grads(False)
        B, T, d = x.shape
        x = x.contiguous().float()
        y = torch.empty_like(x)
        ylp = torch.empty(x.shape, dtype=half_dtype(), device=x.device) if is_half() else None
        ctx.scale = math.sqrt(d)
        ctx.g16 = getattr(x, '_otr_g16', None)
        u8 = None
        if (mask is not None and d % 4 == 0 and mask.is_cuda and mask.dim() == 2 and tuple(mask.shape) == (B, T)
                and mask.dtype in (torch.bool, torch.uint8) and getattr(mask, '_otr_u8', (None,))[0] != mask._version):
            u8 = torch.empty((B, T), dtype=torch.uint8, device=x.device)
            L.check(L.load().otr_posenc_mask_fwd(_p(x), _p(y), _p(ylp), B * T, T, d, ctx.scale, _p(mask), mask.stride(0), mask.stride(1),
                                                 _p(u8), _stream()), 'otr_posenc_mask_fwd')
            mask._otr_u8 = (mask._version, u8)
        else:
            L.check(L.load().otr_posenc_fwd(_p(x), _p(y), _p(ylp), B * T, T, d, ctx.scale, _stream()), 'otr_posenc_fwd')
        if ylp is not None:
            ctx.mark_non_differentiable(ylp)
        return y, ylp

    @staticmethod
    def backward(ctx, dy, _dylp=None):
        if dy is None:
            return None, None
        dy = dy.contiguous()
        link = ctx.g16
        if (link is not None and link.armed and link.buf is None and dy.dtype == torch.float32 and is_half() and _in_backward()
                and dy.data_ptr() % 16 == 0):
            g16 = torch.empty(dy.shape, dtype=half_dtype(), device=dy.device)
            L.check(L.load().otr_scale_cast(_p(dy), _p(g16), dy.numel(), ctx.scale, _stream()), 'otr_scale_cast')
            link.buf = g16
            _park(link)
            return _zero_placeholder(dy.device, dy.shape), None
        dx = torch.empty_like(dy)
        L.check(L.load().otr_scale(_p(dy), _p(dx), dy.numel(), None, ctx.scale, _stream()), 'otr_scale')
        return dx, None
# ... 1260 lines not shown
```

Before: 8013 utterances/s.

## Cut kernel launches: merge colsum passes, one wgrad init, fused optimizer tick, piggyback touches

Several changes aim to reduce the number of kernel launches per step. Colsum groups now mix fp32 and half items in one launch and hold up to 240 descriptors, found by binary search. The wgrad256 flag init runs once for all runs. Optimizer norm and tick work appears to be fused through a ticket counter. Separate decoder weight-prefetch launches are replaced by extra 'rider' workgroups attached to the LN forward and LN backward kernels. The risks are larger kernel argument structs, extra workgroups on existing kernels, and more complex ordering logic. A launch counter is also added for debugging.

```diff
diff --git a/include/otrans_hip.h b/include/otrans_hip.h
--- a/include/otrans_hip.h
+++ b/include/otrans_hip.h
@@ -110,6 +110,7 @@
 int32_t otr_debug_attention_grid(int32_t nx, int32_t H, int32_t B, int32_t* out, int32_t cap);
 int32_t otr_debug_wgrad256_plan(const otr_wgrad_item_t* items, int32_t n, int32_t grid_cap, int32_t* out);
 int32_t otr_debug_wgrad256_errors(const void* workspace);
+int64_t otr_debug_launch_count(void);
 int32_t otr_linear_wgrad_grouped(const otr_wgrad_item_t* items, int32_t n, int32_t compute, void* workspace,
                                  int64_t workspace_bytes, void* stream);
 typedef struct {
diff --git a/opentransformer_amd/_lib.py b/opentransformer_amd/_lib.py
--- a/opentransformer_amd/_lib.py
+++ b/opentransformer_amd/_lib.py
@@ -129,6 +129,7 @@
     'otr_debug_attention_grid': [_I32, _I32, _I32, _P, _I32],
     'otr_debug_wgrad256_plan': [C.POINTER(WgradItem), _I32, _I32, _P],
     'otr_debug_wgrad256_errors': [_P],
+    'otr_debug_launch_count': [],
     'otr_debug_trread': [_P, _P, _P, _P],
     'otr_spec_mask': [_P, _P, _I32, _I32, _I32, _I32, _P],
     'otr_transpose_batched': [_P, _P, _P, _I32, _I64, _I32, _P],
@@ -246,7 +247,7 @@
     'otr_bn_swish_bwd_sums': [_P, _P, _I32, _P, _P, _P, _P, _P, _P, _P, _I64, _I32, _P],
     'otr_conformer_conv_bwd_mid': [_P] * 13 + [_I32] * 7 + [_P],
 }
-_RESTYPE = {'otr_last_error_string': C.c_char_p, 'otr_dec_ffn_hsave_bytes': C.c_int64, 'otr_ffn_split_scratch_bytes': C.c_int64, 'otr_ffn_split_sync_ints': C.c_int64, 'otr_ffn_split_hsave_bytes': C.c_int64,
+_RESTYPE = {'otr_last_error_string': C.c_char_p, 'otr_debug_launch_count': C.c_int64, 'otr_dec_ffn_hsave_bytes': C.c_int64, 'otr_ffn_split_scratch_bytes': C.c_int64, 'otr_ffn_split_sync_ints': C.c_int64, 'otr_ffn_split_hsave_bytes': C.c_int64,
             'otr_ffn_split_padded_rows': C.c_int64, 'otr_add_layernorm_bwd_partial_rows': C.c_int64,
             'otr_ln_bwd_proj_partial_rows': C.c_int64, 'otr_dwconv_bwd_partial_rows': C.c_int64, 'otr_dwconv_fwd_partial_rows': C.c_int64,
             'otr_conv2_wide_scratch_bytes': C.c_int64, 'otr_add2_colsum_partial_rows': C.c_int64,
diff --git a/opentransformer_amd/csrc/api.hip b/opentransformer_amd/csrc/api.hip
--- a/opentransformer_amd/csrc/api.hip
+++ b/opentransformer_amd/csrc/api.hip
@@ -3,6 +3,7 @@
 #include <stdlib.h>
 
 #include <algorithm>
+#include <atomic>
 #include <vector>
 
 #include "gemm_kernel.h"
@@ -17,7 +18,12 @@
   va_end(ap);
 }
 
+static std::atomic<int64_t> g_launches{0};
+void otr_note_launches(int n) { g_launches.fetch_add(n, std::memory_order_relaxed); }
+extern "C" int64_t otr_debug_launch_count(void) { return g_launches.exchange(0, std::memory_order_relaxed); }
+
 int32_t otr_check_launch(const char* what) {
+  g_launches.fetch_add(1, std::memory_order_relaxed);
   hipError_t e = hipGetLastError();
   if (e != hipSuccess) {
     otr_set_error("%s: launch failed: %s", what, hipGetErrorString(e));
@@ -273,19 +279,31 @@
       if (items[a].M != items[b].M) return items[a].M > items[b].M;
       return narrow(a) < narrow(b);
     });
-    size_t c0 = 0;
-    while (c0 < idx.size()) {
+    struct Run { size_t c0, c1; int flag0; };
+    std::vector<Run> runs;
+    int flags = 0;
+    for (size_t c0 = 0; c0 < idx.size();) {
       size_t c1 = c0;
       while (c1 < idx.size() && c1 - c0 < (size_t)W256_MAX_PROBS && items[idx[c1]].M == items[idx[c0]].M && narrow(idx[c1]) == narrow(idx[c0])) ++c1;
+      int64_t tiles = 0;
+      for (size_t c = c0; c < c1; ++c) tiles += (int64_t)((items[idx[c]].N + 255) / 256) * ((items[idx[c]].K + 255) / 256);
+      if (!workspace || 64 + ((int64_t)flags + tiles) * 4 > workspace_bytes) break;
+      runs.push_back(Run{c0, c1, flags});
+      flags += (int)tiles;
+      c0 = c1;
+    }
+    if (!runs.empty()) {
+      wgrad256_init(workspace, flags, s);
+      otr_note_launches(1);
+    }
+    for (const Run& r : runs) {
       big.clear();
-      for (size_t c = c0; c < c1; ++c) {
+      for (size_t c = r.c0; c < r.c1; ++c) {
         const otr_wgrad_item_t& it = items[idx[c]];
         big.push_back(W256Item{it.dy, it.x, it.dw, it.dbias, it.M, it.N, it.K, it.ldy, it.ldx, it.ldw, it.overwrite != 0});
       }
-      if (!workspace || wgrad256_workspace_bytes(big.data(), (int)big.size()) > workspace_bytes) break;
-      if (int32_t e = wgrad256_launch(big.data(), (int)big.size(), workspace, workspace_bytes, g_otr_wgrad256_grid, s)) return e;
-      for (size_t c = c0; c < c1; ++c) taken[(size_t)idx[c]] = 1;
-      c0 = c1;
+      if (int32_t e = wgrad256_launch(big.data(), (int)big.size(), workspace, workspace_bytes, g_otr_wgrad256_grid, s, r.flag0)) return e;
+      for (size_t c = r.c0; c < r.c1; ++c) taken[(size_t)idx[c]] = 1;
     }
   }
   std::vector<int> order[16];
diff --git a/opentransformer_amd/csrc/common.h b/opentransformer_amd/csrc/common.h
--- a/opentransformer_amd/csrc/common.h
+++ b/opentransformer_amd/csrc/common.h
@@ -19,6 +19,7 @@
 
 void otr_set_error(const char* fmt, ...);
 int32_t otr_check_launch(const char* what);
+void otr_note_launches(int n);
 void otr_zero_f32(float* p, int64_t n, hipStream_t s);
 #define OTR_REQUIRE(cond, ...)          \
   do {                                  \
@@ -49,6 +50,34 @@
 extern int32_t* g_otr_fault;
 extern unsigned long long* g_otr_trace;
 
+struct RbTouch { const unsigned char* p[2]; int64_t lines[2]; };
+RbTouch otr_take_touch_hint();
+static inline unsigned otr_touch_riders(const RbTouch& t) {
+  const int64_t total = t.p[0] ? t.lines[0] + t.lines[1] : 0;
+  const int64_t g = (total + 511) / 512;
+  return (unsigned)(g > 1024 ? 1024 : g);
+}
+#ifdef __HIPCC__
+__device__ __forceinline__ void otr_touch_ride(const RbTouch& t, int rider, int nriders) {
+  const int64_t total = t.lines[0] + t.lines[1];
+  if (total <= 0) return;
+  const int64_t nthr = (int64_t)blockDim.x * blockDim.y * blockDim.z, stride = nthr * nriders;
+  const int tid = (int)((threadIdx.z * blockDim.y + threadIdx.y) * blockDim.x + threadIdx.x);
+  uint32_t acc = 0;
+  for (int64_t l = (int64_t)rider * nthr + tid; l < total; l += 4 * stride) {
+    uint32_t v[4];
+#pragma unroll
+    for (int u = 0; u < 4; ++u) {
+      const int64_t k = min(l + u * stride, total - 1);
+      const unsigned char* a = k < t.lines[0] ? t.p[0] + k * 64 : t.p[1] + (k - t.lines[0]) * 64;
+      v[u] = *reinterpret_cast<const volatile uint32_t*>(a);
+    }
+    acc |= v[0] | v[1] | v[2] | v[3];
+  }
+  if (acc == 0x9e3779b9u && total < 0) const_cast<unsigned char*>(t.p[0])[0] = 0;
+}
+#endif
+
 typedef uint32_t otr_u32x4 __attribute__((ext_vector_type(4)));
 typedef uint32_t otr_u32x2 __attribute__((ext_vector_type(2)));
 #define OTR_GLOBAL __attribute__((address_space(1)))
diff --git a/opentransformer_amd/csrc/declayer.hip b/opentransformer_amd/csrc/declayer.hip
--- a/opentransformer_amd/csrc/declayer.hip
+++ b/opentransformer_amd/csrc/declayer.hip
@@ -799,7 +799,10 @@
     }
   }
 }
-__global__ __launch_bounds__(256) void dec_ln_kernel(DlLnArgs p) { dec_ln_body(p, (int)blockIdx.x); }
+__global__ __launch_bounds__(256) void dec_ln_kernel(DlLnArgs p, RbTouch touch, int own) {
+  if ((int)blockIdx.x >= own) { otr_touch_ride(touch, (int)blockIdx.x - own, (int)gridDim.x - own); return; }
+  dec_ln_body(p, (int)blockIdx.x);
+}
 struct DlLnPair { DlLnArgs a, b; int n0; };
 __global__ __launch_bounds__(256) void dec_ln_pair_kernel(DlLnPair pp) {
   if ((int)blockIdx.x < pp.n0) dec_ln_body(pp.a, (int)blockIdx.x);
@@ -1668,7 +1671,9 @@
   OTR_REQUIRE(R > 0 && R < (1ll << 31), "dec_ln: bad row count");
   if (int32_t e = dl_check_ln("dec_ln", ln, R, a.ln)) return e;
   OTR_REQUIRE(ln->nslab > 0, "dec_ln: nothing to normalise");
-  hipLaunchKernelGGL(dec_ln_kernel, dim3((unsigned)((R + 7) / 8)), dim3(256), 0, (hipStream_t)stream, a);
+  const RbTouch touch = otr_take_touch_hint();
+  const unsigned own = (unsigned)((R + 7) / 8);
+  hipLaunchKernelGGL(dec_ln_kernel, dim3(own + otr_touch_riders(touch)), dim3(256), 0, (hipStream_t)stream, a, touch, (int)own);
   return otr_check_launch("dec_ln");
 }
 
diff --git a/opentransformer_amd/csrc/elementwise.hip b/opentransformer_amd/csrc/elementwise.hip
--- a/opentransformer_amd/csrc/elementwise.hip
+++ b/opentransformer_amd/csrc/elementwise.hip
@@ -530,28 +530,27 @@
   return otr_check_launch("colsum");
 }
 
-constexpr int CSG_MAX = 64;
+constexpr int CSG_MAX = 240;
+struct ColsumDesc {
+  const void* a;
+  float* out;
+  int M, N, lda;
+  int first;
+  int rpb;
+  int tpr_h16;
+};
 struct ColsumGroup {
-  int n;
-  int first[CSG_MAX + 1];
-  const void* a[CSG_MAX];
-  float* out[CSG_MAX];
-  int M[CSG_MAX], N[CSG_MAX], lda[CSG_MAX], rblocks[CSG_MAX];
-  int tpr[CSG_MAX];
-  int rpb[CSG_MAX];
+  int n, blocks;
+  ColsumDesc d[CSG_MAX];
 };
-template <class T> __global__ void colsum_grouped_kernel(ColsumGroup g) {
+template <class T> __device__ __forceinline__ void colsum_item(const ColsumDesc& d, const int lb, float (*red)[4]) {
   constexpr int EPT = 4, UN = 8;
-  __shared__ float red[256][EPT];
-  const int b = (int)blockIdx.x;
-  int i = 0;
-  for (int j = 1; j < g.n; ++j) i = (g.first[j] <= b) ? j : i;
-  const T* a = reinterpret_cast<const T*>(g.a[i]);
-  float* out = g.out[i];
-  const int64_t M = g.M[i], N = g.N[i], lda = g.lda[i];
-  const int tpr = g.tpr[i], nrl = 256 / tpr;
-  const int rpb = g.rpb[i];
-  const int lb = b - g.first[i], by = lb % g.rblocks[i], bx = lb / g.rblocks[i];
+  const T* a = reinterpret_cast<const T*>(d.a);
+  float* out = d.out;
+  const int64_t M = d.M, N = d.N, lda = d.lda;
+  const int tpr = d.tpr_h16 & 0xff, nrl = 256 / tpr;
+  const int rpb = d.rpb, rblocks = (int)((M + rpb - 1) / rpb);
+  const int by = lb % rblocks, bx = lb / rblocks;
   const int t = (int)(threadIdx.y * 64 + threadIdx.x);
   const int tx = t % tpr, ty = t / tpr;
   const int64_t c = ((int64_t)bx * tpr + tx) * EPT;
@@ -595,47 +594,59 @@
     }
   }
 }
+__global__ __launch_bounds__(256) void colsum_grouped_kernel(ColsumGroup g) {
+  __shared__ float red[256][4];
+  const int b = (int)blockIdx.x;
+  int lo = 0, hi = g.n - 1;
+  while (lo < hi) {
+    const int mid = (lo + hi + 1) >> 1;
+    if (g.d[mid].first <= b) lo = mid; else hi = mid - 1;
+  }
+  const ColsumDesc d = g.d[lo];
+  if (d.tpr_h16 >> 8) colsum_item<bf16_t>(d, b - d.first, red);
+  else colsum_item<float>(d, b - d.first, red);
+}
 extern "C" int32_t otr_colsum_grouped(const otr_colsum_item_t* items, int32_t n, void* stream) {
   OTR_REQUIRE(n >= 0 && (items || n == 0), "colsum_grouped: null items");
   hipStream_t s = (hipStream_t)stream;
-  for (int pass = 0; pass < 2; ++pass) {
-    const int dt = pass == 0 ? OTR_F32 : OTR_H16;
-    ColsumGroup g{};
-    int blocks = 0;
-    auto flush = [&]() -> int32_t {
-      if (g.n == 0) return 0;
-      g.first[g.n] = blocks;
-      if (dt == OTR_F32) hipLaunchKernelGGL(colsum_grouped_kernel<float>, dim3((unsigned)blocks), dim3(64, 4), 0, s, g);
-      else hipLaunchKernelGGL(colsum_grouped_kernel<bf16_t>, dim3((unsigned)blocks), dim3(64, 4), 0, s, g);
-      g.n = 0;
-      blocks = 0;
-      return otr_check_launch("colsum_grouped");
-    };
-    for (int i = 0; i < n; ++i) {
-      const otr_colsum_item_t& it = items[i];
-      OTR_REQUIRE(it.a && it.out, "colsum_grouped: item %d has a null pointer", i);
-      OTR_REQUIRE(it.dtype == OTR_F32 || it.dtype == OTR_H16, "colsum_grouped: item %d has a bad dtype", i);
-      OTR_REQUIRE(it.N > 0 && it.M >= 0 && it.lda >= it.N && it.lda < (1ll << 31) && it.M < (1ll << 31),
-                  "colsum_grouped: item %d has a bad shape", i);
-      OTR_REQUIRE((uintptr_t)it.a % 16 == 0, "colsum_grouped: item %d input must be 16-byte aligned", i);
-      if (it.dtype != dt || it.M == 0) continue;
-      int tpr = 64;
-      while (tpr > 8 && (int64_t)(tpr / 2) * 4 >= it.N) tpr /= 2;
-      const int nrl = 256 / tpr, pass_rows = nrl * 8 > 128 ? nrl * 8 : 128;
-      int rpb = pass_rows;
-      if ((it.M + rpb - 1) / rpb > 192) rpb = (int)(((it.M + 191) / 192 + pass_rows - 1) / pass_rows) * pass_rows;
-      const int cpb = tpr * 4;
-      const int rb = (int)((it.M + rpb - 1) / rpb), cb = (int)((it.N + cpb - 1) / cpb);
-      const int k = g.n++;
-      g.first[k] = blocks;
-      g.a[k] = it.a; g.out[k] = it.out; g.M[k] = (int)it.M; g.N[k] = (int)it.N; g.lda[k] = (int)it.lda; g.rblocks[k] = rb; g.tpr[k] = tpr; g.rpb[k] = rpb;
-      blocks += rb * cb;
-      if (g.n == CSG_MAX)
-        if (int32_t e = flush()) return e;
-    }
-    if (int32_t e = flush()) return e;
-  }
-  return 0;
+  for (int i = 0; i < n; ++i) {
+    const otr_colsum_item_t& it = items[i];
+    OTR_REQUIRE(it.a && it.out, "colsum_grouped: item %d has a null pointer", i);
+    OTR_REQUIRE(it.dtype == OTR_F32 || it.dtype == OTR_H16, "colsum_grouped: item %d has a bad dtype", i);
+    OTR_REQUIRE(it.N > 0 && it.M >= 0 && it.lda >= it.N && it.lda < (1ll << 31) && it.M < (1ll << 31) && it.N < (1ll << 31),
+                "colsum_grouped: item %d has a bad shape", i);
+    OTR_REQUIRE((uintptr_t)it.a % 16 == 0, "colsum_grouped: item %d input must be 16-byte aligned", i);
+  }
+  static thread_local ColsumGroup g;
+  g.n = 0; g.blocks = 0;
+  int launches = 0;
+  auto flush = [&]() {
+    if (g.n == 0) return;
+    hipLaunchKernelGGL(colsum_grouped_kernel, dim3((unsigned)g.blocks), dim3(64, 4), 0, s, g);
+    g.n = 0; g.blocks = 0;
+    ++launches;
+  };
+  for (int i = 0; i < n; ++i) {
+    const otr_colsum_item_t& it = items[i];
+    if (it.M == 0) continue;
+    int tpr = 64;
+    while (tpr > 8 && (int64_t)(tpr / 2) * 4 >= it.N) tpr /= 2;
+    const int nrl = 256 / tpr, pass_rows = nrl * 8 > 128 ? nrl * 8 : 128;
+    int rpb = pass_rows;
+    if ((it.M + rpb - 1) / rpb > 192) rpb = (int)(((it.M + 191) / 192 + pass_rows - 1) / pass_rows) * pass_rows;
+    const int cpb = tpr * 4;
+    const int64_t nb = ((it.M + rpb - 1) / rpb) * ((it.N + cpb - 1) / cpb);
+    if (g.n == CSG_MAX || g.blocks + nb >= (1ll << 31)) flush();
+    OTR_REQUIRE(nb < (1ll << 31), "colsum_grouped: item %d needs too many workgroups", i);
+    ColsumDesc& d = g.d[g.n++];
+    d.a = it.a; d.out = it.out; d.M = (int)it.M; d.N = (int)it.N; d.lda = (int)it.lda; d.first = g.blocks; d.rpb = rpb;
+    d.tpr_h16 = tpr | ((it.dtype == OTR_H16 ? 1 : 0) << 8);
+    g.blocks += (int)nb;
+  }
+  flush();
+  if (launches == 0) return 0;
+  otr_note_launches(launches - 1);
+  return otr_check_launch("colsum_grouped");
 }
 
 template <class T>
diff --git a/opentransformer_amd/csrc/norm.hip b/opentransformer_amd/csrc/norm.hip
--- a/opentransformer_amd/csrc/norm.hip
+++ b/opentransformer_amd/csrc/norm.hip
@@ -13,6 +13,7 @@
   const float* gamma3; const float* beta3; float* mean3; float* rstd3; float* y3; bf16_t* y3_lp; const void* dy3; int dy3_h16;
   int dy_h16;
   const uint8_t* amask;
+  RbTouch touch; int riders;
 };
 
 constexpr int LN_MAXV = 4;
@@ -168,6 +169,7 @@
 
 template <class AT, bool HAS_A, int NV, bool LN2 = false> __global__ __launch_bounds__(512) void add_ln_bwd_kernel(LnArgs p) {
   constexpr int ROWS = 1, NWV = 8, NTH = 64 * NWV;
+  if (p.riders && blockIdx.x >= gridDim.x - p.riders) { otr_touch_ride(p.touch, (int)(blockIdx.x - (gridDim.x - p.riders)), p.riders); return; }
   __shared__ float red[2][NWV][NV * 256];
   const int lane = threadIdx.x & 63, wid = threadIdx.x >> 6;
   const int d = p.d;
@@ -449,7 +451,8 @@
   p.seed = seed; p.skip = skip; p.dx = dx; p.da = da; p.dgamma = dgamma; p.dbeta = dbeta; p.da_colsum = da ? da_colsum : nullptr; p.partial = partial;
   p.M = d->M; p.d = d->d; p.eps = d->eps; p.p_drop = d->p_drop; p.rng_offset = d->rng_offset;
   p.a_scale = d->a_scale == 0.f ? 1.f : d->a_scale; p.amask = d->a_row_mask;
-  dim3 grid((unsigned)((d->M + 2 * LN_BWD_ROWS - 1) / (2 * LN_BWD_ROWS)));
+  p.touch = otr_take_touch_hint(); p.riders = (int)otr_touch_riders(p.touch);
+  dim3 grid((unsigned)((d->M + 2 * LN_BWD_ROWS - 1) / (2 * LN_BWD_ROWS)) + (unsigned)p.riders);
   hipStream_t s = (hipStream_t)stream;
 #define LN_BWD_LAUNCH(NV)                                                                                   \
   {                                                                                                         \
diff --git a/opentransformer_amd/csrc/optim.hip b/opentransformer_amd/csrc/optim.hip
--- a/opentransformer_amd/csrc/optim.hip
+++ b/opentransformer_amd/csrc/optim.hip
@@ -1,5 +1,6 @@
 #include "common.h"
 
+constexpr int OPT_NORM_WG = 512;
 struct OptState {
   float step;
   float lr;
@@ -11,13 +12,17 @@
   float unscale;
   float growth_interval;
   float faults;
-  float reserved[5];
+  uint32_t ticket;
+  float reserved[4];
   float norm_part[512];
 };
-constexpr int OPT_NORM_WG = 512;
 
-__global__ void sqnorm_kernel(const float* g, int64_t n, OptState* st) {
+struct TickArgs { float base_lr, model_size, warmup, factor, step_offset, beta1, beta2, grad_scale; int32_t* fault; };
+__device__ void opt_tick(OptState* st, const TickArgs& a, int nparts);
+
+__global__ void sqnorm_kernel(const float* g, int64_t n, OptState* st, TickArgs tick) {
   __shared__ float sh[4];
+  __shared__ int last_flag;
   float s = 0.f;
   const int64_t n4 = n / 4;
   const float4* g4 = reinterpret_cast<const float4*>(g);
@@ -38,42 +43,61 @@
   s = wave_sum(s);
   if ((threadIdx.x & 63) == 0) sh[threadIdx.x >> 6] = s;
   __syncthreads();
-  if (threadIdx.x == 0) st->norm_part[blockIdx.x] = sh[0] + sh[1] + sh[2] + sh[3];
+  if (threadIdx.x == 0) {
+    __hip_atomic_store(st->norm_part + blockIdx.x, sh[0] + sh[1] + sh[2] + sh[3], __ATOMIC_RELAXED, __HIP_MEMORY_SCOPE_AGENT);
+    asm volatile("s_waitcnt vmcnt(0)" ::: "memory");
+    const uint32_t arrived = __hip_atomic_fetch_add(&st->ticket, 1u, __ATOMIC_RELAXED, __HIP_MEMORY_SCOPE_AGENT);
+    last_flag = (arrived == gridDim.x - 1);
+  }
+  __syncthreads();
+  if (!last_flag || threadIdx.x >= 64) return;
+  opt_tick(st, tick, (int)gridDim.x);
 }
 
-__global__ void opt_tick_kernel(OptState* st, float base_lr, float model_size, float warmup, float factor,
-                                float step_offset, float beta1, float beta2, float grad_scale, int32_t* fault, int nparts) {
+__device__ void opt_tick(OptState* st, const TickArgs& a, int nparts) {
+  const float base_lr = a.base_lr, model_size = a.model_size, warmup = a.warmup, factor = a.factor, step_offset = a.step_offset;
+  const float beta1 = a.beta1, beta2 = a.beta2, grad_scale = a.grad_scale;
+  int32_t* fault = a.fault;
+  const float loss_scale = st->loss_scale, good_steps = st->good_steps, growth_interval = st->growth_interval, step = st->step;
+  const float skipped = st->skipped, faults = st->faults;
+  int32_t nf = 0;
+  if (fault && threadIdx.x == 0) nf = __hip_atomic_exchange(fault, 0, __ATOMIC_RELAXED, __HIP_MEMORY_SCOPE_AGENT);
+  static_assert(OPT_NORM_WG == 8 * 64, "eight parts per lane");
+  float v[8];
+#pragma unroll
+  for (int k = 0; k < 8; ++k) {
+    const int i = (int)threadIdx.x + 64 * k;
+    v[k] = __hip_atomic_load(st->norm_part + min(i, nparts - 1), __ATOMIC_RELAXED, __HIP_MEMORY_SCOPE_AGENT);
+  }
   float part = 0.f;
-  for (int i = threadIdx.x; i < nparts; i += 64) part += st->norm_part[i];
+#pragma unroll
+  for (int k = 0; k < 8; ++k) part += ((int)threadIdx.x + 64 * k < nparts) ? v[k] : 0.f;
   part = wave_sum(part);
   if (threadIdx.x != 0) return;
+  __hip_atomic_store(&st->ticket, 0u, __ATOMIC_RELAXED, __HIP_MEMORY_SCOPE_AGENT);
   st->sqnorm = part;
-  const float ls = st->loss_scale > 0.f ? st->loss_scale : 1.f;
+  const float ls = loss_scale > 0.f ? loss_scale : 1.f;
   const float us = grad_scale / ls;
   st->unscale = us;
-  if (fault) {
-    const int32_t nf = __hip_atomic_exchange(fault, 0, __ATOMIC_RELAXED, __HIP_MEMORY_SCOPE_AGENT);
-    if (nf != 0) {
-      st->faults += (float)nf;
-      st->skipped += 1.f;
-      st->unscale = __builtin_nanf("");
-      return;
-    }
-  }
-  float norm = sqrtf(st->sqnorm) * us;
-  if (!isfinite(norm)) {
-    st->skipped += 1.f;
-    if (st->loss_scale > 0.f) { st->loss_scale = fmaxf(ls * 0.5f, 1.f); st->good_steps = 0.f; }
+  if (nf != 0) {
+    st->faults = faults + (float)nf;
+    st->skipped = skipped + 1.f;
+    st->unscale = __builtin_nanf("");
     return;
   }
-  if (st->loss_scale > 0.f) {
-    st->good_steps += 1.f;
-    if (st->growth_interval > 0.f && st->good_steps >= st->growth_interval) {
-      st->loss_scale = fminf(ls * 2.f, 65536.f);
-      st->good_steps = 0.f;
-    }
+  float norm = sqrtf(part) * us;
+  if (!isfinite(norm)) {
+    st->skipped = skipped + 1.f;
+    if (loss_scale > 0.f) { st->loss_scale = fmaxf(ls * 0.5f, 1.f); st->good_steps = 0.f; }
+    return;
   }
-  float t = st->step + 1.f;
+  if (loss_scale > 0.f) {
+    const float good = good_steps + 1.f;
+    const bool grow = growth_interval > 0.f && good >= growth_interval;
+    if (grow) st->loss_scale = fminf(ls * 2.f, 65536.f);
+    st->good_steps = grow ? 0.f : good;
+  }
+  float t = step + 1.f;
   st->step = t;
   st->bc1 = 1.f - powf(beta1, t);
   st->bc2 = 1.f - powf(beta2, t);
@@ -154,12 +178,12 @@
   OptState* st = reinterpret_cast<OptState*>(state);
   unsigned grid = (unsigned)((n / 4 + 255) / 256 > OPT_NORM_WG ? OPT_NORM_WG : (n / 4 + 255) / 256);
   if (grid < 1) grid = 1;
-  hipLaunchKernelGGL(sqnorm_kernel, dim3(grid), dim3(256), 0, s, grad, n, st);
-  hipLaunchKernelGGL(opt_tick_kernel, dim3(1), dim3(64), 0, s, st, base_lr, noam_model_size, noam_warmup, noam_factor,
-                     noam_step_offset, beta1, beta2, grad_scale, g_otr_fault, (int)grid);
+  const TickArgs tick{base_lr, noam_model_size, noam_warmup, noam_factor, noam_step_offset, beta1, beta2, grad_scale, g_otr_fault};
+  hipLaunchKernelGGL(sqnorm_kernel, dim3(grid), dim3(256), 0, s, grad, n, st, tick);
   unsigned g2 = (unsigned)((n / 4 + 255) / 256 > 4096 ? 4096 : (n / 4 + 255) / 256);
   if (g2 < 1) g2 = 1;
   hipLaunchKernelGGL(adam_kernel, dim3(g2), dim3(256), 0, s, param, grad, exp_avg, exp_avg_sq, n, st, (bf16_t*)param_bf16, beta1, beta2, eps,
                      weight_decay, clip_norm, grad_noise_std);
+  otr_note_launches(1);
   return otr_check_launch("optimizer_step");
 }
diff --git a/opentransformer_amd/csrc/rowblock.hip b/opentransformer_amd/csrc/rowblock.hip
--- a/opentransformer_amd/csrc/rowblock.hip
+++ b/opentransformer_amd/csrc/rowblock.hip
@@ -53,7 +53,6 @@
   }
 };
 
-struct RbTouch { const unsigned char* p[2]; int64_t lines[2]; };
 constexpr int RB_TOUCH_PER = 10;
 __device__ __forceinline__ void rb_touch_issue(const RbTouch& t, uint32_t (&sink)[RB_TOUCH_PER], int tid, int nthr) {
   if (!t.p[0]) return;
@@ -598,7 +597,7 @@
   if (bytes1 >= 64) { g_touch_hint.p[n] = reinterpret_cast<const unsigned char*>(p1); g_touch_hint.lines[n] = bytes1 / 64; ++n; }
   return 0;
 }
-static RbTouch take_touch_hint() { RbTouch t = g_touch_hint; g_touch_hint = RbTouch{}; return t; }
+RbTouch otr_take_touch_hint() { RbTouch t = g_touch_hint; g_touch_hint = RbTouch{}; return t; }
 
 extern "C" int32_t otr_proj_ln_fwd(const float* x, const void* c16, int64_t ldc, const void* w_pack, const float* bias, const float* gamma,
                                    const float* beta, const uint64_t* seed, float* y, void* y16, float* z, float* mean, float* rstd,
@@ -612,7 +611,7 @@
   p.x = x; p.c16 = reinterpret_cast<const uint16_t*>(c16); p.pw = reinterpret_cast<const uint4*>(w_pack); p.bias = bias; p.gamma = gamma;
   p.beta = beta; p.seed = seed; p.y = y; p.y16 = reinterpret_cast<uint16_t*>(y16); p.z = z; p.mean = mean; p.rstd = rstd;
   p.ldc = ldc; p.M = (int)M; p.eps = eps; p.p_drop = p_drop; p.rng_offset = rng_offset;
-  p.touch = take_touch_hint();
+  p.touch = otr_take_touch_hint();
   hipLaunchKernelGGL(proj_ln_fwd_kernel<8>, dim3((unsigned)((M + RB - 1) / RB)), dim3(512), 0, (hipStream_t)stream, p);
   return otr_check_launch("proj_ln_fwd");
 }
@@ -632,7 +631,7 @@
   p.dy = dy; p.z = z; p.mean = mean; p.rstd = rstd; p.gamma = gamma; p.seed = seed; p.pwt = reinterpret_cast<const uint4*>(wt_pack);
   p.dx = dx; p.da16 = reinterpret_cast<uint16_t*>(da16); p.dc16 = reinterpret_cast<uint16_t*>(dc16); p.partial = partial;
   p.ldc = ldc; p.M = (int)M; p.p_drop = p_drop; p.rng_offset = rng_offset;
-  p.touch = take_touch_hint();
+  p.touch = otr_take_touch_hint();
   hipLaunchKernelGGL(ln_bwd_proj_kernel<8>, dim3((unsigned)((M + RB - 1) / RB)), dim3(512), 0, (hipStream_t)stream, p);
   return otr_check_launch("ln_bwd_proj");
 }
@@ -652,7 +651,7 @@
   p.dy = dskip; p.z = z; p.mean = mean; p.rstd = rstd; p.gamma = gamma; p.seed = seed; p.pwt = reinterpret_cast<const uint4*>(wt_pack);
   p.dx = dx; p.da16 = reinterpret_cast<uint16_t*>(da16); p.dc16 = reinterpret_cast<uint16_t*>(dc16); p.partial = partial;
   p.ldc = ldc; p.M = (int)M; p.p_drop = p_drop; p.rng_offset = rng_offset;
-  p.touch = take_touch_hint();
+  p.touch = otr_take_touch_hint();
   hipLaunchKernelGGL(ln_bwd_proj_kernel<8>, dim3((unsigned)((M + RB - 1) / RB)), dim3(512), 0, (hipStream_t)stream, p);
   return otr_check_launch("ln_bwd_proj_slabs");
 }
@@ -687,7 +686,7 @@
   p.ldg = ldg; p.lds = lds; p.M = (int)M; p.p_drop = p_drop; p.rng_offset = rng_offset;
   if (prefetch_bytes >= 64) { p.touch.p[0] = reinterpret_cast<const unsigned char*>(prefetch); p.touch.lines[0] = prefetch_bytes / 64; }
   {
-    const RbTouch h = take_touch_hint();
+    const RbTouch h = otr_take_touch_hint();
     if (h.p[0]) {
       const int k = p.touch.p[0] ? 1 : 0;
       p.touch.p[k] = h.p[0]; p.touch.lines[k] = h.lines[0];
diff --git a/opentransformer_amd/csrc/wgrad256.h b/opentransformer_amd/csrc/wgrad256.h
--- a/opentransformer_amd/csrc/wgrad256.h
+++ b/opentransformer_amd/csrc/wgrad256.h
@@ -39,7 +39,8 @@
   int* fault;
 };
 
-int32_t wgrad256_launch(const W256Item* items, int n, void* workspace, int64_t workspace_bytes, int grid_cap, hipStream_t s);
+int32_t wgrad256_launch(const W256Item* items, int n, void* workspace, int64_t workspace_bytes, int grid_cap, hipStream_t s, int flag_offset = -1);
+void wgrad256_init(void* workspace, int flags, hipStream_t s);
 int64_t wgrad256_workspace_bytes(const W256Item* items, int n);
 int32_t wgrad256_conv_launch(const void* g2, const void* act1, float* dw2r, int B, int T1, int F1, int T2, int F2, int C1, int C2,
                              void* workspace, int64_t workspace_bytes, hipStream_t s);
diff --git a/opentransformer_amd/csrc/wgrad256.hip b/opentransformer_amd/csrc/wgrad256.hip
--- a/opentransformer_amd/csrc/wgrad256.hip
+++ b/opentransformer_amd/csrc/wgrad256.hip
@@ -434,19 +434,28 @@
   return 0;
 }
 
-int32_t wgrad256_launch(const W256Item* it, int n, void* workspace, int64_t workspace_bytes, int grid_cap, hipStream_t s) {
+void wgrad256_init(void* workspace, int flags, hipStream_t s) {
+  hipLaunchKernelGGL(wgrad256_init_kernel, dim3(1), dim3(256), 0, s, reinterpret_cast<int*>(reinterpret_cast<unsigned char*>(workspace) + 64), flags,
+                     reinterpret_cast<uint32_t*>(workspace));
+}
+
+int32_t wgrad256_launch(const W256Item* it, int n, void* workspace, int64_t workspace_bytes, int grid_cap, hipStream_t s, int flag_offset) {
   if (n <= 0) return 0;
   W256Args g{};
   int grid = 0, flags = 0;
   if (int32_t e = wgrad256_plan(it, n, grid_cap, g, grid, flags)) return e;
-  const int64_t need = 64 + (int64_t)flags * 4;
+  const int first = flag_offset < 0 ? 0 : flag_offset;
+  const int64_t need = 64 + ((int64_t)first + flags) * 4;
   if (!workspace || workspace_bytes < need) {
     otr_set_error("wgrad256: workspace of %lld bytes, need %lld", (long long)workspace_bytes, (long long)need);
     return -1;
   }
   g.zeros = workspace;
-  g.flags = reinterpret_cast<int*>(reinterpret_cast<unsigned char*>(workspace) + 64);
-  hipLaunchKernelGGL(wgrad256_init_kernel, dim3(1), dim3(256), 0, s, g.flags, flags, reinterpret_cast<uint32_t*>(workspace));
+  g.flags = reinterpret_cast<int*>(reinterpret_cast<unsigned char*>(workspace) + 64) + first;
+  if (flag_offset < 0) {
+    wgrad256_init(workspace, flags, s);
+    otr_note_launches(1);
+  }
   hipLaunchKernelGGL(wgrad256_kernel<>, dim3((unsigned)grid), dim3(512), 0, s, g);
   return otr_check_launch("wgrad256");
 }
diff --git a/opentransformer_amd/model.py b/opentransformer_amd/model.py
--- a/opentransformer_amd/model.py
+++ b/opentransformer_amd/model.py
@@ -66,6 +66,7 @@
         enc_inputs, enc_mask = inputs['inputs'], inputs['mask']
         truth, truth_length = targets['targets'], targets['targets_length']
         enc_inputs, enc_mask = self.frontend(enc_inputs, enc_mask)
+        ops.touch_decoder_behind_encoder(self.decoder)
         memory, memory_mask, _ = self.encoder(enc_inputs, enc_mask)
         memory = ops.early_mark(memory, self)
         if self.ctc_weight > 0 or not truth.is_cuda or truth.stride(-1) != 1:
@@ -74,6 +75,7 @@
         else:
             dec_in, target_out = truth[:, :-1], truth[:, 1:]
         logits, _ = self.decoder(dec_in, memory, memory_mask)
+        ops.touch_behind(None)
         if self.ctc_weight <= 0 and isinstance(self.crit, LabelSmoothingLoss):
             self.crit._otr_grad_scale = ops.loss_scale_of(self)
             try:
diff --git a/opentransformer_amd/ops.py b/opentransformer_amd/ops.py
--- a/opentransformer_amd/ops.py
+++ b/opentransformer_amd/ops.py
@@ -382,11 +382,25 @@
         self.done, self.kw = True, None
 
 
+def touch_behind(ranges):
+    _state['touch_behind'] = {'ranges': [tuple(r) for r in ranges], 'done': False} if ranges and len(ranges) <= 2 else None
+
+
+def touched(ranges):
+    t, _state['touch_behind'] = _state.get('touch_behind'), None
+    return t is not None and t['done'] and t['ranges'] == [tuple(r) for r in ranges]
+
+
 def materialize(x):
     pend = getattr(x, '_otr_pending', None)
     if pend is not None and not pend.done:
         M = pend.M
         d = pend.desc()
+        t = _state.get('touch_behind')
+        if t is not None and not t['done']:
+            r = t['ranges'] + [(None, 0)]
+            L.check(L.load().otr_touch_hint(C.c_void_p(r[0][0]), r[0][1], C.c_void_p(r[1][0]), r[1][1]), 'otr_touch_hint')
+            t['done'] = True
         L.check(_timed('dec_ln', {'bytes': M * 256 * (4 + 8 + 4 + 2 + 4)}, lambda: L.load().otr_dec_ln(C.byref(d), M, _stream())), 'otr_dec_ln')
         pend.finish()
     return x
@@ -1837,6 +1851,8 @@
                 part = torch.empty((lib.otr_add_layernorm_bwd_partial_rows(M), 3 * d), dtype=torch.float32, device=dy.device)
             else:
                 dgb = torch.zeros((3, d), dtype=torch.float32, device=dy.device)
+            if ctx.split and hsave is not None and P4.data_ptr() == P3.data_ptr() + P3.numel() * P3.element_size():
+                L.check(lib.otr_touch_hint(_p(P3), (P3.numel() + P4.numel()) * P3.element_size(), None, 0), 'otr_touch_hint')
             L.check(lib.otr_add_layernorm_bwd(C.byref(desc), _p(dy2), _p(z), _p(mean), _p(rstd), _p(gamma), _p(seed), _p(dx), _p(da),
                                               _p(dgb[0]) if dgb is not None else None, _p(dgb[1]) if dgb is not None else None,
                                               _p(dgb[2]) if dgb is not None else None, _p(part), _stream()), 'otr_add_layernorm_bwd')
@@ -1990,6 +2006,49 @@
     return None if gt is not None else r
 
 
+def dec_pack_ranges(layers):
+    rng = []
+    for pr in layers:
+        packs = (lin_packs(pr[0]), lin_packs(pr[2]), lin_packs(pr[6]), lin_packs(pr[8]), ffn_packs(pr[12], pr[14]))
+        if any(pk is None for pk in packs):
+            return None
+        for t in (t for pk in packs for t in pk):
+            rng.append((t.data_ptr(), t.numel() * t.element_size()))
+    rng.sort()
+    merged = [list(rng[0])]
+    for a, n in rng[1:]:
+        if a <= merged[-1][0] + merged[-1][1] + 4096:
+            merged[-1][1] = max(merged[-1][1], a + n - merged[-1][0])
+        else:
+            merged.append([a, n])
+    return [tuple(m) for m in merged]
+
+
+def touch_decoder_behind_encoder(decoder):
+    _state['touch_behind'] = None
+    blocks = getattr(decoder, 'blocks', None)
+    if not blocks or not _DEC_FUSED or not is_half() or not torch.is_grad_enabled():
+        return
+    try:
+        if any(getattr(b.feed_forward, 'activation', None) != 'glu' for b in blocks):
+            return
+        layers = [_dec_layer_params(b) for b in blocks]
+    except AttributeError:
+        return
+    if any(getattr(pr[i], '_otr_lin_packs', None) is None for pr in layers for i in (0, 2, 6, 8)):
+        return
+    if any(getattr(pr[12], '_otr_ffn_packs', None) is None for pr in layers):
+        return
+    touch_behind(dec_pack_ranges(layers))
+
+
+def _dec_layer_params(b):
+    sa, ca, ff = b.slf_attn, b.src_attn, b.feed_forward
+    return [sa.qvk_proj.weight, sa.qvk_proj.bias, sa.output_proj.weight, sa.output_proj.bias, b.norm1.weight, b.norm1.bias,
+            ca.q_proj.weight, ca.q_proj.bias, ca.output_proj.weight, ca.output_proj.bias, b.norm2.weight, b.norm2.bias,
+            ff.w_1.weight, ff.w_1.bias, ff.w_2.weight, ff.w_2.bias, b.norm3.weight, b.norm3.bias]
+
+
 class DecoderStackFn(torch.autograd.Function):
 
     @staticmethod
@@ -2022,20 +2081,10 @@
         y_in, y_in16, pending = xres, x16, None
         F = params[12].shape[0] // 2
         if need:
-            rng = []
-            for l in range(n_layers):
-                pr = params[DEC_LAYER_PARAMS * l:DEC_LAYER_PARAMS * (l + 1)]
-                for t in (*lin_packs(pr[0]), *lin_packs(pr[2]), *lin_packs(pr[6]), *lin_packs(pr[8]), *ffn_packs(pr[12], pr[14])):
-                    rng.append((t.data_ptr(), t.numel() * t.element_size()))
-            rng.sort()
-            merged = [list(rng[0])]
-            for a, n in rng[1:]:
-                if a <= merged[-1][0] + merged[-1][1] + 4096:
-                    merged[-1][1] = max(merged[-1][1], a + n - merged[-1][0])
-                else:
-                    merged.append([a, n])
-            for a, n in merged:
-                L.check(lib.otr_touch(C.c_void_p(a), n, st), 'otr_touch')
+            merged = dec_pack_ranges([params[DEC_LAYER_PARAMS * l:DEC_LAYER_PARAMS * (l + 1)] for l in range(n_layers)])
+            if not touched(merged):
+                for a, n in merged:
+                    L.check(lib.otr_touch(C.c_void_p(a), n, st), 'otr_touch')
         for l in range(n_layers):
             (wqkv, bqkv, wo, bo, g1, be1, wq, bq, wo2, bo2, g2, be2, w1, b1, w2, b2, g3, be3) = params[DEC_LAYER_PARAMS * l:DEC_LAYER_PARAMS * (l + 1)]
             pk = (lin_packs(wqkv), lin_packs(wo), lin_packs(wq), lin_packs(wo2), ffn_packs(w1, w2))
@@ -2172,10 +2221,7 @@
     p = blocks[0].residual_dropout if blocks[0].training else 0.0
     params = []
     for b in blocks:
-        sa, ca, ff = b.slf_attn, b.src_attn, b.feed_forward
-        params += [sa.qvk_proj.weight, sa.qvk_proj.bias, sa.output_proj.weight, sa.output_proj.bias, b.norm1.weight, b.norm1.bias,
-                   ca.q_proj.weight, ca.q_proj.bias, ca.output_proj.weight, ca.output_proj.bias, b.norm2.weight, b.norm2.bias,
-                   ff.w_1.weight, ff.w_1.bias, ff.w_2.weight, ff.w_2.bias, b.norm3.weight, b.norm3.bias]
+        params += _dec_layer_params(b)
     y, y16 = DecoderStackFn.apply(x0, kv_all, kmask_u8, len(blocks), float(p), float(blocks[0].norm1.eps), S, int(share), *params)
     return attach_lp(y, y16)
 
```

Measured after the change: 8005 utterances/s. Within noise of the previous version (-0.1%).
